# shroglck/open-pi-zero

Hardware: AMD Instinct MI355X
Metric: train samples/sec at gbsz 1024 (bf16 fwd+bwd+clip+AdamW) (higher is better)
Workload: dtype bf16; 1 GPU; Pi0 bridge training step: 256 img + 20 text + 1 proprio + 4 action tokens; model=pi0 (SigLIP-So400m/14 + Gemma-2B + 0.3B action expert), global_batch=1024, micro_batch=256, grad_accum=4, seq_len=281, parallelism=dp1

## Files before the change

### include/pz_abi.h

```cpp
#ifndef PZ_ABI_H
#define PZ_ABI_H

#include <stdint.h>

#ifdef __cplusplus
extern "C" {
#endif

#define PZ_ABI_VERSION 22

enum {
  PZ_OK = 0,
  PZ_ERR_INVALID_ARG = 1,
  PZ_ERR_LAUNCH = 2,
  PZ_ERR_UNSUPPORTED = 3,
};

enum {
  PZ_EPI_NONE = 0,
  PZ_EPI_GELU = 1,
  PZ_EPI_GEGLU = 2,
  PZ_EPI_SILU = 3,
  PZ_EPI_DGELU = 4,
  PZ_EPI_DSILU = 5,
  PZ_EPI_DGEGLU = 6,
};

typedef struct pz_gemm_args {
  int64_t M, N, K;
  const void* A; int64_t lda; int32_t a_kcontig;
  const void* B; int64_t ldb; int32_t b_kcontig;
  void* C; int64_t ldc; int32_t c_fp32;
  int64_t batch, batch_inner;
  int64_t sA_outer, sA_inner, sB_outer, sB_inner, sC_outer, sC_inner, sR_outer, sR_inner;
  int32_t epilogue;
  float alpha;
  int32_t beta_accum;
  const void* bias;
  const void* resid; int64_t ld_resid;
  void* aux; int64_t ld_aux;
  int64_t geglu_inter;
  void* workspace; int64_t ws_bytes;
  const void* norm_w; float norm_eps;
  int32_t fp8_mode; const float* a_row_scale;
  const void* A2; int64_t lda2;
  const void* B2; int64_t ldb2;
  int64_t K2;
} pz_gemm_args;
int pz_gemm(const pz_gemm_args* args, void* stream);
#define PZ_ABSMAX_PARTS 1024
int pz_fp8_quant_vt(const void* v, int64_t ldv, int64_t v_bstride, int64_t Z, int64_t nk, void* vt, float* vs,
                    int64_t ldt, void* stream);
int pz_fp8_quant_attn(const void* q, int64_t nqr, const void* k, int64_t nkr, const void* v, int64_t ldv,
                      int64_t v_bstride, int64_t Z, int64_t nk, void* qc, float* qs, void* kc, float* ks, void* vt,
                      float* vs, int64_t ldt, void* stream);
int pz_rmsnorm_fwd_f8(const void* x, int64_t ldx, const void* w, void* q, int64_t ldq, float* qscale, int64_t R,
                      int64_t D, float eps, void* stream);
int pz_layernorm_fwd_f8(const void* x, int64_t ldx, const void* w, const void* b, void* q, int64_t ldq, float* qscale,
                        int64_t R, int64_t D, float eps, void* stream);
int pz_fp8_quant_rows(const void* x, int64_t ldx, void* q, int64_t ldq, float* row_scale, int64_t R, int64_t D,
                      void* stream);
int pz_fp8_quant_tensor(const void* x, int64_t n, void* q, float inv_scale, void* stream);
int pz_fp8_absmax(const void* x, int64_t n, float* parts, void* stream);
const char* pz_gemm_kernel_name(const pz_gemm_args* args);

typedef struct pz_small_gemm_args {
  int64_t M, N, K;
  const void* A; int64_t sAm, sAk;
  const void* B; int64_t sBk, sBn;
  void* C; int64_t ldc;
  const void* bias;
  float alpha;
  int32_t beta;
} pz_small_gemm_args;
int pz_gemm_small(const pz_small_gemm_args* args, void* stream);

int pz_rmsnorm_fwd(const void* x, int64_t ldx, const void* w, void* y, int64_t ldy, float* rstd,
                   int64_t R, int64_t D, float eps, void* stream);
int pz_rmsnorm_bwd(const void* dy, int64_t lddy, const void* x, int64_t ldx, const void* w,
                   const float* rstd, const void* dres, void* dx, int64_t lddx, float* dw_part,
                   int64_t R, int64_t D, void* stream);
int pz_layernorm_fwd(const void* x, int64_t ldx, const void* w, const void* b, void* y, int64_t ldy,
                     float* mean, float* rstd, int64_t R, int64_t D, float eps, void* stream);
int pz_layernorm_bwd(const void* dy, int64_t lddy, const void* x, int64_t ldx, const void* w,
                     const float* mean, const float* rstd, const void* dres, void* dx, int64_t lddx,
                     float* dw_part, float* db_part, int64_t R, int64_t D, float* dx_part, void* stream);
int64_t pz_norm_rows_per_part(void);
int pz_reduce_parts(const float* part, int64_t P, int64_t D, void* out, int32_t beta, void* stream);
typedef struct pz_reduce_seg {
  const float* part; int64_t P, D; void* out; int32_t beta;
} pz_reduce_seg;
int pz_reduce_parts_multi(const pz_reduce_seg* segs, int32_t nseg, void* stream);
int pz_act_bwd_colsum(const void* dh, int64_t lddh, const void* pre, int64_t ldpre, void* dpre, int64_t M, int64_t N,
                      int32_t act, float* ws, int64_t ws_rows, void* dbias, int32_t beta, void* stream);
int pz_colsum(const void* X, int64_t ld, int64_t M, int64_t N, void* out, int32_t beta, float* ws,
              void* stream);
int pz_batch_sum(const void* X, int64_t B, int64_t stride, int64_t n, void* out, int32_t beta, void* stream);

int pz_rope_table(float* cs, int64_t max_pos, int64_t head_dim, float theta, void* stream);
int pz_qkv_rope_split(const void* qkv, const int64_t* pos, const float* cs, void* q_out, void* k_out,
                      void* v_out, int64_t B, int64_t T, int64_t nh, int64_t nkv, int64_t hd,
                      int64_t Lq, int64_t qoff, int64_t Lk, int64_t koff, void* stream);
typedef struct pz_qkv_rope_args {
  const void* x; int64_t ldx;
  const void* W; int64_t ldw;
  int64_t M, N, K;
  const void* norm_w; float norm_eps;
  const int64_t* pos; const float* cs;
  void* q_out; void* k_out; void* v_out;
  int64_t T, nh, hd, Lq, qoff, Lk, koff;
  int32_t w_fp8; float w_scale;
  const void* x2; int64_t ldx2;
  const void* W2; int64_t ldw2;
  int64_t K2;
} pz_qkv_rope_args;
int pz_gemv_qkv_rope(const pz_qkv_rope_args* a, void* stream);
int pz_gemm_qkv_rope(const pz_qkv_rope_args* a, void* stream);
int pz_qkv_rope_split_bwd(const void* dq, const void* dk, const void* dv, const int64_t* pos,
                          const float* cs, void* dqkv, int64_t B, int64_t T, int64_t nh, int64_t nkv,
                          int64_t hd, int64_t Lq, int64_t qoff, int64_t Lk, int64_t koff, void* stream);

typedef struct pz_softmax_args {
  const float* S; int64_t lds;
  void* P; int64_t ldp;
  void* tcap;
  int64_t R, N;
  float scale, cap;
  int32_t mask_mode;
  int64_t rows_per_batch, heads, qoff;
  const int32_t* cnt; int64_t prefix, cond;
  const float* mask; int64_t ldm, mask_bstride;
} pz_softmax_args;
int pz_attn_softmax(const pz_softmax_args* a, void* stream);
int pz_attn_softmax_bwd(const void* P, const float* dP, int64_t lddp, const void* tcap, void* dS,
                        int64_t ldp, int64_t R, int64_t N, float scale, float cap, void* stream);

typedef struct pz_flash_args {
  int64_t Z, H, nq, nk, head_dim;
  const void* q; int64_t ldq, q_bstride, q_hstride;
  const void* k; int64_t ldk, k_bstride, k_hstride;
  const void* v; int64_t ldv, v_bstride, v_hstride;
  int32_t n_groups;
  int64_t g_row0[3];
  void* g_o[3];
  int64_t g_bstride[3], g_ld[3];
  int64_t o_hstride;
  float* lse;
  float scale, cap;
  int32_t mask_mode;
  const int32_t* cnt; int64_t prefix, cond, rows_per_token;
  const void* g_do[3];
  float* delta;
  void* dq; void* dk; void* dv;
  float* ws; int64_t ws_bytes;
  int64_t mask_row0;
} pz_flash_args;
int pz_flash_fwd(const pz_flash_args* a, void* stream);
int pz_flash_fwd_f8(const pz_flash_args* a, const void* qc, const float* qs, const void* kc, const float* ks,
                    int64_t krows, const void* vtc, const float* vs, int64_t ldvt, void* stream);
int pz_flash_fwd_probs(const pz_flash_args* a, void* P, void* tcap, int64_t ldp, void* stream);
int pz_flash_bwd_ds(const pz_flash_args* a, const void* P, const void* tcap, void* dS, int64_t ldp, void* stream);
int pz_flash_bwd_prep(const pz_flash_args* a, void* stream);
int pz_flash_bwd(const pz_flash_args* a, void* stream);

typedef struct pz_decode_attn_args {
  const void* q; int64_t ldq, Lq, qoff;
  const void* k; const void* v; int64_t k_bstride, v_bstride;
  void* o; int64_t ldo;
  int64_t B, nh, T, nk, head_dim;
  float scale, cap;
  const int32_t* cnt; int64_t prefix, cond, qtok0;
  float* ws; int64_t ws_bytes;
} pz_decode_attn_args;
int64_t pz_decode_attn_ws_bytes(int64_t B, int64_t rows, int64_t nk);
int pz_decode_attn(const pz_decode_attn_args* a, void* stream);

int pz_patchify(const void* pix, void* cols, int64_t B, int64_t H, int64_t W, int64_t ps, int64_t ldc,
                void* stream);
int pz_embed_merge(const int64_t* ids, const void* table, int64_t vocab, const void* img, void* out,
                   int64_t B, int64_t P, int64_t D, int64_t n_img, int64_t image_token, int64_t pad_token,
                   float emb_scale, float img_scale, void* stream);
int pz_embed_merge_bwd(const int64_t* ids, const void* dout, void* dimg, int64_t B, int64_t P,
                       int64_t D, int64_t n_img, int64_t image_token, float img_scale, void* stream);

int pz_time_embed(const float* t, void* out, int64_t B, int64_t D, float max_period, int32_t mode,
                  void* stream);
int pz_time_embed_rows(const float* t, void* out, int64_t ldo, int64_t B, int64_t H, int64_t D, float max_period,
                       int32_t mode, void* stream);
int pz_concat_time(const void* temb, const void* e1, void* out, int64_t B, int64_t H, int64_t D,
                   void* stream);
int pz_split_time_grad(const void* dcat, void* de1, int64_t rows, int64_t D, void* stream);
int pz_flow_psi(const float* x0, const float* x1, const float* t, void* psi, int64_t B, int64_t HA,
                float sig_min, void* stream);
int pz_flow_loss(const void* v, int64_t ldv, int64_t v_bstride, const float* x0, const float* x1, float* loss,
                 void* dv, const float* grad_scale, int64_t B, int64_t H, int64_t A, float sig_min, void* stream);
int pz_action_in(const float* action, int64_t A, const void* w1, const void* b1, const float* t, void* cat,
                 int64_t ldc, int64_t B, int64_t H, int64_t D, float max_period, int32_t mode, void* stream);
int pz_action_out(const void* x, int64_t ldx, const void* norm_w, float eps, const void* wd, const void* bd, int64_t D,
                  int64_t A, float* action, float* t, int64_t B, int64_t H, float dt, void* stream);
int pz_euler_step(float* action, const void* v, int64_t ldv, int64_t v_bstride, float* t, int64_t B, int64_t H,
                  int64_t A, float dt, void* stream);
int pz_clamp(float* x, int64_t n, float lo, float hi, void* stream);

int pz_geglu_bwd(const void* dh, int64_t lddh, const void* gu, int64_t ldgu, void* dgu, void* h_out,
                 int64_t ldh, int64_t M, int64_t I, void* stream);
int pz_act_bwd(const void* dh, int64_t lddh, const void* pre, int64_t ldpre, void* dpre, void* h_out,
               int64_t ldh, int64_t M, int64_t N, int32_t act ,
               void* stream);

int pz_adamw(void* p, const void* g, float* m, float* v, int64_t n, float lr, float beta1,
             float beta2, float eps, float wd, float bc1, float bc2, const float* gscale, void* stream);
#define PZ_SUMSQ_PARTS 2048
int pz_sumsq(const void* g, int64_t n, float* parts, void* stream);
int pz_clip_coef(const float* parts, int64_t nparts, float* coef, float* norm_out, float max_norm,
                 void* stream);

typedef struct pz_adamw8_args {
  void* p; const void* g;
  uint8_t* s1; uint8_t* s2;
  float* absmax1; float* absmax2;
  float* m32; float* v32;
  const int64_t* seg;
  int64_t nseg, nblocks;
  const float* qmap1; const float* qmap2;
  float beta1, beta2, omb1, omb2, step, epsc, decay;
  const float* gscale;
} pz_adamw8_args;
int pz_adamw8bit(const pz_adamw8_args* a, void* stream);

int pz_adamw8bit_r(const pz_adamw8_args* a, void* comp, int32_t mode, uint64_t rng_key, int64_t rng_base,
                   void* stream);
int pz_adamw_r(void* p, void* comp, const void* g, float* m, float* v, int64_t n, float lr, float beta1, float beta2,
               float eps, float wd, float bc1, float bc2, const float* gscale, int32_t mode, uint64_t rng_key,
               int64_t rng_base, void* stream);

int pz_fill_uniform(void* x, int32_t out_fp32, int64_t n, uint64_t seed, float off, float scale,
                    void* stream);
int pz_copy_rows(const void* src, int64_t sld, int64_t sbs, void* dst, int64_t dld, int64_t dbs, int64_t B,
                 int64_t rows, int64_t D, float scale, int32_t beta, void* stream);
int pz_cast_f32_bf16(const float* x, void* y, int64_t n, void* stream);
int pz_cast_bf16_f32(const void* x, float* y, int64_t n, void* stream);

int pz_adaln_fwd(const void* x, int64_t ldx, const void* y, int64_t ldy, const float* gate_pre,
                 const void* gate_bias, void* xm, int64_t ldxm, const float* gamma_pre, const void* gamma_bias,
                 const float* beta, void* h, int64_t ldh, float* rstd, int64_t ldmod, int64_t R, int64_t D,
                 int64_t rows_per_sample, float eps, void* stream);
int pz_adaln_norm_bwd(const void* dh, int64_t lddh, const void* x, int64_t ldx, const float* rstd,
                      const float* gamma_pre, const void* gamma_bias, const void* dres, void* dx, int64_t lddx,
                      float* dgamma_pre, float* dbeta, int64_t ldmod, int64_t R, int64_t D, int64_t rows_per_sample,
                      void* stream);
int pz_adaln_gate_bwd(const void* dout, int64_t lddo, const void* y, int64_t ldy, const float* gate_pre,
                      const void* gate_bias, void* dy, int64_t lddy, float* dgate_pre, int64_t ldmod, int64_t R,
                      int64_t D, int64_t rows_per_sample, void* stream);

int64_t pz_lora_wgrad_ws_bytes(int64_t M, int64_t D, int64_t R);
int pz_lora_wgrad(const void* Q, int64_t ldq, const void* P, int64_t ldp, void* out, int64_t ld_out, int64_t M,
                  int64_t D, int64_t R, int32_t transposed, float alpha, int32_t beta, void* ws, int64_t ws_bytes,
                  void* stream);

int pz_avg_lerp(void* avg, const void* p, int64_t n, float w, void* stream);
int pz_avg_swap(void* a, void* b, int64_t n, void* stream);

#define PZ_OBS_MAX_TAPS 64
#define PZ_OBS_MAX_EXTENT 16384
enum { PZ_OBS_NORM_BOUND = 0, PZ_OBS_NORM_GAUSSIAN = 1 };
int64_t pz_image_resize_scratch_bytes(int64_t n, int64_t H_in, int64_t S);
int pz_image_resize_norm(const void* frames, int32_t channels_last, int64_t n, int64_t H_in, int64_t W_in, int64_t S,
                         const void* h_first, const void* h_count, const void* h_w, int64_t h_taps,
                         const void* v_first, const void* v_count, const void* v_w, int64_t v_taps, const void* lut,
                         void* scratch, int64_t scratch_bytes, void* out, void* stream);
int pz_proprio_normalize(const void* x, void* y, int64_t rows, int64_t D, const void* a, const void* b, int32_t mode,
                         void* stream);
int pz_action_denormalize(const void* x, void* y, int64_t rows, int64_t D, int64_t n_pass, const void* a,
                          const void* b, int32_t mode, void* stream);

enum {
  PZ_AUG_CROP = 1,
  PZ_AUG_BRIGHTNESS = 2,
  PZ_AUG_CONTRAST = 4,
  PZ_AUG_SATURATION = 8,
  PZ_AUG_HUE = 16,
  PZ_AUG_ALL = 31
};
int64_t pz_image_augment_scratch_bytes(int64_t n, int64_t S);
int pz_image_augment(const void* frames, int32_t channels_last, int64_t n, int64_t S, const void* params,
                     const void* mask, int32_t ops_union, const void* lut, void* scratch, int64_t scratch_bytes,
                     void* out, void* stream);
int pz_image_resize_u8(const void* frames, int32_t channels_last, int64_t n, int64_t H_in, int64_t W_in, int64_t S,
                       const void* h_first, const void* h_count, const void* h_w, int64_t h_taps, const void* v_first,
                       const void* v_count, const void* v_w, int64_t v_taps, void* scratch, int64_t scratch_bytes,
                       void* out, void* stream);

int pz_debug_poison_lds(uint32_t word, void* stream);
int pz_debug_spin(int64_t wgs, int64_t ticks, void* stream);

const char* pz_last_error(void);
int pz_abi_version(void);

#ifdef __cplusplus
}
#endif
#endif
```

### open-pi-zero_amd/csrc/pz_attn.hip

```cpp
#include "pz_common.h"

namespace {

__global__ void rope_table_kernel(float* cs, int64_t max_pos, int hd, float theta) {
  const int half = hd / 2;
  const int64_t idx = (int64_t)blockIdx.x * blockDim.x + threadIdx.x;
  if (idx >= (max_pos + 1) * half) return;
  const int64_t pos = idx / half;
  const int i = (int)(idx % half);
  const float expo = (float)(2 * i) / (float)hd;
  const float inv = 1.0f / powf(theta, expo);
  const float f = (float)pos * inv;
  cs[2 * idx] = cosf(f);
  cs[2 * idx + 1] = sinf(f);
}

__global__ void qkv_rope_split_kernel(const bf16_t* __restrict__ qkv, const int64_t* __restrict__ pos,
                                      const float* __restrict__ cs, bf16_t* q_out, bf16_t* k_out,
                                      bf16_t* v_out, int64_t T, int nh, int nkv, int hd, int64_t Lq,
                                      int64_t qoff, int64_t Lk, int64_t koff) {
  const int64_t t = blockIdx.x, b = blockIdx.y;
  const int64_t tok = b * T + t;
  const int half = hd / 2;
  const int width = (nh + 2 * nkv) * hd;
  const bf16_t* src = qkv + tok * width;
  const float* c = cs + pos[tok] * hd;
  if (q_out) {
    bf16_t* dq = q_out + (b * Lq + qoff + t) * (int64_t)(nh * hd);
    for (int e = threadIdx.x; e < nh * half; e += blockDim.x) {
      const int h = e / half, i = e % half;
      const float x1 = bf2f(src[h * hd + i]), x2 = bf2f(src[h * hd + i + half]);
      const float co = c[2 * i], si = c[2 * i + 1];
      float o1, o2;
      rope_pair(x1, x2, co, si, o1, o2);
      dq[h * hd + i] = f2bf(o1);
      dq[h * hd + i + half] = f2bf(o2);
    }
  }
  bf16_t* dk = k_out + (b * Lk + koff + t) * (int64_t)(nkv * hd);
  bf16_t* dv = v_out + (b * Lk + koff + t) * (int64_t)(nkv * hd);
  const bf16_t* sk = src + nh * hd;
  const bf16_t* sv = src + (nh + nkv) * hd;
  for (int e = threadIdx.x; e < nkv * half; e += blockDim.x) {
    const int h = e / half, i = e % half;
    const float x1 = bf2f(sk[h * hd + i]), x2 = bf2f(sk[h * hd + i + half]);
    const float co = c[2 * i], si = c[2 * i + 1];
    float o1, o2;
    rope_pair(x1, x2, co, si, o1, o2);
    dk[h * hd + i] = f2bf(o1);
    dk[h * hd + i + half] = f2bf(o2);
  }
  for (int e = threadIdx.x; e < nkv * hd; e += blockDim.x) dv[e] = sv[e];
}

__global__ void qkv_rope_split_bwd_kernel(const bf16_t* __restrict__ dq, const bf16_t* __restrict__ dk,
                                          const bf16_t* __restrict__ dv, const int64_t* __restrict__ pos,
                                          const float* __restrict__ cs, bf16_t* dqkv, int64_t T, int nh,
                                          int nkv, int hd, int64_t Lq, int64_t qoff, int64_t Lk,
                                          int64_t koff) {
  const int64_t t = blockIdx.x, b = blockIdx.y;
  const int64_t tok = b * T + t;
  const int half = hd / 2;
  const int width = (nh + 2 * nkv) * hd;
  bf16_t* dst = dqkv + tok * width;
  const float* c = cs + pos[tok] * hd;
  const bf16_t* sq = dq ? dq + (b * Lq + qoff + t) * (int64_t)(nh * hd) : nullptr;
  for (int e = threadIdx.x; e < nh * half; e += blockDim.x) {
    const int h = e / half, i = e % half;
    float o1 = 0.f, o2 = 0.f;
    if (sq) {
      const float y1 = bf2f(sq[h * hd + i]), y2 = bf2f(sq[h * hd + i + half]);
      const float co = c[2 * i], si = c[2 * i + 1];
      o1 = y1 * co + y2 * si;
      o2 = y2 * co - y1 * si;
    }
    dst[h * hd + i] = f2bf(o1);
    dst[h * hd + i + half] = f2bf(o2);
  }
  const bf16_t* sk = dk + (b * Lk + koff + t) * (int64_t)(nkv * hd);
  const bf16_t* sv = dv + (b * Lk + koff + t) * (int64_t)(nkv * hd);
  bf16_t* ok = dst + nh * hd;
  bf16_t* ov = dst + (nh + nkv) * hd;
  for (int e = threadIdx.x; e < nkv * half; e += blockDim.x) {
    const int h = e / half, i = e % half;
    const float y1 = bf2f(sk[h * hd + i]), y2 = bf2f(sk[h * hd + i + half]);
    const float co = c[2 * i], si = c[2 * i + 1];
    ok[h * hd + i] = f2bf(y1 * co + y2 * si);
    ok[h * hd + i + half] = f2bf(y2 * co - y1 * si);
  }
  for (int e = threadIdx.x; e < nkv * hd; e += blockDim.x) ov[e] = sv[e];
}

__device__ __forceinline__ bool block_allowed(int64_t i, int64_t j, int64_t cnt, int64_t P, int64_t C) {
  if (i < P) return i < cnt && j < cnt;
  if (i < P + C) return j < cnt || (j >= P && j < P + C);
  return j < cnt || j >= P;
}

template <int MAXE>
__global__ void __launch_bounds__(256) softmax_kernel(pz_softmax_args a) {
  const int lane = threadIdx.x & 63;
  const int64_t row = (int64_t)blockIdx.x * 4 + (threadIdx.x >> 6);
  if (row >= a.R) return;
  const float* s = a.S + row * a.lds;
  int64_t b = 0, qi = 0;
  if (a.mask_mode != 0) {
    b = row / a.rows_per_batch;
    qi = a.qoff + (row % a.rows_per_batch) / a.heads;
  }
  const int64_t cnt = a.mask_mode == 1 ? (int64_t)a.cnt[b] : 0;
  const float* mrow = a.mask_mode == 2 ? a.mask + b * a.mask_bstride + (qi - a.qoff) * a.ldm : nullptr;
  float x[MAXE];
  bool ok[MAXE];
  float mx = -INFINITY;
#pragma unroll
  for (int e = 0; e < MAXE; ++e) {
    const int64_t j = lane + 64 * e;
    ok[e] = false;
    x[e] = 0.f;
    if (j < a.N) {
      float v = s[j] * a.scale;
      if (a.cap > 0.f) v = a.cap * tanhf(v / a.cap);
      bool al = true;
      if (a.mask_mode == 1) al = block_allowed(qi, j, cnt, a.prefix, a.cond);
      else if (a.mask_mode == 2) {
        v += mrow[j];
        al = v > -INFINITY;
      }
      x[e] = v;
      ok[e] = al;
      if (al) mx = fmaxf(mx, v);
    }
  }
  mx = warp_max(mx);
  bf16_t* prow = (bf16_t*)a.P + row * a.ldp;
  bf16_t* trow = a.tcap ? (bf16_t*)a.tcap + row * a.ldp : nullptr;
  if (mx == -INFINITY) {
    const float u = 1.f / (float)a.N;
    for (int64_t j = lane; j < a.ldp; j += 64) {
      prow[j] = f2bf(j < a.N ? u : 0.f);
      if (trow) trow[j] = 0;
    }
    return;
  }
  float sum = 0.f;
#pragma unroll
  for (int e = 0; e < MAXE; ++e) {
    const float p = ok[e] ? __expf(x[e] - mx) : 0.f;
    x[e] = p;
    sum += p;
  }
  const float inv = 1.f / warp_sum(sum);
#pragma unroll
  for (int e = 0; e < MAXE; ++e) {
    const int64_t j = lane + 64 * e;
    if (j < a.N) {
      prow[j] = f2bf(x[e] * inv);
      if (trow) {
        float v = s[j] * a.scale;
        trow[j] = f2bf(a.cap > 0.f ? tanhf(v / a.cap) : 0.f);
      }
    }
  }
  for (int64_t j = a.N + lane; j < a.ldp; j += 64) {
    prow[j] = 0;
    if (trow) trow[j] = 0;
  }
}

__device__ __forceinline__ u32x2 pack4bf(const float (&v)[4]) { return u32x2{pack2bf(v[0], v[1]), pack2bf(v[2], v[3])}; }

template <int MAXV>
__global__ void __launch_bounds__(256) softmax4_kernel(pz_softmax_args a) {
  const int lane = threadIdx.x & 63;
  const int64_t row = (int64_t)blockIdx.x * 4 + (threadIdx.x >> 6);
  if (row >= a.R) return;
  const float* s = a.S + row * a.lds;
  int b = 0, qi = 0;
  if (a.mask_mode != 0) {
    const int rr = (int)row, rpb = (int)a.rows_per_batch;
    b = rr / rpb;
    qi = (int)a.qoff + (rr - b * rpb) / (int)a.heads;
  }
  const int cnt = a.mask_mode == 1 ? a.cnt[b] : 0;
  const int P = (int)a.prefix, Cc = (int)a.cond, N = (int)a.N;
  const float* mrow = a.mask_mode == 2 ? a.mask + b * a.mask_bstride + (qi - a.qoff) * a.ldm : nullptr;
  const float inv_cap = a.cap > 0.f ? 1.f / a.cap : 0.f;
  float x[MAXV][4], th[MAXV][4];
  bool ok[MAXV][4];
  float mx = -INFINITY;
#pragma unroll
  for (int e = 0; e < MAXV; ++e) {
    const int j0 = 4 * (lane + 64 * e);
    f32x4 sv = {0.f, 0.f, 0.f, 0.f};
    if (j0 < N) sv = *reinterpret_cast<const f32x4*>(s + j0);
#pragma unroll
    for (int i = 0; i < 4; ++i) {
      const int j = j0 + i;
      float v = j < N ? sv[i] * a.scale : 0.f;
      th[e][i] = 0.f;
      if (a.cap > 0.f && j < N) {
        th[e][i] = tanh_fast(v * inv_cap);
        v = a.cap * th[e][i];
      }
      bool al = j < N;
      if (al && a.mask_mode == 1) al = block_allowed(qi, j, cnt, P, Cc);
      else if (al && a.mask_mode == 2) {
        v += mrow[j];
        al = v > -INFINITY;
      }
      x[e][i] = v;
      ok[e][i] = al;
      if (al) mx = fmaxf(mx, v);
    }
  }
  mx = warp_max(mx);
  bf16_t* prow = (bf16_t*)a.P + row * a.ldp;
  bf16_t* trow = a.tcap ? (bf16_t*)a.tcap + row * a.ldp : nullptr;
  const int ldp = (int)a.ldp;
  if (mx == -INFINITY) {
    const float u = 1.f / (float)N;
    for (int j0 = 4 * lane; j0 < ldp; j0 += 256) {
      float v[4] = {j0 < N ? u : 0.f, j0 + 1 < N ? u : 0.f, j0 + 2 < N ? u : 0.f, j0 + 3 < N ? u : 0.f};
      *reinterpret_cast<u32x2*>(prow + j0) = pack4bf(v);
      if (trow) *reinterpret_cast<u32x2*>(trow + j0) = u32x2{0u, 0u};
    }
    return;
  }
  float sum = 0.f;
#pragma unroll
  for (int e = 0; e < MAXV; ++e)
#pragma unroll
    for (int i = 0; i < 4; ++i) {
      const float pv = ok[e][i] ? __expf(x[e][i] - mx) : 0.f;
      x[e][i] = pv;
      sum += pv;
    }
  const float inv = 1.f / warp_sum(sum);
#pragma unroll
  for (int e = 0; e < MAXV; ++e) {
    const int j0 = 4 * (lane + 64 * e);
    if (j0 < ldp) {
      float v[4] = {x[e][0] * inv, x[e][1] * inv, x[e][2] * inv, x[e][3] * inv};
      *reinterpret_cast<u32x2*>(prow + j0) = pack4bf(v);
      if (trow) *reinterpret_cast<u32x2*>(trow + j0) = pack4bf(th[e]);
    }
  }
}

template <int MAXV>
__global__ void __launch_bounds__(256) softmax_bwd4_kernel(const bf16_t* __restrict__ Pm, const float* __restrict__ dP,
                                                           int64_t lddp, const bf16_t* __restrict__ tcap, bf16_t* dS,
                                                           int64_t ldp, int64_t R, int N, float scale, float cap) {
  const int lane = threadIdx.x & 63;
  const int64_t row = (int64_t)blockIdx.x * 4 + (threadIdx.x >> 6);
  if (row >= R) return;
  const bf16_t* prow = Pm + row * ldp;
  const float* drow = dP + row * lddp;
  float p[MAXV][4], d[MAXV][4];
  float dot = 0.f;
#pragma unroll
  for (int e = 0; e < MAXV; ++e) {
    const int j0 = 4 * (lane + 64 * e);
    u32x2 pw = {0u, 0u};
    f32x4 dv = {0.f, 0.f, 0.f, 0.f};
    if (j0 < N) {
      pw = *reinterpret_cast<const u32x2*>(prow + j0);
      dv = *reinterpret_cast<const f32x4*>(drow + j0);
    }
    p[e][0] = __uint_as_float(pw[0] << 16);
    p[e][1] = __uint_as_float(pw[0] & 0xffff0000u);
    p[e][2] = __uint_as_float(pw[1] << 16);
    p[e][3] = __uint_as_float(pw[1] & 0xffff0000u);
#pragma unroll
    for (int i = 0; i < 4; ++i) {
      d[e][i] = j0 + i < N ? dv[i] : 0.f;
      dot += p[e][i] * d[e][i];
    }
  }
  dot = warp_sum(dot);
  bf16_t* orow = dS + row * ldp;
#pragma unroll
  for (int e = 0; e < MAXV; ++e) {
    const int j0 = 4 * (lane + 64 * e);
    if (j0 < (int)ldp) {
      float g[4];
      u32x2 tw = {0u, 0u};
      if (cap > 0.f && j0 < N) tw = *reinterpret_cast<const u32x2*>(tcap + row * ldp + j0);
      const float t[4] = {__uint_as_float(tw[0] << 16), __uint_as_float(tw[0] & 0xffff0000u),
                          __uint_as_float(tw[1] << 16), __uint_as_float(tw[1] & 0xffff0000u)};
#pragma unroll
      for (int i = 0; i < 4; ++i) {
        g[i] = j0 + i < N ? p[e][i] * (d[e][i] - dot) * scale : 0.f;
        if (cap > 0.f) g[i] *= (1.f - t[i] * t[i]);
      }
      *reinterpret_cast<u32x2*>(orow + j0) = pack4bf(g);
    }
  }
}

template <int MAXE>
__global__ void __launch_bounds__(256) softmax_bwd_kernel(const bf16_t* __restrict__ P,
                                                          const float* __restrict__ dP, int64_t lddp,
                                                          const bf16_t* __restrict__ tcap, bf16_t* dS,
                                                          int64_t ldp, int64_t R, int64_t N, float scale,
                                                          float cap) {
  const int lane = threadIdx.x & 63;
  const int64_t row = (int64_t)blockIdx.x * 4 + (threadIdx.x >> 6);
  if (row >= R) return;
  const bf16_t* prow = P + row * ldp;
  const float* drow = dP + row * lddp;
  float p[MAXE], d[MAXE];
  float dot = 0.f;
#pragma unroll
  for (int e = 0; e < MAXE; ++e) {
    const int64_t j = lane + 64 * e;
    p[e] = 0.f;
    d[e] = 0.f;
    if (j < N) {
      p[e] = bf2f(prow[j]);
      d[e] = drow[j];
      dot += p[e] * d[e];
    }
  }
  dot = warp_sum(dot);
  bf16_t* orow = dS + row * ldp;
#pragma unroll
  for (int e = 0; e < MAXE; ++e) {
    const int64_t j = lane + 64 * e;
    if (j < N) {
      float g = p[e] * (d[e] - dot) * scale;
      if (cap > 0.f) {
        const float t = bf2f(tcap[row * ldp + j]);
        g *= (1.f - t * t);
      }
      orow[j] = f2bf(g);
    }
  }
  for (int64_t j = N + lane; j < ldp; j += 64) orow[j] = 0;
}

}

extern "C" int pz_rope_table(float* cs, int64_t max_pos, int64_t head_dim, float theta, void* stream) {
  PZ_CHECK_ARG(cs && max_pos >= 0 && head_dim % 2 == 0, "rope_table: bad args");
  const int64_t n = (max_pos + 1) * (head_dim / 2);
  hipLaunchKernelGGL(rope_table_kernel, dim3((unsigned)((n + 255) / 256)), dim3(256), 0, (hipStream_t)stream, cs,
                     max_pos, (int)head_dim, theta);
  PZ_CHECK_LAUNCH();
  return PZ_OK;
}

extern "C" int pz_qkv_rope_split(const void* qkv, const int64_t* pos, const float* cs, void* q_out, void* k_out,
                                 void* v_out, int64_t B, int64_t T, int64_t nh, int64_t nkv, int64_t hd,
                                 int64_t Lq, int64_t qoff, int64_t Lk, int64_t koff, void* stream) {
  PZ_CHECK_ARG(qkv && pos && cs && k_out && v_out && B > 0 && T > 0 && hd % 2 == 0, "qkv_rope_split: bad args");
  PZ_CHECK_ARG(koff + T <= Lk && (!q_out || qoff + T <= Lq), "qkv_rope_split: token range");
  hipLaunchKernelGGL(qkv_rope_split_kernel, dim3((unsigned)T, (unsigned)B), dim3(256), 0, (hipStream_t)stream,
                     (const bf16_t*)qkv, pos, cs, (bf16_t*)q_out, (bf16_t*)k_out, (bf16_t*)v_out, T, (int)nh,
                     (int)nkv, (int)hd, Lq, qoff, Lk, koff);
  PZ_CHECK_LAUNCH();
  return PZ_OK;
}

extern "C" int pz_qkv_rope_split_bwd(const void* dq, const void* dk, const void* dv, const int64_t* pos,
                                     const float* cs, void* dqkv, int64_t B, int64_t T, int64_t nh, int64_t nkv,
                                     int64_t hd, int64_t Lq, int64_t qoff, int64_t Lk, int64_t koff, void* stream) {
  PZ_CHECK_ARG(dk && dv && pos && cs && dqkv && B > 0 && T > 0, "qkv_rope_split_bwd: bad args");
  hipLaunchKernelGGL(qkv_rope_split_bwd_kernel, dim3((unsigned)T, (unsigned)B), dim3(256), 0,
                     (hipStream_t)stream, (const bf16_t*)dq, (const bf16_t*)dk, (const bf16_t*)dv, pos, cs,
                     (bf16_t*)dqkv, T, (int)nh, (int)nkv, (int)hd, Lq, qoff, Lk, koff);
  PZ_CHECK_LAUNCH();
  return PZ_OK;
}

extern "C" int pz_attn_softmax(const pz_softmax_args* a, void* stream) {
  PZ_CHECK_ARG(a && a->S && a->P && a->R > 0 && a->N > 0 && a->ldp >= a->N && a->lds >= a->N,
               "attn_softmax: bad args");
  PZ_CHECK_ARG(a->N <= 1024, "attn_softmax: N=%lld > 1024 unsupported", (long long)a->N);
  if (a->mask_mode == 1) PZ_CHECK_ARG(a->cnt && a->rows_per_batch > 0 && a->heads > 0, "attn_softmax: block mask");
  if (a->mask_mode == 2) PZ_CHECK_ARG(a->mask && a->rows_per_batch > 0 && a->heads > 0, "attn_softmax: mask");
  dim3 grid((unsigned)((a->R + 3) / 4));
  hipStream_t st = (hipStream_t)stream;
  const bool vec = a->lds % 4 == 0 && a->ldp % 4 == 0 && PZ_ALIGNED(a->S, 16) && PZ_ALIGNED(a->P, 8) &&
                   (!a->tcap || PZ_ALIGNED(a->tcap, 8)) && a->R < (1LL << 31) && a->ldp <= 1024;
  if (vec) {
    if (a->ldp <= 512) hipLaunchKernelGGL(softmax4_kernel<2>, grid, dim3(256), 0, st, *a);
    else hipLaunchKernelGGL(softmax4_kernel<4>, grid, dim3(256), 0, st, *a);
    PZ_CHECK_LAUNCH();
    return PZ_OK;
  }
  if (a->N <= 256) hipLaunchKernelGGL(softmax_kernel<4>, grid, dim3(256), 0, st, *a);
  else if (a->N <= 512) hipLaunchKernelGGL(softmax_kernel<8>, grid, dim3(256), 0, st, *a);
  else hipLaunchKernelGGL(softmax_kernel<16>, grid, dim3(256), 0, st, *a);
  PZ_CHECK_LAUNCH();
  return PZ_OK;
}

extern "C" int pz_attn_softmax_bwd(const void* P, const float* dP, int64_t lddp, const void* tcap, void* dS,
                                   int64_t ldp, int64_t R, int64_t N, float scale, float cap, void* stream) {
  PZ_CHECK_ARG(P && dP && dS && R > 0 && N > 0 && N <= 1024 && (cap <= 0.f || tcap), "attn_softmax_bwd: bad args");
  dim3 grid((unsigned)((R + 3) / 4));
  hipStream_t st = (hipStream_t)stream;
  if (lddp % 4 == 0 && ldp % 4 == 0 && ldp <= 1024 && PZ_ALIGNED(dP, 16) && PZ_ALIGNED(P, 8) && PZ_ALIGNED(dS, 8) &&
      (cap <= 0.f || PZ_ALIGNED(tcap, 8))) {
    if (ldp <= 512)
      hipLaunchKernelGGL(softmax_bwd4_kernel<2>, grid, dim3(256), 0, st, (const bf16_t*)P, dP, lddp,
                         (const bf16_t*)tcap, (bf16_t*)dS, ldp, R, (int)N, scale, cap);
    else
      hipLaunchKernelGGL(softmax_bwd4_kernel<4>, grid, dim3(256), 0, st, (const bf16_t*)P, dP, lddp,
                         (const bf16_t*)tcap, (bf16_t*)dS, ldp, R, (int)N, scale, cap);
    PZ_CHECK_LAUNCH();
    return PZ_OK;
  }
  if (N <= 256)
    hipLaunchKernelGGL(softmax_bwd_kernel<4>, grid, dim3(256), 0, st, (const bf16_t*)P, dP, lddp,
                       (const bf16_t*)tcap, (bf16_t*)dS, ldp, R, N, scale, cap);
  else if (N <= 512)
    hipLaunchKernelGGL(softmax_bwd_kernel<8>, grid, dim3(256), 0, st, (const bf16_t*)P, dP, lddp,
                       (const bf16_t*)tcap, (bf16_t*)dS, ldp, R, N, scale, cap);
  else
    hipLaunchKernelGGL(softmax_bwd_kernel<16>, grid, dim3(256), 0, st, (const bf16_t*)P, dP, lddp,
                       (const bf16_t*)tcap, (bf16_t*)dS, ldp, R, N, scale, cap);
  PZ_CHECK_LAUNCH();
  return PZ_OK;
}
```

### open-pi-zero_amd/csrc/pz_flash.hip

```cpp
#include "pz_common.h"

#include <type_traits>

namespace {

constexpr int FA_KB = 64;
constexpr int FA_NW = 4;
constexpr int FA_QS = 32;

template <int HD>
struct FaDims {
  static constexpr int HDK = (HD + 31) / 32 * 32;
  static constexpr int HDV = (HD + 15) / 16 * 16;
  static constexpr int NKS = HDK / 32;
  static constexpr int NDB = HDV / 16;
  static constexpr int ROW = HD == 256 ? 272 : (HD == 72 ? 112 : HDK + 16);
  static constexpr int FNW = HD == 256 ? 8 : 4;
  static constexpr int FNQB = HD == 256 ? 1 : 2;
};

__device__ __forceinline__ bool fa_allowed(int64_t i, int64_t j, int64_t cnt, int64_t P, int64_t C) {
  if (i < P) return i < cnt && j < cnt;
  if (i < P + C) return j < cnt || (j >= P && j < P + C);
  return j < cnt || j >= P;
// ... 2000 lines not shown
#pragma unroll
    for (int kb2 = 0; kb2 < 2; ++kb2) {
      const int key = wave * 32 + kb2 * 16 + (lane & 15);
      fs_load_rows(kfr[kb2], K + key * a.ldk, g);
      fs_load_rows(vfr[kb2], V + key * a.ldv, g);
    }
  };
  auto issue = [&](int64_t un, int t1) {
    const int64_t bn = un / a.H, hn = un % a.H;
    const bf16_t* Q = (const bf16_t*)a.q + bn * a.q_bstride + hn * a.q_hstride;
    const bf16_t* dO = (const bf16_t*)a.g_do[0] + bn * a.g_bstride[0] + hn * a.o_hstride;
    const float* L = a.lse + un * FS_N;
    const float* D = a.delta + un * FS_N;
    char* nxt = fa_smem + (t1 & 1) * 2 * FS_IMG;
#pragma unroll
    for (int s2 = 0; s2 < FS_PER; ++s2)
      fs_glds16(side[s2] ? (const bf16_t*)(L + offl[s2]) : Q + offq[s2], nxt + (wave * FS_PER + s2) * 1024);
#pragma unroll
    for (int s2 = 0; s2 < FS_PER; ++s2)
      fs_glds16(side[s2] ? (const bf16_t*)(D + offl[s2]) : dO + offd[s2], nxt + FS_IMG + (wave * FS_PER + s2) * 1024);
  };
  if (w0) tix.take(tk);
  FS_WAIT_VM(0);
  if (w0) tix.publish(tk, fa_smem + 2 * FS_IMG + FS_SLOT1);
  FS_BARRIER();
  int64_t u = tix.unit(tix.read(fa_smem + 2 * FS_IMG + FS_SLOT1));
  if (u < units) {
    issue_kv(u);
    issue(u, 0);
    if (w0) tix.take(tk);
  }
  FS_WAIT_VM(0);
  if (u < units && w0) tix.publish(tk, fa_smem + FS_SLOT1);
  FS_BARRIER();
  for (int t = 0; u < units; ++t) {
    const int64_t b = u / a.H, h = u % a.H;
#pragma unroll
    for (int kb2 = 0; kb2 < 2; ++kb2) {
#pragma unroll
      for (int ks = 0; ks < 3; ++ks) asm volatile("" : "+v"(kfr[kb2][ks]), "+v"(vfr[kb2][ks]));
      if (g != 0) kfr[kb2][2] = vfr[kb2][2] = bf16x8{};
    }
    const int64_t un = tix.unit(tix.read(fa_smem + (t & 1) * 2 * FS_IMG + FS_SLOT1));
    if (un < units) {
      issue(un, t + 1);
      if (w0) tix.take(tk);
    }
    const char* cur = fa_smem + (t & 1) * 2 * FS_IMG;
    const bf16_t* Qall = reinterpret_cast<const bf16_t*>(cur);
    const bf16_t* Dall = reinterpret_cast<const bf16_t*>(cur + FS_IMG);
    f32x4 dk[5][2], dv[5][2];
#pragma unroll
    for (int db = 0; db < 5; ++db) dk[db][0] = dk[db][1] = dv[db][0] = dv[db][1] = f32x4{0.f, 0.f, 0.f, 0.f};
    auto step = [&](int qs, bool last) {
      const int r0 = qs * FA_QS;
      const bf16_t* Qs = Qall + r0 * FS_ROW;
      const bf16_t* Ds = Dall + r0 * FS_ROW;
      unsigned pp[2][2][2], dd[2][2][2];
#pragma unroll
      for (int i = 0; i < 2; ++i) {
        const f32x4 l2r = *reinterpret_cast<const f32x4*>(Qs + (i * 16 + 4 * g) * FS_ROW + 72) * FA_LOG2E;
        const f32x4 dlr = *reinterpret_cast<const f32x4*>(Ds + (i * 16 + 4 * g) * FS_ROW + 72);
        bf16x8 qa[3], da[3];
#pragma unroll
        for (int ks = 0; ks < 3; ++ks) {
          qa[ks] = fs_frag(Qs, i * 16, ks, lane);
          da[ks] = fs_frag(Ds, i * 16, ks, lane);
        }
#pragma unroll
        for (int kb2 = 0; kb2 < 2; ++kb2) {
          f32x4 sv = {0.f, 0.f, 0.f, 0.f}, dp = {0.f, 0.f, 0.f, 0.f};
#pragma unroll
          for (int ks = 0; ks < 3; ++ks) {
            sv = mfma(qa[ks], kfr[kb2][ks], sv);
            dp = mfma(da[ks], vfr[kb2][ks], dp);
          }
          float pe[4], de[4];
#pragma unroll
          for (int e = 0; e < 4; ++e) {
            pe[e] = __builtin_amdgcn_exp2f(fmaf(sv[e], sl2, -l2r[e]));
            de[e] = pe[e] * (dp[e] - dlr[e]);
          }
          pp[i][kb2][0] = pack2bf(pe[0], pe[1]);
          pp[i][kb2][1] = pack2bf(pe[2], pe[3]);
          dd[i][kb2][0] = pack2bf(de[0], de[1]);
          dd[i][kb2][1] = pack2bf(de[2], de[3]);
        }
      }
      if (last && un < units) issue_kv(un);
      auto cat4 = [](unsigned x0, unsigned x1, unsigned x2, unsigned x3) {
        return __builtin_bit_cast(bf16x8, u32x4{x0, x1, x2, x3});
      };
      const bf16x8 pb0 = cat4(pp[0][0][0], pp[0][0][1], pp[1][0][0], pp[1][0][1]);
      const bf16x8 pb1 = cat4(pp[0][1][0], pp[0][1][1], pp[1][1][0], pp[1][1][1]);
      const bf16x8 sb0 = cat4(dd[0][0][0], dd[0][0][1], dd[1][0][0], dd[1][0][1]);
      const bf16x8 sb1 = cat4(dd[0][1][0], dd[0][1][1], dd[1][1][0], dd[1][1][1]);
      const unsigned da0 = fs_lds_addr(Ds + (4 * g + ((lane & 15) >> 2)) * FS_ROW + 4 * (lane & 3));
      const unsigned qa0 = fs_lds_addr(Qs + (4 * g + ((lane & 15) >> 2)) * FS_ROW + 4 * (lane & 3));
      s16x4 td[5][2], tq[5][2];
#define FS_TR(db, hf)                                             \
  td[db][hf] = fs_tr<(16 * (hf)) * FS_ROW * 2 + (db) * 32>(da0); \
  tq[db][hf] = fs_tr<(16 * (hf)) * FS_ROW * 2 + (db) * 32>(qa0)
#define FS_MM(db)                                                                \
  {                                                                              \
    const bf16x8 dt = fs_cat(td[db][0], td[db][1]), qt = fs_cat(tq[db][0], tq[db][1]); \
    dv[db][0] = mfma(dt, pb0, dv[db][0]);                                        \
    dv[db][1] = mfma(dt, pb1, dv[db][1]);                                        \
    dk[db][0] = mfma(qt, sb0, dk[db][0]);                                        \
    dk[db][1] = mfma(qt, sb1, dk[db][1]);                                        \
  }
      FS_TR(0, 0); FS_TR(0, 1); FS_TR(1, 0); FS_TR(1, 1);
      asm volatile("s_waitcnt lgkmcnt(0)"
                   : "+v"(td[0][0]), "+v"(td[0][1]), "+v"(td[1][0]), "+v"(td[1][1]), "+v"(tq[0][0]), "+v"(tq[0][1]),
                     "+v"(tq[1][0]), "+v"(tq[1][1]));
      FS_TR(2, 0); FS_TR(2, 1); FS_TR(3, 0); FS_TR(3, 1);
      FS_MM(0) FS_MM(1)
      asm volatile("s_waitcnt lgkmcnt(0)"
                   : "+v"(td[2][0]), "+v"(td[2][1]), "+v"(td[3][0]), "+v"(td[3][1]), "+v"(tq[2][0]), "+v"(tq[2][1]),
                     "+v"(tq[3][0]), "+v"(tq[3][1]));
      FS_TR(4, 0); FS_TR(4, 1);
      FS_MM(2) FS_MM(3)
      asm volatile("s_waitcnt lgkmcnt(0)" : "+v"(td[4][0]), "+v"(td[4][1]), "+v"(tq[4][0]), "+v"(tq[4][1]));
      FS_MM(4)
#undef FS_MM
#undef FS_TR
    };
#pragma unroll 1
    for (int qs = 0; qs < FS_N / FA_QS - 1; ++qs) step(qs, false);
    step(FS_N / FA_QS - 1, true);
    FS_WAIT_VM(0);
#pragma unroll
    for (int kb2 = 0; kb2 < 2; ++kb2) {
      const int key = wave * 32 + kb2 * 16 + (lane & 15);
      bf16_t* dK = (bf16_t*)a.dk + b * a.k_bstride + h * a.k_hstride + (int64_t)key * a.ldk;
      bf16_t* dV = (bf16_t*)a.dv + b * a.v_bstride + h * a.v_hstride + (int64_t)key * a.ldv;
#pragma unroll
      for (int db = 0; db < 5; ++db) {
        const int d = db * 16 + 4 * g;
        if (d < 72) {
          *reinterpret_cast<u32x2*>(dK + d) = u32x2{pack2bf(dk[db][kb2][0] * a.scale, dk[db][kb2][1] * a.scale),
                                                    pack2bf(dk[db][kb2][2] * a.scale, dk[db][kb2][3] * a.scale)};
          *reinterpret_cast<u32x2*>(dV + d) =
              u32x2{pack2bf(dv[db][kb2][0], dv[db][kb2][1]), pack2bf(dv[db][kb2][2], dv[db][kb2][3])};
        }
      }
    }
    if (un < units && w0) tix.publish(tk, fa_smem + ((t + 1) & 1) * 2 * FS_IMG + FS_SLOT1);
    FS_BARRIER();
    u = un;
  }
}

constexpr int JD_SLOT = 64 * 512, JD_SMEM = 4 * JD_SLOT;

struct JdDma {
  int wave, lane;
  bool trs;
  __device__ __forceinline__ JdDma(int wave_, int lane_, bool trs_) : wave(wave_), lane(lane_), trs(trs_) {}
  __device__ __forceinline__ void issue(const bf16_t* X, int64_t ld, int kb, int nk, char* slot, int) const {
    int ln = lane;
    asm volatile("" : "+v"(ln));
#pragma unroll
    for (int s = 0; s < 4; ++s) {
      const int r = 2 * (wave * 4 + s) + (ln >> 5), pch = ln & 31;
      const int coff = 8 * (pch ^ (trs ? 2 * (r & 7) : (r & 15)));
      int key = kb * 64 + r;
      key = key < nk ? key : nk - 1;
      fs_glds16(X + (int64_t)key * ld + coff, slot + (wave * 4 + s) * 1024);
    }
  }
};

template <int K2, int DG>
__device__ __forceinline__ void jd_pv_group(f32x4 (&o)[16], const unsigned (&vs)[8], const bf16x8& pk) {
  s16x4 tv[4][2];
#define JD_TR(u, hf) tv[u][hf] = fs_tr<(K2 * 32 + 16 * (hf)) * 512 + ((DG * 4 + (u)) & 8) * 32>(vs[(DG * 4 + (u)) & 7])
  JD_TR(0, 0); JD_TR(0, 1); JD_TR(1, 0); JD_TR(1, 1); JD_TR(2, 0); JD_TR(2, 1); JD_TR(3, 0); JD_TR(3, 1);
#undef JD_TR
  asm volatile("s_waitcnt lgkmcnt(0)"
               : "+v"(tv[0][0]), "+v"(tv[0][1]), "+v"(tv[1][0]), "+v"(tv[1][1]), "+v"(tv[2][0]), "+v"(tv[2][1]),
                 "+v"(tv[3][0]), "+v"(tv[3][1]));
#pragma unroll
  for (int u = 0; u < 4; ++u) o[DG * 4 + u] = mfma(fs_cat(tv[u][0], tv[u][1]), pk, o[DG * 4 + u]);
}

template <bool CAP>
__global__ void __launch_bounds__(JP_NW * 64, 1) flash_fwd_probs_dma_kernel(pz_flash_args a, bf16_t* P, bf16_t* TC,
                                                                         int64_t ldp) {
  extern __shared__ __attribute__((aligned(16))) char fa_smem[];
  constexpr int RPW = JP_NW * 16;
  const int lane = threadIdx.x & 63, wave = threadIdx.x >> 6, g = lane >> 4, l15 = lane & 15;
  int64_t zh;
  int qblk;
  fa_unit_block((int)((a.nq + RPW - 1) / RPW), (int)(a.Z * a.H), zh, qblk);
  const int64_t b = zh / a.H, h = zh % a.H;
  const int64_t r = (int64_t)qblk * RPW + wave * 16 + l15;
  const bool live = r < a.nq;
  const bf16_t* Q = (const bf16_t*)a.q + b * a.q_bstride + h * a.q_hstride;
  const bf16_t* K = (const bf16_t*)a.k + b * a.k_bstride + h * a.k_hstride;
  const bf16_t* V = (const bf16_t*)a.v + b * a.v_bstride + h * a.v_hstride;
  const FaMask mk(a, b);
  const FaFast ff(a);
  const int nk = (int)a.nk;
  const JdDma dmk(wave, lane, false), dmv(wave, lane, true);
  bf16x8 qf[8];
  {
    const bf16_t* qrow = Q + (live ? r : 0) * a.ldq + 8 * g;
#define JD_QLD(ks) asm volatile("global_load_dwordx4 %0, %1, off offset:%2" : "=v"(qf[ks]) : "v"(qrow), "i"((ks) * 64) : "memory")
    JD_QLD(0); JD_QLD(1); JD_QLD(2); JD_QLD(3); JD_QLD(4); JD_QLD(5); JD_QLD(6); JD_QLD(7);
#undef JD_QLD
  }
  auto issue = [&](int s) {
    char* slot = fa_smem + (s % 4) * JD_SLOT;
    if (s < 5) dmk.issue(K, a.ldk, s, nk, slot, wave);
    else dmv.issue(V, a.ldv, s - 5, nk, slot, wave);
  };
  issue(0);
  issue(1);
  issue(2);
  const int t = mk.token((int)r);
  const bool dead = mk.dead(t);
  const int rb = fa_row_bits(mk, t), full_keys = fa_full_keys(mk);
  const bool clean = __ballot(dead || !live) == 0ull;
  f32x4 sc[JP_MAXKB][4];
  u32x2 tcv[JP_MAXKB][4];
  float mx = -INFINITY;
  auto logits_blk = [&](int kb) {
    auto logits = [&](auto FAST) {
#pragma unroll
      for (int i = 0; i < 4; ++i) {
        float tv[4];
#pragma unroll
        for (int e = 0; e < 4; ++e) {
          const float sv = sc[kb][i][e];
          float th = 0.f, x2;
          if constexpr (CAP) {
            th = fmaf(-2.f, __builtin_amdgcn_rcpf(__builtin_amdgcn_exp2f(sv * ff.k2) + 1.f), 1.f);
            x2 = th * ff.crow_live;
          } else {
            x2 = sv * ff.crow_live;
          }
          if constexpr (!decltype(FAST)::value) {
            const int j = kb * FA_KB + i * 16 + 4 * g + e;
            const bool ok = j < nk && (j < full_keys || ((rb >> fa_key_class(mk, j)) & 1));
            x2 = ok ? x2 : -INFINITY;
            th = (dead || j >= nk) ? 0.f : th;
          }
          sc[kb][i][e] = x2;
          mx = fmaxf(mx, x2);
          tv[e] = th;
        }
        tcv[kb][i] = u32x2{pack2bf(tv[0], tv[1]), pack2bf(tv[2], tv[3])};
      }
    };
    if (clean && (kb + 1) * 64 <= full_keys) logits(std::true_type{});
    else logits(std::false_type{});
  };
#pragma unroll
  for (int kb = 0; kb < JP_MAXKB; ++kb) {
    FS_WAIT_VM(8);
    FS_BARRIER();
    if (kb == 0)
      asm volatile("" : "+v"(qf[0]), "+v"(qf[1]), "+v"(qf[2]), "+v"(qf[3]), "+v"(qf[4]), "+v"(qf[5]), "+v"(qf[6]),
                   "+v"(qf[7]));
    issue(kb + 3);
    const char* slot = fa_smem + (kb % 4) * JD_SLOT + l15 * 512;
#pragma unroll
    for (int i = 0; i < 4; ++i) sc[kb][i] = f32x4{0.f, 0.f, 0.f, 0.f};
#pragma unroll
    for (int ks = 0; ks < 8; ++ks) {
      const char* kp = slot + 16 * ((4 * ks + g) ^ l15);
#pragma unroll
      for (int i = 0; i < 4; ++i) sc[kb][i] = mfma(*reinterpret_cast<const bf16x8*>(kp + i * 8192), qf[ks], sc[kb][i]);
    }
    if (kb >= 1) logits_blk(kb - 1);
  }
  logits_blk(JP_MAXKB - 1);
  FS_WAIT_VM(4);
  bf16_t* prow = P + (b * a.nq + (live ? r : 0)) * ldp;
  if (TC) {
    bf16_t* trow = TC + (b * a.nq + (live ? r : 0)) * ldp;
#pragma unroll
    for (int kb = 0; kb < JP_MAXKB; ++kb)
#pragma unroll
      for (int i = 0; i < 4; ++i) {
        const int j0 = kb * FA_KB + i * 16 + 4 * g;
        if (clean && (kb + 1) * 64 <= full_keys) *reinterpret_cast<u32x2*>(trow + j0) = tcv[kb][i];
        else if (live && j0 < ldp) *reinterpret_cast<u32x2*>(trow + j0) = tcv[kb][i];
      }
  }
  mx = fs_max4(mx);
  float sum = 0.f;
#pragma unroll
  for (int kb = 0; kb < JP_MAXKB; ++kb)
#pragma unroll
    for (int i = 0; i < 4; ++i)
#pragma unroll
      for (int e = 0; e < 4; ++e) {
        const float pv = __builtin_amdgcn_exp2f(sc[kb][i][e] - mx);
        sc[kb][i][e] = pv;
        sum += pv;
      }
  sum = fs_sum4(sum);
  const float inv = 1.f / sum, uni = 1.f / (float)nk;
  bf16x8 pf[JP_MAXKB][2];
#pragma unroll
  for (int kb = 0; kb < JP_MAXKB; ++kb) {
    unsigned pk[4][2];
    auto probs = [&](auto FAST) {
#pragma unroll
      for (int i = 0; i < 4; ++i) {
        if constexpr (decltype(FAST)::value) {
          pk[i][0] = pack2bf(sc[kb][i][0] * inv, sc[kb][i][1] * inv);
          pk[i][1] = pack2bf(sc[kb][i][2] * inv, sc[kb][i][3] * inv);
        } else {
          float pv[4];
#pragma unroll
          for (int e = 0; e < 4; ++e) {
            const int j = kb * FA_KB + i * 16 + 4 * g + e;
            pv[e] = dead ? (j < nk ? uni : 0.f) : sc[kb][i][e] * inv;
          }
          pk[i][0] = pack2bf(pv[0], pv[1]);
          pk[i][1] = pack2bf(pv[2], pv[3]);
        }
        const int j0 = kb * FA_KB + i * 16 + 4 * g;
        if (decltype(FAST)::value || (live && j0 < ldp)) *reinterpret_cast<u32x2*>(prow + j0) = u32x2{pk[i][0], pk[i][1]};
      }
    };
    if (clean && (kb + 1) * 64 <= full_keys) probs(std::true_type{});
    else probs(std::false_type{});
    pf[kb][0] = __builtin_bit_cast(bf16x8, u32x4{pk[0][0], pk[0][1], pk[1][0], pk[1][1]});
    pf[kb][1] = __builtin_bit_cast(bf16x8, u32x4{pk[2][0], pk[2][1], pk[3][0], pk[3][1]});
  }
  f32x4 o[16];
#pragma unroll
  for (int db = 0; db < 16; ++db) o[db] = f32x4{0.f, 0.f, 0.f, 0.f};
  const int q4 = l15 >> 2, p4 = lane & 3, w = 4 * (g & 1) + q4;
  unsigned va[8];
#pragma unroll
  for (int d7 = 0; d7 < 8; ++d7) va[d7] = fs_lds_addr(fa_smem + (4 * g + q4) * 512 + 32 * (d7 ^ w) + 8 * p4);
#pragma unroll
  for (int kb = 0; kb < JP_MAXKB; ++kb) {
    const int s = 5 + kb;
    if (s == 7) FS_WAIT_VM(8);
    if (s == 8) FS_WAIT_VM(4);
    if (s == 9) FS_WAIT_VM(0);
    FS_BARRIER();
    if (s + 3 <= 9) issue(s + 3);
    const unsigned sb = (unsigned)((s % 4) * JD_SLOT);
    unsigned vs[8];
#pragma unroll
    for (int d7 = 0; d7 < 8; ++d7) vs[d7] = va[d7] + sb;
    jd_pv_group<0, 0>(o, vs, pf[kb][0]);
    jd_pv_group<0, 1>(o, vs, pf[kb][0]);
    jd_pv_group<0, 2>(o, vs, pf[kb][0]);
    jd_pv_group<0, 3>(o, vs, pf[kb][0]);
    jd_pv_group<1, 0>(o, vs, pf[kb][1]);
    jd_pv_group<1, 1>(o, vs, pf[kb][1]);
    jd_pv_group<1, 2>(o, vs, pf[kb][1]);
    jd_pv_group<1, 3>(o, vs, pf[kb][1]);
  }
  if (!live) return;
  const FaRow fr{&a};
  const int gi = fr.grp(r);
  bf16_t* O = (bf16_t*)a.g_o[gi] + fr.off(b, h, r, gi);
#pragma unroll
  for (int db = 0; db < 16; ++db) {
    const int d = db * 16 + 4 * g;
    *reinterpret_cast<u32x2*>(O + d) = u32x2{pack2bf(o[db][0], o[db][1]), pack2bf(o[db][2], o[db][3])};
  }
}

__global__ void __launch_bounds__(JP_NW * 64, 1) flash_bwd_ds_dma_kernel(pz_flash_args a, const bf16_t* P,
                                                                      const bf16_t* TC, bf16_t* dS, int64_t ldp) {
  extern __shared__ __attribute__((aligned(16))) char fa_smem[];
  constexpr int RPW = JP_NW * 16;
  const int lane = threadIdx.x & 63, wave = threadIdx.x >> 6, g = lane >> 4, l15 = lane & 15;
  int64_t zh;
  int qblk;
  fa_unit_block((int)((a.nq + RPW - 1) / RPW), (int)(a.Z * a.H), zh, qblk);
  const int64_t b = zh / a.H, h = zh % a.H;
  const int64_t r = (int64_t)qblk * RPW + wave * 16 + l15;
  const bool live = r < a.nq;
  const bool want_dq = a.dq != nullptr;
  const bf16_t* V = (const bf16_t*)a.v + b * a.v_bstride + h * a.v_hstride;
  const bf16_t* K = want_dq ? (const bf16_t*)a.k + b * a.k_bstride + h * a.k_hstride : V;
  const int64_t ldk = want_dq ? a.ldk : a.ldv;
  const int nk = (int)a.nk;
  const JdDma dmv(wave, lane, false), dmk(wave, lane, true);
  auto issue = [&](int s) {
    char* slot = fa_smem + (s % 4) * JD_SLOT;
    if (s < 5) dmv.issue(V, a.ldv, s, nk, slot, wave);
    else dmk.issue(K, ldk, s - 5, nk, slot, wave);
  };
  bf16x8 df[8];
  bool has_do;
  {
    const FaRow fr{&a};
    const int gi = live ? fr.grp(r) : 0;
    has_do = live && a.g_do[gi];
    const bf16_t* dOr = has_do ? (const bf16_t*)a.g_do[gi] + fr.off(b, h, r, gi) + 8 * g : V;
#define JD_DLD(ks) asm volatile("global_load_dwordx4 %0, %1, off offset:%2" : "=v"(df[ks]) : "v"(dOr), "i"((ks) * 64) : "memory")
    JD_DLD(0); JD_DLD(1); JD_DLD(2); JD_DLD(3); JD_DLD(4); JD_DLD(5); JD_DLD(6); JD_DLD(7);
#undef JD_DLD
  }
  issue(0);
  issue(1);
  issue(2);
  const bf16_t* prow = P + (b * a.nq + (live ? r : 0)) * ldp;
  const bf16_t* trow = TC ? TC + (b * a.nq + (live ? r : 0)) * ldp : prow;
  const bool clean = __ballot(!live) == 0ull;
  f32x4 dp[JP_MAXKB][4];
  u32x2 pw[JP_MAXKB][4], tw[JP_MAXKB][4];
#pragma unroll
  for (int kb = 0; kb < JP_MAXKB; ++kb) {
    FS_WAIT_VM(8);
    FS_BARRIER();
    if (kb == 0) {
      asm volatile("" : "+v"(df[0]), "+v"(df[1]), "+v"(df[2]), "+v"(df[3]), "+v"(df[4]), "+v"(df[5]), "+v"(df[6]),
                   "+v"(df[7]));
      if (!has_do) {
#pragma unroll
        for (int ks = 0; ks < 8; ++ks) df[ks] = bf16x8{};
      }
    }
    issue(kb + 3);
    const char* slot = fa_smem + (kb % 4) * JD_SLOT + l15 * 512;
#pragma unroll
    for (int i = 0; i < 4; ++i) dp[kb][i] = f32x4{0.f, 0.f, 0.f, 0.f};
#pragma unroll
    for (int ks = 0; ks < 8; ++ks) {
      const char* vp = slot + 16 * ((4 * ks + g) ^ l15);
#pragma unroll
      for (int i = 0; i < 4; ++i) dp[kb][i] = mfma(*reinterpret_cast<const bf16x8*>(vp + i * 8192), df[ks], dp[kb][i]);
    }
  }
  int gl = g;
  asm volatile("" : "+v"(gl));
#pragma unroll
  for (int k2 = 0; k2 < JP_MAXKB; ++k2)
#pragma unroll
    for (int i = 0; i < 4; ++i) {
      const int j0 = k2 * FA_KB + i * 16 + 4 * gl;
      const int jc = j0 < ldp ? j0 : 0;
      asm volatile("global_load_dwordx2 %0, %1, off" : "=v"(pw[k2][i]) : "v"(prow + jc) : "memory");
    }
#pragma unroll
  for (int k2 = 0; k2 < JP_MAXKB; ++k2)
#pragma unroll
    for (int i = 0; i < 4; ++i) {
      const int j0 = k2 * FA_KB + i * 16 + 4 * gl;
      const int jc = j0 < ldp ? j0 : 0;
      asm volatile("global_load_dwordx2 %0, %1, off" : "=v"(tw[k2][i]) : "v"(trow + jc) : "memory");
    }
  FS_WAIT_VM(20);
  bf16_t* orow = dS + (b * a.nq + (live ? r : 0)) * ldp;
  const bool cap = a.cap > 0.f;
  float dot = 0.f;
#pragma unroll
  for (int kb = 0; kb < JP_MAXKB; ++kb)
#pragma unroll
    for (int i = 0; i < 4; ++i) {
      asm volatile("" : "+v"(pw[kb][i]));
      const int j0 = kb * FA_KB + i * 16 + 4 * g;
      if (!(live && j0 < nk)) pw[kb][i] = u32x2{0u, 0u};
      const float p0 = __uint_as_float(pw[kb][i][0] << 16), p1 = __uint_as_float(pw[kb][i][0] & 0xffff0000u);
      const float p2 = __uint_as_float(pw[kb][i][1] << 16), p3 = __uint_as_float(pw[kb][i][1] & 0xffff0000u);
      dot += p0 * dp[kb][i][0] + p1 * dp[kb][i][1] + p2 * dp[kb][i][2] + p3 * dp[kb][i][3];
    }
  dot += __shfl_xor(dot, 16, 64);
  dot += __shfl_xor(dot, 32, 64);
  FS_WAIT_VM(0);
#pragma unroll
  for (int kb = 0; kb < JP_MAXKB; ++kb)
#pragma unroll
    for (int i = 0; i < 4; ++i) asm volatile("" : "+v"(tw[kb][i]));
  bf16x8 dsf[JP_MAXKB][2];
#pragma unroll
  for (int kb = 0; kb < JP_MAXKB; ++kb) {
    unsigned pk[4][2];
#pragma unroll
    for (int i = 0; i < 4; ++i) {
      const int j0 = kb * FA_KB + i * 16 + 4 * g;
      const u32x2 tv2 = (cap && live && j0 < nk) ? tw[kb][i] : u32x2{0u, 0u};
      const float pv[4] = {__uint_as_float(pw[kb][i][0] << 16), __uint_as_float(pw[kb][i][0] & 0xffff0000u),
                           __uint_as_float(pw[kb][i][1] << 16), __uint_as_float(pw[kb][i][1] & 0xffff0000u)};
      const float tv[4] = {__uint_as_float(tv2[0] << 16), __uint_as_float(tv2[0] & 0xffff0000u),
                           __uint_as_float(tv2[1] << 16), __uint_as_float(tv2[1] & 0xffff0000u)};
      float x[4];
#pragma unroll
      for (int e = 0; e < 4; ++e) {
        x[e] = pv[e] * (dp[kb][i][e] - dot) * a.scale;
        if (cap) x[e] *= fmaf(-tv[e], tv[e], 1.f);
      }
      pk[i][0] = pack2bf(x[0], x[1]);
      pk[i][1] = pack2bf(x[2], x[3]);
      if (clean ? j0 < ldp : (live && j0 < ldp)) *reinterpret_cast<u32x2*>(orow + j0) = u32x2{pk[i][0], pk[i][1]};
    }
    dsf[kb][0] = __builtin_bit_cast(bf16x8, u32x4{pk[0][0], pk[0][1], pk[1][0], pk[1][1]});
    dsf[kb][1] = __builtin_bit_cast(bf16x8, u32x4{pk[2][0], pk[2][1], pk[3][0], pk[3][1]});
  }
  f32x4 dq[16];
#pragma unroll
  for (int db = 0; db < 16; ++db) dq[db] = f32x4{0.f, 0.f, 0.f, 0.f};
  const int q4 = l15 >> 2, p4 = lane & 3, w = 4 * (g & 1) + q4;
  unsigned ka[8];
#pragma unroll
  for (int d7 = 0; d7 < 8; ++d7) ka[d7] = fs_lds_addr(fa_smem + (4 * g + q4) * 512 + 32 * (d7 ^ w) + 8 * p4);
#pragma unroll
  for (int kb = 0; kb < JP_MAXKB; ++kb) {
    const int s = 5 + kb;
    if (s == 8) FS_WAIT_VM(4);
    if (s == 9) FS_WAIT_VM(0);
    FS_BARRIER();
    if (s + 3 <= 9) issue(s + 3);
    if (want_dq) {
      const unsigned sb = (unsigned)((s % 4) * JD_SLOT);
      unsigned ks_[8];
#pragma unroll
      for (int d7 = 0; d7 < 8; ++d7) ks_[d7] = ka[d7] + sb;
      jd_pv_group<0, 0>(dq, ks_, dsf[kb][0]);
      jd_pv_group<0, 1>(dq, ks_, dsf[kb][0]);
      jd_pv_group<0, 2>(dq, ks_, dsf[kb][0]);
      jd_pv_group<0, 3>(dq, ks_, dsf[kb][0]);
      jd_pv_group<1, 0>(dq, ks_, dsf[kb][1]);
      jd_pv_group<1, 1>(dq, ks_, dsf[kb][1]);
      jd_pv_group<1, 2>(dq, ks_, dsf[kb][1]);
      jd_pv_group<1, 3>(dq, ks_, dsf[kb][1]);
    }
  }
  if (!live || !want_dq) return;
  bf16_t* dQ = (bf16_t*)a.dq + b * a.q_bstride + h * a.q_hstride + r * a.ldq;
#pragma unroll
  for (int db = 0; db < 16; ++db) {
    const int d = db * 16 + 4 * g;
    *reinterpret_cast<u32x2*>(dQ + d) = u32x2{pack2bf(dq[db][0], dq[db][1]), pack2bf(dq[db][2], dq[db][3])};
  }
}

constexpr int F8_KB = 128, F8_KT = F8_KB * 256, F8_VT = 256 * F8_KB;
constexpr int F8_SMEM = 2 * (F8_KT + F8_VT) + 2 * F8_KB * 4;

__device__ __forceinline__ int f8_kswz(int r) { return (r & 3) | ((r >> 5) << 2); }
__device__ __forceinline__ int f8_vswz(int d) { return (d & 6) | ((d >> 3) & 1); }
__device__ __forceinline__ i32x8 f8_cat(const u32x4& lo, const u32x4& hi) {
  return i32x8{(int)lo[0], (int)lo[1], (int)lo[2], (int)lo[3], (int)hi[0], (int)hi[1], (int)hi[2], (int)hi[3]};
}
__device__ __forceinline__ unsigned f8_enc4(float a, float b, float c, float d) {
  int v = __builtin_amdgcn_cvt_pk_fp8_f32(a, b, 0, false);
  v = __builtin_amdgcn_cvt_pk_fp8_f32(c, d, v, true);
  return (unsigned)v;
}

__global__ void __launch_bounds__(512) flash_fwd_f8_kernel(pz_flash_args a, const uint8_t* __restrict__ qc,
                                                          const float* __restrict__ qs, const uint8_t* __restrict__ kc,
                                                          const float* __restrict__ ks, int64_t krows,
                                                          const uint8_t* __restrict__ vtc,
                                                          const float* __restrict__ vs, int64_t ldvt) {
  extern __shared__ __attribute__((aligned(16))) char fa_smem[];
  auto Kt = [&](int bi) { return fa_smem + bi * F8_KT; };
  auto Vt = [&](int bi) { return fa_smem + 2 * F8_KT + bi * F8_VT; };
  auto Sk = [&](int bi) { return reinterpret_cast<float*>(fa_smem + 2 * (F8_KT + F8_VT)) + bi * F8_KB; };
  const int t = threadIdx.x, lane = t & 63, wave = t >> 6, g = lane >> 4, l15 = lane & 15;
  const int64_t b = blockIdx.y;
  const int64_t q0 = (int64_t)blockIdx.x * 128 + wave * 16;
  const int64_t r = q0 + l15;
  const FaMask mk(a, b);
  const int nkb = (int)((a.nk + F8_KB - 1) / F8_KB);
  const int per = (nkb + (int)gridDim.z - 1) / (int)gridDim.z;
  const int kb_begin = (int)blockIdx.z * per, kb_end = min(nkb, kb_begin + per);
  u32x4 sk_[4], sv_[4];
  float sks = 0.f;
  auto load = [&](int kb) {
#pragma unroll
    for (int j = 0; j < 4; ++j) {
      const int c = t + 512 * j;
      const int64_t kr = min((int64_t)kb * F8_KB + (c >> 4), krows - 1);
      sk_[j] = *reinterpret_cast<const u32x4*>(kc + (b * krows + kr) * 256 + (c & 15) * 16);
      sv_[j] = *reinterpret_cast<const u32x4*>(vtc + (b * 256 + (c >> 3)) * ldvt + (int64_t)kb * F8_KB + (c & 7) * 16);
    }
    if (t < F8_KB) sks = ks[b * krows + min((int64_t)kb * F8_KB + t, krows - 1)];
  };
  auto store = [&](int bi) {
#pragma unroll
    for (int j = 0; j < 4; ++j) {
      const int c = t + 512 * j;
      const int kr = c >> 4, d = c >> 3;
      *reinterpret_cast<u32x4*>(Kt(bi) + kr * 256 + (((c & 15) ^ f8_kswz(kr)) << 4)) = sk_[j];
      *reinterpret_cast<u32x4*>(Vt(bi) + d * 128 + (((c & 7) ^ f8_vswz(d)) << 4)) = sv_[j];
    }
    if (t < F8_KB) Sk(bi)[t] = sks;
  };
  i32x8 qf[2];
  float sq = 0.f;
  {
    const bool ok = r < a.nq;
    const uint8_t* qr = qc + (b * a.nq + (ok ? r : 0)) * 256 + 32 * g;
#pragma unroll
    for (int k2 = 0; k2 < 2; ++k2) {
      const u32x4 lo = ok ? *reinterpret_cast<const u32x4*>(qr + 128 * k2) : u32x4{0u, 0u, 0u, 0u};
      const u32x4 hi = ok ? *reinterpret_cast<const u32x4*>(qr + 128 * k2 + 16) : u32x4{0u, 0u, 0u, 0u};
      qf[k2] = f8_cat(lo, hi);
    }
    if (ok) sq = qs[b * a.nq + r];
  }
  const int tq = mk.token((int)r);
  f32x4 o[16];
#pragma unroll
  for (int db = 0; db < 16; ++db) o[db] = f32x4{0.f, 0.f, 0.f, 0.f};
  float m = -INFINITY, l = 0.f;
  if (kb_begin < kb_end) {
    load(kb_begin);
    store(0);
  }
  __syncthreads();
  const int krow0 = 32 * (l15 >> 2) + (l15 & 3);
  for (int kb = kb_begin; kb < kb_end; ++kb) {
    const int bi = (kb - kb_begin) & 1;
    const bool more = kb + 1 < kb_end;
    if (more) load(kb + 1);
    const char* K = Kt(bi);
    f32x4 sc[8];
#pragma unroll
    for (int i = 0; i < 8; ++i) {
      sc[i] = f32x4{0.f, 0.f, 0.f, 0.f};
      const int kr = krow0 + 4 * i, sw = f8_kswz(kr);
#pragma unroll
      for (int k2 = 0; k2 < 2; ++k2) {
        const int c0 = 8 * k2 + 2 * g;
        const u32x4 lo = *reinterpret_cast<const u32x4*>(K + kr * 256 + ((c0 ^ sw) << 4));
        const u32x4 hi = *reinterpret_cast<const u32x4*>(K + kr * 256 + (((c0 + 1) ^ sw) << 4));
        sc[i] = __builtin_amdgcn_mfma_scale_f32_16x16x128_f8f6f4(f8_cat(lo, hi), qf[k2], sc[i], 0, 0, 0, 0, 0, 0);
      }
    }
    float mx = -INFINITY;
#pragma unroll
    for (int i = 0; i < 8; ++i) {
      const f32x4 skv = *reinterpret_cast<const f32x4*>(Sk(bi) + 32 * g + 4 * i);
#pragma unroll
      for (int e = 0; e < 4; ++e) {
        const int j = kb * F8_KB + 32 * g + 4 * i + e;
        const float x = fa_logit(mk, sc[i][e] * sq * skv[e], tq, j);
        sc[i][e] = x;
        mx = fmaxf(mx, x);
      }
    }
    mx = fmaxf(mx, __shfl_xor(mx, 16, 64));
    mx = fmaxf(mx, __shfl_xor(mx, 32, 64));
    const float mn = fmaxf(m, mx);
    const float alpha = mn == -INFINITY ? 1.f : __expf(m - mn);
    float sum = 0.f;
    unsigned pw[8];
#pragma unroll
    for (int i = 0; i < 8; ++i) {
      float pv[4];
#pragma unroll
      for (int e = 0; e < 4; ++e) {
        pv[e] = mn == -INFINITY ? 0.f : __expf(sc[i][e] - mn);
        sum += pv[e];
      }
      pw[i] = f8_enc4(pv[0] * 256.f, pv[1] * 256.f, pv[2] * 256.f, pv[3] * 256.f);
    }
    sum += __shfl_xor(sum, 16, 64);
    sum += __shfl_xor(sum, 32, 64);
    l = l * alpha + sum;
    m = mn;
#pragma unroll
    for (int db = 0; db < 16; ++db) o[db] *= alpha;
    const i32x8 pf = i32x8{(int)pw[0], (int)pw[1], (int)pw[2], (int)pw[3], (int)pw[4], (int)pw[5], (int)pw[6], (int)pw[7]};
    const char* V = Vt(bi);
#pragma unroll
    for (int db = 0; db < 16; ++db) {
      const int d = 16 * db + l15, sw = f8_vswz(d);
      const u32x4 lo = *reinterpret_cast<const u32x4*>(V + d * 128 + (((2 * g) ^ sw) << 4));
      const u32x4 hi = *reinterpret_cast<const u32x4*>(V + d * 128 + (((2 * g + 1) ^ sw) << 4));
      o[db] = __builtin_amdgcn_mfma_scale_f32_16x16x128_f8f6f4(f8_cat(lo, hi), pf, o[db], 0, 0, 0, 0, 0, 0);
    }
    __syncthreads();
    if (more) store(bi ^ 1);
    __syncthreads();
  }
  if (r >= a.nq) return;
  const float* svb = vs + b * 256;
  if (gridDim.z > 1) {
// ... 12 lines not shown
    }
    return;
  }
  const float inv = l > 0.f ? 1.f / (256.f * l) : 0.f;
  const FaRow fr{&a};
  const int gi = fr.grp(r);
  bf16_t* O = (bf16_t*)a.g_o[gi] + fr.off(b, 0, r, gi);
#pragma unroll
  for (int db = 0; db < 16; ++db) {
    const int d = 16 * db + 4 * g;
    const f32x4 sv4 = *reinterpret_cast<const f32x4*>(svb + d);
    const f32x4 v = o[db] * sv4 * inv;
    *reinterpret_cast<u32x2*>(O + d) = u32x2{pack2bf(v[0], v[1]), pack2bf(v[2], v[3])};
  }
  if (g == 0 && a.lse) a.lse[b * a.nq + r] = m + __logf(l);
}

}

#define FA_DISPATCH(HDV_, KERNEL, GRID, ...)                                                        \
  switch (HDV_) {                                                                                   \
    case 256: hipLaunchKernelGGL(KERNEL<256>, GRID, __VA_ARGS__); break;                            \
    case 72: hipLaunchKernelGGL(KERNEL<72>, GRID, __VA_ARGS__); break;                              \
    case 32: hipLaunchKernelGGL(KERNEL<32>, GRID, __VA_ARGS__); break;                              \
    default: hipLaunchKernelGGL(KERNEL<16>, GRID, __VA_ARGS__); break;                              \
  }
#define FA_T2(K, X) FaT2<X>::template K##_t
template <auto X>
struct FaT2 {
  template <int HD> static constexpr auto flash_bwd_q2_kernel_t = flash_bwd_q2_kernel<HD, (bool)X>;
  template <int HD> static constexpr auto flash_bwd_kv_kernel_t = flash_bwd_kv_kernel<HD, (int)X>;
};
static int fa_fast_bwd(const pz_flash_args* a) { return a->cap > 0.f ? 2 : 1; }
static bool fa_hd_ok(int64_t hd) { return hd == 256 || hd == 72 || hd == 32 || hd == 16; }

static bool fa_resident(const pz_flash_args* a) {
  const char* e = getenv("PZ_FLASH_RESIDENT");
  if (e && e[0] == '0') return false;
  return a->head_dim == 72 && a->nq <= FR_MAX && a->nk <= FR_MAX;
}

static bool fa_unit(const pz_flash_args* a) {
  const char* e = getenv("PZ_FLASH_UNIT");
  if (e && e[0] == '0') return false;
  if (e && e[0] == '1') return true;
  return a->Z * a->H >= 128;
}

static bool fa_plain(const pz_flash_args* a) { return a->mask_mode == 0 && a->cap == 0.f; }

static int fa_device_cus() {
  static int cache[64] = {0};
  int dev = 0;
  if (hipGetDevice(&dev) != hipSuccess || dev < 0 || dev >= 64) return 256;
  if (!cache[dev]) {
    int n = 0;
    if (hipDeviceGetAttribute(&n, hipDeviceAttributeMultiprocessorCount, dev) != hipSuccess || n <= 0) n = 256;
    cache[dev] = n;
  }
  return cache[dev];
}

static int fa_sig_grid(const pz_flash_args* a) { return (int)std::min<int64_t>(a->Z * a->H, fa_device_cus()); }

static bool fa_sig(const pz_flash_args* a) {
  const char* e = getenv("PZ_FLASH_SIG");
  if (e && e[0] == '0') return false;
  return fa_plain(a) && a->head_dim == 72 && a->nq == FS_N && a->nk == FS_N && a->n_groups == 1 &&
         a->o_hstride % 8 == 0 && a->g_ld[0] % 8 == 0 && a->g_bstride[0] % 8 == 0 &&
         a->ldq * FS_N < (1 << 30) && a->ldk * FS_N < (1 << 30) && a->ldv * FS_N < (1 << 30) &&
         a->g_ld[0] * FS_N < (1 << 30);
}

template <class Kern>
static void fa_smem_attr(Kern k, int bytes, bool& done) {
  if (!done) {
    if (hipFuncSetAttribute((const void*)k, hipFuncAttributeMaxDynamicSharedMemorySize, bytes) != hipSuccess)
      (void)hipGetLastError();
    done = true;
  }
}

extern "C" int pz_flash_fwd(const pz_flash_args* a, void* stream) {
  PZ_CHECK_ARG(a && a->q && a->k && a->v && a->Z > 0 && a->H > 0 && a->nq > 0 && a->nk > 0,
               "flash_fwd: bad args");
  PZ_CHECK_ARG(fa_hd_ok(a->head_dim), "flash_fwd: head_dim %lld unsupported (16, 32, 72, 256)",
               (long long)a->head_dim);
  PZ_CHECK_ARG(a->n_groups >= 1 && a->n_groups <= 3 && a->g_row0[0] == 0, "flash_fwd: output groups");
  for (int i = 0; i < a->n_groups; ++i) PZ_CHECK_ARG(a->g_o[i] && a->g_ld[i] % 4 == 0, "flash_fwd: group %d", i);
  PZ_CHECK_ARG(PZ_ALIGNED(a->q, 16) && PZ_ALIGNED(a->k, 16) && PZ_ALIGNED(a->v, 16) && a->ldq % 8 == 0 &&
                   a->ldk % 8 == 0 && a->ldv % 8 == 0 && a->q_hstride % 8 == 0 && a->k_hstride % 8 == 0 &&
                   a->v_hstride % 8 == 0 && a->q_bstride % 8 == 0 && a->k_bstride % 8 == 0 &&
                   a->v_bstride % 8 == 0 && a->o_hstride % 4 == 0,
               "flash_fwd: operands need 16-byte aligned rows");
  if (a->mask_mode == 1) PZ_CHECK_ARG(a->cnt && a->rows_per_token > 0, "flash_fwd: block mask needs cnt");
  PZ_CHECK_ARG(a->nq + a->mask_row0 < (1 << 22) && a->nk < (1 << 22) && a->mask_row0 >= 0, "flash_fwd: nq/nk too large");
  PZ_CHECK_ARG(a->Z * a->H < 65536, "flash_fwd: too many units");
  const int64_t qblk = (a->nq + 127) / 128, units = qblk * a->Z * a->H;
  const int64_t nkb = (a->nk + FA_KB - 1) / FA_KB;
  int64_t sp = 1;
  if (a->ws && units < 128 && nkb > 1 && a->head_dim % 4 == 0) {
    sp = (256 + units - 1) / units;
    sp = sp < nkb ? sp : nkb;
    sp = sp < 16 ? sp : 16;
    while (sp > 1 && sp * a->Z * a->H * a->nq * (a->head_dim + 2) * 4 > a->ws_bytes) --sp;
    const int64_t per = (nkb + sp - 1) / sp;
    sp = (nkb + per - 1) / per;
  }
  dim3 grid((unsigned)qblk, (unsigned)(a->Z * a->H), (unsigned)sp);
  hipStream_t st = (hipStream_t)stream;
  if (sp == 1 && fa_resident(a) && fa_unit(a)) {
    static bool attr = false;
    static bool attr2 = false;
    static bool attr3 = false;
    const dim3 gu((unsigned)(a->Z * a->H));
    if (fa_sig(a)) {
      const int G = fa_sig_grid(a);
      (void)attr3;
      {
        static bool attr4 = false;
        fa_smem_attr(flash_fwd_sig_kernel<1>, FS_SMEM, attr4);
        hipLaunchKernelGGL(flash_fwd_sig_kernel<1>, dim3((unsigned)G), dim3(16 * 64), FS_SMEM, st, *a, G);
      }
    } else if (fa_plain(a)) {
      fa_smem_attr(flash_fwd_unit_kernel<72, true>, FR_SMEM_KQ, attr);
      hipLaunchKernelGGL((flash_fwd_unit_kernel<72, true>), gu, dim3(FU_NW * 64), FR_SMEM_KQ, st, *a);
    } else {
      fa_smem_attr(flash_fwd_unit_kernel<72, false>, FR_SMEM_KQ, attr2);
      hipLaunchKernelGGL((flash_fwd_unit_kernel<72, false>), gu, dim3(FU_NW * 64), FR_SMEM_KQ, st, *a);
    }
    PZ_CHECK_LAUNCH();
    return PZ_OK;
  }
  if (sp == 1 && fa_resident(a)) {
    static bool attr = false;
    fa_smem_attr(flash_fwd_res_kernel<72>, FR_SMEM_KQ, attr);
    hipLaunchKernelGGL(flash_fwd_res_kernel<72>, dim3((unsigned)((a->nq + FR_NW * 16 - 1) / (FR_NW * 16) * a->Z * a->H)),
                       dim3(FR_NW * 64), FR_SMEM_KQ, st, *a);
    PZ_CHECK_LAUNCH();
    return PZ_OK;
  }
  FA_DISPATCH(a->head_dim, flash_fwd_kernel, grid, dim3((a->head_dim == 256 ? 8 : 4) * 64), 0, st, *a);
  PZ_CHECK_LAUNCH();
  if (sp > 1) {
    const int64_t n = a->Z * a->H * a->nq * (a->head_dim / 4);
    FA_DISPATCH(a->head_dim, flash_fwd_combine_kernel, dim3((unsigned)((n + 255) / 256)), dim3(256), 0, st, *a,
                (int)sp);
    PZ_CHECK_LAUNCH();
  }
  return PZ_OK;
}


extern "C" int pz_flash_fwd_probs(const pz_flash_args* a, void* P, void* tcap, int64_t ldp, void* stream) {
  PZ_CHECK_ARG(a && a->q && a->k && a->v && P && a->Z > 0 && a->H > 0 && a->nq > 0 && a->nk > 0,
               "flash_fwd_probs: bad args");
  PZ_CHECK_ARG(a->head_dim == 256, "flash_fwd_probs: head_dim %lld (256 only)", (long long)a->head_dim);
  PZ_CHECK_ARG(a->nk <= JP_MAXKB * FA_KB && ldp >= a->nk && ldp % 4 == 0, "flash_fwd_probs: nk %lld / ldp %lld",
               (long long)a->nk, (long long)ldp);
  PZ_CHECK_ARG(a->mask_mode == 0 || (a->mask_mode == 1 && a->cnt && a->rows_per_token > 0),
               "flash_fwd_probs: mask mode %d", a->mask_mode);
  PZ_CHECK_ARG(a->n_groups >= 1 && a->n_groups <= 3 && a->g_row0[0] == 0, "flash_fwd_probs: output groups");
  for (int i = 0; i < a->n_groups; ++i) PZ_CHECK_ARG(a->g_o[i] && a->g_ld[i] % 4 == 0, "flash_fwd_probs: group %d", i);
  PZ_CHECK_ARG(PZ_ALIGNED(a->q, 16) && PZ_ALIGNED(a->k, 16) && PZ_ALIGNED(a->v, 16) && PZ_ALIGNED(P, 8) &&
                   (!tcap || PZ_ALIGNED(tcap, 8)) && a->ldq % 8 == 0 && a->ldk % 8 == 0 && a->ldv % 8 == 0 &&
                   a->q_bstride % 8 == 0 && a->k_bstride % 8 == 0 && a->v_bstride % 8 == 0,
               "flash_fwd_probs: operands need 16-byte aligned rows");
  PZ_CHECK_ARG(a->nq + a->mask_row0 < (1 << 22) && a->Z * a->H < 65536, "flash_fwd_probs: nq / units too large");
  const int64_t units = a->Z * a->H, nqb = (a->nq + JP_NW * 16 - 1) / (JP_NW * 16);
  {
    static bool attr0 = false, attr1 = false;
    if (a->cap > 0.f) {
      fa_smem_attr(flash_fwd_probs_dma_kernel<true>, JD_SMEM, attr1);
      hipLaunchKernelGGL(flash_fwd_probs_dma_kernel<true>, dim3((unsigned)(nqb * units)), dim3(JP_NW * 64), JD_SMEM,
                         (hipStream_t)stream, *a, (bf16_t*)P, (bf16_t*)tcap, ldp);
    } else {
      fa_smem_attr(flash_fwd_probs_dma_kernel<false>, JD_SMEM, attr0);
      hipLaunchKernelGGL(flash_fwd_probs_dma_kernel<false>, dim3((unsigned)(nqb * units)), dim3(JP_NW * 64), JD_SMEM,
                         (hipStream_t)stream, *a, (bf16_t*)P, (bf16_t*)tcap, ldp);
    }
    PZ_CHECK_LAUNCH();
    return PZ_OK;
  }
}

extern "C" int pz_flash_bwd_ds(const pz_flash_args* a, const void* P, const void* tcap, void* dS, int64_t ldp,
                               void* stream) {
  PZ_CHECK_ARG(a && a->v && P && dS && a->Z > 0 && a->H > 0 && a->nq > 0 && a->nk > 0, "flash_bwd_ds: bad args");
  PZ_CHECK_ARG(a->head_dim == 256, "flash_bwd_ds: head_dim %lld (256 only)", (long long)a->head_dim);
  PZ_CHECK_ARG(a->nk <= JP_MAXKB * FA_KB && ldp >= a->nk && ldp % 4 == 0, "flash_bwd_ds: nk %lld / ldp %lld",
               (long long)a->nk, (long long)ldp);
  PZ_CHECK_ARG(a->cap <= 0.f || tcap, "flash_bwd_ds: soft-cap needs tcap");
  PZ_CHECK_ARG(a->n_groups >= 1 && a->n_groups <= 3 && a->g_row0[0] == 0, "flash_bwd_ds: output groups");
  for (int i = 0; i < a->n_groups; ++i) PZ_CHECK_ARG(!a->g_do[i] || a->g_ld[i] % 8 == 0, "flash_bwd_ds: dO group %d", i);
  PZ_CHECK_ARG(PZ_ALIGNED(a->v, 16) && a->ldv % 8 == 0 && a->v_bstride % 8 == 0 && PZ_ALIGNED(P, 8) &&
                   PZ_ALIGNED(dS, 8) && (!tcap || PZ_ALIGNED(tcap, 8)),
               "flash_bwd_ds: alignment");
  if (a->dq)
    PZ_CHECK_ARG(a->k && PZ_ALIGNED(a->k, 16) && a->ldk % 8 == 0 && a->k_bstride % 8 == 0 && PZ_ALIGNED(a->dq, 8) &&
                     a->ldq % 4 == 0 && a->q_bstride % 4 == 0,
                 "flash_bwd_ds: dQ needs K (16-byte rows) and an 8-byte aligned dQ");
  PZ_CHECK_ARG(a->Z * a->H < 65536, "flash_bwd_ds: too many units");
  const int64_t units = a->Z * a->H, nqb = (a->nq + JP_NW * 16 - 1) / (JP_NW * 16);
  static bool attr = false;
  fa_smem_attr(flash_bwd_ds_dma_kernel, JD_SMEM, attr);
  hipLaunchKernelGGL(flash_bwd_ds_dma_kernel, dim3((unsigned)(nqb * units)), dim3(JP_NW * 64), JD_SMEM,
                     (hipStream_t)stream, *a, (const bf16_t*)P, (const bf16_t*)tcap, (bf16_t*)dS, ldp);
  PZ_CHECK_LAUNCH();
  return PZ_OK;
}

extern "C" int pz_flash_bwd_prep(const pz_flash_args* a, void* stream) {
  PZ_CHECK_ARG(a && a->delta && a->n_groups >= 1 && a->n_groups <= 3, "flash_bwd_prep: bad args");
  for (int i = 0; i < a->n_groups; ++i) PZ_CHECK_ARG(a->g_o[i] && a->g_do[i], "flash_bwd_prep: group %d", i);
  const int64_t rows = a->Z * a->H * a->nq;
  PZ_CHECK_ARG(fa_hd_ok(a->head_dim), "flash_bwd_prep: head_dim");
  FA_DISPATCH(a->head_dim, flash_bwd_prep_kernel, dim3((unsigned)((rows + 3) / 4)), dim3(256), 0, (hipStream_t)stream,
              *a);
  PZ_CHECK_LAUNCH();
  return PZ_OK;
}

extern "C" int pz_flash_bwd(const pz_flash_args* a, void* stream) {
  PZ_CHECK_ARG(a && a->lse && a->delta && a->dq && a->dk && a->dv, "flash_bwd: bad args");
  PZ_CHECK_ARG(fa_hd_ok(a->head_dim), "flash_bwd: head_dim");
  PZ_CHECK_ARG(PZ_ALIGNED(a->dq, 16) && PZ_ALIGNED(a->dk, 16) && PZ_ALIGNED(a->dv, 16), "flash_bwd: alignment");
  for (int i = 0; i < a->n_groups; ++i) PZ_CHECK_ARG(a->g_do[i] && a->g_ld[i] % 8 == 0, "flash_bwd: dO group %d", i);
  hipStream_t st = (hipStream_t)stream;
  const int64_t nkb = (a->nk + FA_KB - 1) / FA_KB;
  int64_t splits = 1;
  if (a->ws && a->head_dim % 4 == 0) {
    splits = (1024 + nkb * a->Z * a->H - 1) / (nkb * a->Z * a->H);
    splits = splits < 8 ? splits : 8;
    while (splits > 1 && splits * 2 * a->Z * a->H * a->nk * a->head_dim * 4 > a->ws_bytes) --splits;
  }
  if (fa_resident(a) && fa_unit(a)) {
    static bool aq = false, akv = false, aq2 = false, akv2 = false, aq3 = false, akv3 = false;
    const dim3 gu((unsigned)(a->Z * a->H));
    if (fa_sig(a)) {
      const int G = fa_sig_grid(a);
      fa_smem_attr(flash_bwd_kv_sig_kernel, FS_SMEM, akv3);
      (void)aq3;
      {
        static bool aq4 = false;
        fa_smem_attr(flash_bwd_q_sig_kernel<true>, FS_SMEM, aq4);
        hipLaunchKernelGGL(flash_bwd_q_sig_kernel<true>, dim3((unsigned)G), dim3(FS_NW * 64), FS_SMEM, st, *a, G);
      }
      PZ_CHECK_LAUNCH();
      hipLaunchKernelGGL(flash_bwd_kv_sig_kernel, dim3((unsigned)G), dim3(FS_NW * 64), FS_SMEM, st, *a, G);
    } else if (fa_plain(a)) {
      fa_smem_attr(flash_bwd_q_unit_kernel<72, true>, FR_SMEM_KQ, aq);
      fa_smem_attr(flash_bwd_kv_unit_kernel<72, true>, FU_SMEM_KV, akv);
      hipLaunchKernelGGL((flash_bwd_q_unit_kernel<72, true>), gu, dim3(FU_NW * 64), FR_SMEM_KQ, st, *a);
      PZ_CHECK_LAUNCH();
      hipLaunchKernelGGL((flash_bwd_kv_unit_kernel<72, true>), gu, dim3(FU_NW * 64), FU_SMEM_KV, st, *a);
    } else {
      fa_smem_attr(flash_bwd_q_unit_kernel<72, false>, FR_SMEM_KQ, aq2);
      fa_smem_attr(flash_bwd_kv_unit_kernel<72, false>, FU_SMEM_KV, akv2);
      hipLaunchKernelGGL((flash_bwd_q_unit_kernel<72, false>), gu, dim3(FU_NW * 64), FR_SMEM_KQ, st, *a);
      PZ_CHECK_LAUNCH();
      hipLaunchKernelGGL((flash_bwd_kv_unit_kernel<72, false>), gu, dim3(FU_NW * 64), FU_SMEM_KV, st, *a);
    }
    PZ_CHECK_LAUNCH();
    return PZ_OK;
  }
  if (fa_resident(a)) {
    static bool aq = false, akv = false;
    fa_smem_attr(flash_bwd_q_res_kernel<72>, FR_SMEM_KQ, aq);
    fa_smem_attr(flash_bwd_kv_res_kernel<72>, FR_SMEM_KV, akv);
    hipLaunchKernelGGL(flash_bwd_q_res_kernel<72>, dim3((unsigned)((a->nq + FR_NW * 16 - 1) / (FR_NW * 16) * a->Z * a->H)),
                       dim3(FR_NW * 64), FR_SMEM_KQ, st, *a);
    PZ_CHECK_LAUNCH();
    hipLaunchKernelGGL(flash_bwd_kv_res_kernel<72>, dim3((unsigned)(nkb * a->Z * a->H)), dim3(FR_NW * 64),
                       FR_SMEM_KV, st, *a);
    PZ_CHECK_LAUNCH();
    return PZ_OK;
  }
  const int fm = fa_fast_bwd(a);
  {
    const int64_t units = a->Z * a->H, nqb = (a->nq + JQ_NW * 32 - 1) / (JQ_NW * 32);
    const dim3 gq2((unsigned)(nqb * units));
    if (fm == 2) {
      FA_DISPATCH(a->head_dim, FA_T2(flash_bwd_q2_kernel, true), gq2, dim3(JQ_NW * 64), 0, st, *a);
    } else {
      FA_DISPATCH(a->head_dim, FA_T2(flash_bwd_q2_kernel, false), gq2, dim3(JQ_NW * 64), 0, st, *a);
    }
  }
  PZ_CHECK_LAUNCH();
  const dim3 gkv1((unsigned)(nkb * a->Z * a->H * splits));
  if (fm == 2) {
    FA_DISPATCH(a->head_dim, FA_T2(flash_bwd_kv_kernel, 2), gkv1, dim3(FA_NW * 64), 0, st, *a, (int)splits);
  } else {
    FA_DISPATCH(a->head_dim, FA_T2(flash_bwd_kv_kernel, 1), gkv1, dim3(FA_NW * 64), 0, st, *a, (int)splits);
  }
  if (splits > 1) {
    PZ_CHECK_LAUNCH();
    const int64_t n4 = 2 * a->Z * a->H * a->nk * (a->head_dim / 4);
    FA_DISPATCH(a->head_dim, flash_bwd_kv_reduce_kernel, dim3((unsigned)((n4 + 255) / 256)), dim3(256), 0, st, *a,
                (int)splits);
  }
  PZ_CHECK_LAUNCH();
  return PZ_OK;
}

extern "C" int pz_flash_fwd_f8(const pz_flash_args* a, const void* qc, const float* qs, const void* kc, const float* ks,
                               int64_t krows, const void* vtc, const float* vs, int64_t ldvt, void* stream) {
  PZ_CHECK_ARG(a && qc && qs && kc && ks && vtc && vs && a->Z > 0 && a->nq > 0 && a->nk > 0 && a->H == 1,
               "flash_fwd_f8: bad args (one K / V head: H == 1)");
  PZ_CHECK_ARG(a->head_dim == 256, "flash_fwd_f8: head_dim %lld (256 only)", (long long)a->head_dim);
  PZ_CHECK_ARG(krows >= a->nk && ldvt >= (a->nk + F8_KB - 1) / F8_KB * F8_KB && ldvt % 16 == 0,
               "flash_fwd_f8: krows %lld / ldvt %lld (ldvt >= nk rounded up to 128)", (long long)krows,
               (long long)ldvt);
  PZ_CHECK_ARG(PZ_ALIGNED(qc, 16) && PZ_ALIGNED(kc, 16) && PZ_ALIGNED(vtc, 16) && PZ_ALIGNED(vs, 16),
               "flash_fwd_f8: 16-byte aligned codes / scales");
  PZ_CHECK_ARG(a->n_groups >= 1 && a->n_groups <= 3 && a->g_row0[0] == 0 && a->o_hstride == 0, "flash_fwd_f8: groups");
  for (int i = 0; i < a->n_groups; ++i) PZ_CHECK_ARG(a->g_o[i] && a->g_ld[i] % 4 == 0, "flash_fwd_f8: group %d", i);
  PZ_CHECK_ARG(a->mask_mode == 0 || (a->mask_mode == 1 && a->cnt && a->rows_per_token > 0), "flash_fwd_f8: mask");
  PZ_CHECK_ARG(a->nq + a->mask_row0 < (1 << 22) && a->Z < 65536, "flash_fwd_f8: nq / Z too large");
  const int64_t qblk = (a->nq + 127) / 128, nkb = (a->nk + F8_KB - 1) / F8_KB;
  int64_t sp = 1;
  if (a->ws && qblk * a->Z < 128 && nkb > 1) {
    sp = (256 + qblk * a->Z - 1) / (qblk * a->Z);
    sp = sp < nkb ? sp : nkb;
    sp = sp < 16 ? sp : 16;
    while (sp > 1 && sp * a->Z * a->nq * (256 + 2) * 4 > a->ws_bytes) --sp;
    const int64_t per = (nkb + sp - 1) / sp;
    sp = (nkb + per - 1) / per;
  }
  static bool attr = false;
  fa_smem_attr(flash_fwd_f8_kernel, F8_SMEM, attr);
  hipStream_t st = (hipStream_t)stream;
  hipLaunchKernelGGL(flash_fwd_f8_kernel, dim3((unsigned)qblk, (unsigned)a->Z, (unsigned)sp), dim3(512), F8_SMEM, st, *a,
                     (const uint8_t*)qc, qs, (const uint8_t*)kc, ks, krows, (const uint8_t*)vtc, vs, ldvt);
  PZ_CHECK_LAUNCH();
  if (sp > 1) {
    const int64_t n = a->Z * a->nq * 64;
    hipLaunchKernelGGL(flash_fwd_combine_kernel<256>, dim3((unsigned)((n + 255) / 256)), dim3(256), 0, st, *a, (int)sp);
    PZ_CHECK_LAUNCH();
  }
  return PZ_OK;
}
```

### open-pi-zero_amd/pizero_native/_lib.py

```python

from __future__ import annotations

import ctypes as C
import os

_HERE = os.path.dirname(os.path.dirname(os.path.abspath(__file__)))
LIB_PATH = os.path.join(_HERE, "libpizero_hip.so")
if os.environ.get("PZ_LIB_PATH"):
    LIB_PATH = os.path.join(_HERE, os.path.basename(os.environ["PZ_LIB_PATH"]))
    import sys as _sys

    print(f"[pizero_native] PZ_LIB_PATH override: loading {LIB_PATH} instead of the default libpizero_hip.so",
          file=_sys.stderr, flush=True)

ABI_VERSION = 22
PZ_EPI_NONE, PZ_EPI_GELU, PZ_EPI_GEGLU, PZ_EPI_SILU = 0, 1, 2, 3
PZ_EPI_DGELU, PZ_EPI_DSILU, PZ_EPI_DGEGLU = 4, 5, 6
PZ_SUMSQ_PARTS = 2048
PZ_OBS_MAX_TAPS, PZ_OBS_MAX_EXTENT = 64, 16384
PZ_OBS_NORM_BOUND, PZ_OBS_NORM_GAUSSIAN = 0, 1
PZ_AUG_CROP, PZ_AUG_BRIGHTNESS, PZ_AUG_CONTRAST, PZ_AUG_SATURATION, PZ_AUG_HUE, PZ_AUG_ALL = 1, 2, 4, 8, 16, 31

i64, i32, f32, vp = C.c_int64, C.c_int32, C.c_float, C.c_void_p
fp = C.POINTER(C.c_float)


class GemmArgs(C.Structure):
    _fields_ = [
        ("M", i64), ("N", i64), ("K", i64),
        ("A", vp), ("lda", i64), ("a_kcontig", i32),
        ("B", vp), ("ldb", i64), ("b_kcontig", i32),
        ("C", vp), ("ldc", i64), ("c_fp32", i32),
        ("batch", i64), ("batch_inner", i64),
        ("sA_outer", i64), ("sA_inner", i64), ("sB_outer", i64), ("sB_inner", i64),
        ("sC_outer", i64), ("sC_inner", i64), ("sR_outer", i64), ("sR_inner", i64),
        ("epilogue", i32), ("alpha", f32), ("beta_accum", i32),
        ("bias", vp), ("resid", vp), ("ld_resid", i64), ("aux", vp), ("ld_aux", i64),
        ("geglu_inter", i64),
        ("workspace", vp), ("ws_bytes", i64),
        ("norm_w", vp), ("norm_eps", f32),
        ("fp8_mode", i32), ("a_row_scale", vp),
        ("A2", vp), ("lda2", i64), ("B2", vp), ("ldb2", i64), ("K2", i64),
    ]


class SmallGemmArgs(C.Structure):
    _fields_ = [
        ("M", i64), ("N", i64), ("K", i64),
        ("A", vp), ("sAm", i64), ("sAk", i64),
        ("B", vp), ("sBk", i64), ("sBn", i64),
        ("C", vp), ("ldc", i64), ("bias", vp), ("alpha", f32), ("beta", i32),
    ]


class SoftmaxArgs(C.Structure):
    _fields_ = [
        ("S", vp), ("lds", i64), ("P", vp), ("ldp", i64), ("tcap", vp),
        ("R", i64), ("N", i64), ("scale", f32), ("cap", f32), ("mask_mode", i32),
        ("rows_per_batch", i64), ("heads", i64), ("qoff", i64),
        ("cnt", vp), ("prefix", i64), ("cond", i64),
        ("mask", vp), ("ldm", i64), ("mask_bstride", i64),
    ]


class FlashArgs(C.Structure):
    _fields_ = [
        ("Z", i64), ("H", i64), ("nq", i64), ("nk", i64), ("head_dim", i64),
        ("q", vp), ("ldq", i64), ("q_bstride", i64), ("q_hstride", i64),
        ("k", vp), ("ldk", i64), ("k_bstride", i64), ("k_hstride", i64),
        ("v", vp), ("ldv", i64), ("v_bstride", i64), ("v_hstride", i64),
        ("n_groups", i32),
        ("g_row0", i64 * 3), ("g_o", vp * 3), ("g_bstride", i64 * 3), ("g_ld", i64 * 3),
        ("o_hstride", i64),
        ("lse", vp),
        ("scale", f32), ("cap", f32),
        ("mask_mode", i32),
        ("cnt", vp), ("prefix", i64), ("cond", i64), ("rows_per_token", i64),
        ("g_do", vp * 3),
        ("delta", vp),
        ("dq", vp), ("dk", vp), ("dv", vp),
        ("ws", vp), ("ws_bytes", i64),
        ("mask_row0", i64),
    ]


class AdamW8Args(C.Structure):
    _fields_ = [
        ("p", vp), ("g", vp), ("s1", vp), ("s2", vp), ("absmax1", vp), ("absmax2", vp),
        ("m32", vp), ("v32", vp), ("seg", vp), ("nseg", i64), ("nblocks", i64),
        ("qmap1", vp), ("qmap2", vp),
        ("beta1", f32), ("beta2", f32), ("omb1", f32), ("omb2", f32), ("step", f32), ("epsc", f32),
        ("decay", f32), ("gscale", vp),
    ]


class QkvRopeArgs(C.Structure):
    _fields_ = [
        ("x", vp), ("ldx", i64), ("W", vp), ("ldw", i64), ("M", i64), ("N", i64), ("K", i64),
        ("norm_w", vp), ("norm_eps", f32), ("pos", vp), ("cs", vp), ("q_out", vp), ("k_out", vp), ("v_out", vp),
        ("T", i64), ("nh", i64), ("hd", i64), ("Lq", i64), ("qoff", i64), ("Lk", i64), ("koff", i64),
        ("w_fp8", i32), ("w_scale", f32),
        ("x2", vp), ("ldx2", i64), ("W2", vp), ("ldw2", i64), ("K2", i64),
    ]


class ReduceSeg(C.Structure):
    _fields_ = [("part", vp), ("P", i64), ("D", i64), ("out", vp), ("beta", i32)]


class DecodeAttnArgs(C.Structure):
    _fields_ = [
        ("q", vp), ("ldq", i64), ("Lq", i64), ("qoff", i64), ("k", vp), ("v", vp), ("k_bstride", i64),
        ("v_bstride", i64), ("o", vp), ("ldo", i64), ("B", i64), ("nh", i64), ("T", i64), ("nk", i64),
        ("head_dim", i64), ("scale", f32), ("cap", f32), ("cnt", vp), ("prefix", i64), ("cond", i64),
        ("qtok0", i64), ("ws", vp), ("ws_bytes", i64),
    ]


SIGNATURES = {
    "pz_gemm": [C.POINTER(GemmArgs), vp],
    "pz_fp8_quant_rows": [vp, i64, vp, i64, vp, i64, i64, vp],
    "pz_fp8_quant_tensor": [vp, i64, vp, f32, vp],
    "pz_fp8_quant_vt": [vp, i64, i64, i64, i64, vp, vp, i64, vp],
    "pz_rmsnorm_fwd_f8": [vp, i64, vp, vp, i64, vp, i64, i64, f32, vp],
    "pz_layernorm_fwd_f8": [vp, i64, vp, vp, vp, i64, vp, i64, i64, f32, vp],
    "pz_fp8_quant_attn": [vp, i64, vp, i64, vp, i64, i64, i64, i64, vp, vp, vp, vp, vp, vp, i64, vp],
    "pz_flash_fwd_f8": [C.POINTER(FlashArgs), vp, vp, vp, vp, i64, vp, vp, i64, vp],
    "pz_fp8_absmax": [vp, i64, vp, vp],
    "pz_gemm_kernel_name": [C.POINTER(GemmArgs)],
    "pz_gemm_small": [C.POINTER(SmallGemmArgs), vp],
    "pz_rmsnorm_fwd": [vp, i64, vp, vp, i64, vp, i64, i64, f32, vp],
    "pz_rmsnorm_bwd": [vp, i64, vp, i64, vp, vp, vp, vp, i64, vp, i64, i64, vp],
    "pz_layernorm_fwd": [vp, i64, vp, vp, vp, i64, vp, vp, i64, i64, f32, vp],
    "pz_layernorm_bwd": [vp, i64, vp, i64, vp, vp, vp, vp, vp, i64, vp, vp, i64, i64, vp, vp],
    "pz_act_bwd_colsum": [vp, i64, vp, i64, vp, i64, i64, i32, vp, i64, vp, i32, vp],
    "pz_reduce_parts_multi": [vp, i32, vp],
    "pz_norm_rows_per_part": [],
    "pz_reduce_parts": [vp, i64, i64, vp, i32, vp],
    "pz_colsum": [vp, i64, i64, i64, vp, i32, vp, vp],
    "pz_batch_sum": [vp, i64, i64, i64, vp, i32, vp],
    "pz_rope_table": [vp, i64, i64, f32, vp],
    "pz_qkv_rope_split": [vp, vp, vp, vp, vp, vp, i64, i64, i64, i64, i64, i64, i64, i64, i64, vp],
    "pz_qkv_rope_split_bwd": [vp, vp, vp, vp, vp, vp, i64, i64, i64, i64, i64, i64, i64, i64, i64, vp],
    "pz_gemv_qkv_rope": [C.POINTER(QkvRopeArgs), vp],
    "pz_gemm_qkv_rope": [C.POINTER(QkvRopeArgs), vp],
    "pz_decode_attn": [C.POINTER(DecodeAttnArgs), vp],
    "pz_decode_attn_ws_bytes": [i64, i64, i64],
    "pz_attn_softmax": [C.POINTER(SoftmaxArgs), vp],
    "pz_attn_softmax_bwd": [vp, vp, i64, vp, vp, i64, i64, i64, f32, f32, vp],
    "pz_flash_fwd": [C.POINTER(FlashArgs), vp],
    "pz_flash_fwd_probs": [C.POINTER(FlashArgs), vp, vp, i64, vp],
    "pz_flash_bwd_ds": [C.POINTER(FlashArgs), vp, vp, vp, i64, vp],
    "pz_flash_bwd_prep": [C.POINTER(FlashArgs), vp],
    "pz_flash_bwd": [C.POINTER(FlashArgs), vp],
    "pz_patchify": [vp, vp, i64, i64, i64, i64, i64, vp],
    "pz_embed_merge": [vp, vp, i64, vp, vp, i64, i64, i64, i64, i64, i64, f32, f32, vp],
    "pz_embed_merge_bwd": [vp, vp, vp, i64, i64, i64, i64, i64, f32, vp],
    "pz_time_embed": [vp, vp, i64, i64, f32, i32, vp],
    "pz_concat_time": [vp, vp, vp, i64, i64, i64, vp],
    "pz_split_time_grad": [vp, vp, i64, i64, vp],
    "pz_flow_psi": [vp, vp, vp, vp, i64, i64, f32, vp],
    "pz_flow_loss": [vp, i64, i64, vp, vp, vp, vp, vp, i64, i64, i64, f32, vp],
    "pz_euler_step": [vp, vp, i64, i64, vp, i64, i64, i64, f32, vp],
    "pz_action_in": [vp, i64, vp, vp, vp, vp, i64, i64, i64, i64, f32, i32, vp],
    "pz_action_out": [vp, i64, vp, f32, vp, vp, i64, i64, vp, vp, i64, i64, f32, vp],
    "pz_copy_rows": [vp, i64, i64, vp, i64, i64, i64, i64, i64, f32, i32, vp],
    "pz_time_embed_rows": [vp, vp, i64, i64, i64, i64, f32, i32, vp],
    "pz_clamp": [vp, i64, f32, f32, vp],
    "pz_geglu_bwd": [vp, i64, vp, i64, vp, vp, i64, i64, i64, vp],
    "pz_act_bwd": [vp, i64, vp, i64, vp, vp, i64, i64, i64, i32, vp],
    "pz_adamw": [vp, vp, vp, vp, i64, f32, f32, f32, f32, f32, f32, f32, vp, vp],
    "pz_adamw8bit": [C.POINTER(AdamW8Args), vp],
    "pz_adamw8bit_r": [C.POINTER(AdamW8Args), vp, i32, C.c_uint64, i64, vp],
    "pz_adamw_r": [vp, vp, vp, vp, vp, i64, f32, f32, f32, f32, f32, f32, f32, vp, i32, C.c_uint64, i64, vp],
    "pz_sumsq": [vp, i64, vp, vp],
    "pz_clip_coef": [vp, i64, vp, vp, f32, vp],
    "pz_fill_uniform": [vp, i32, i64, C.c_uint64, f32, f32, vp],
    "pz_cast_f32_bf16": [vp, vp, i64, vp],
    "pz_cast_bf16_f32": [vp, vp, i64, vp],
    "pz_adaln_fwd": [vp, i64, vp, i64, vp, vp, vp, i64, vp, vp, vp, vp, i64, vp, i64, i64, i64, i64, f32, vp],
    "pz_adaln_norm_bwd": [vp, i64, vp, i64, vp, vp, vp, vp, vp, i64, vp, vp, i64, i64, i64, i64, vp],
    "pz_adaln_gate_bwd": [vp, i64, vp, i64, vp, vp, vp, i64, vp, i64, i64, i64, i64, vp],
    "pz_lora_wgrad_ws_bytes": [i64, i64, i64],
    "pz_lora_wgrad": [vp, i64, vp, i64, vp, i64, i64, i64, i64, i32, f32, i32, vp, i64, vp],
    "pz_avg_lerp": [vp, vp, i64, f32, vp],
    "pz_avg_swap": [vp, vp, i64, vp],
    "pz_image_resize_scratch_bytes": [i64, i64, i64],
    "pz_image_resize_norm": [vp, i32, i64, i64, i64, i64, vp, vp, vp, i64, vp, vp, vp, i64, vp, vp, i64, vp, vp],
    "pz_proprio_normalize": [vp, vp, i64, i64, vp, vp, i32, vp],
    "pz_action_denormalize": [vp, vp, i64, i64, i64, vp, vp, i32, vp],
    "pz_image_augment_scratch_bytes": [i64, i64],
    "pz_image_augment": [vp, i32, i64, i64, vp, vp, i32, vp, vp, i64, vp, vp],
    "pz_image_resize_u8": [vp, i32, i64, i64, i64, i64, vp, vp, vp, i64, vp, vp, vp, i64, vp, i64, vp, vp],
    "pz_debug_poison_lds": [C.c_uint32, vp],
    "pz_debug_spin": [i64, i64, vp],
    "pz_last_error": [],
    "pz_abi_version": [],
}
_RESTYPE = {"pz_last_error": C.c_char_p, "pz_gemm_kernel_name": C.c_char_p, "pz_norm_rows_per_part": i64,
            "pz_decode_attn_ws_bytes": i64, "pz_lora_wgrad_ws_bytes": i64, "pz_image_resize_scratch_bytes": i64,
            "pz_image_augment_scratch_bytes": i64}

_lib = None


class NativeError(RuntimeError):
    pass


def lib():
    global _lib
    if _lib is None:
        if not os.path.exists(LIB_PATH):
            raise NativeError(
                f"{LIB_PATH} not found: build it with `python open-pi-zero_amd/build_native.py` "
                "(or __graft_entry__.build()); the Pi0 path has no CPU/eager fallback")
        L = C.CDLL(LIB_PATH)
        for name, argt in SIGNATURES.items():
            fn = getattr(L, name)
            fn.argtypes = argt
            fn.restype = _RESTYPE.get(name, C.c_int)
        if L.pz_abi_version() != ABI_VERSION:
            raise NativeError(f"{LIB_PATH}: ABI version {L.pz_abi_version()} != {ABI_VERSION}; rebuild it")
        _lib = L
    return _lib


_NO_LAUNCH = {"pz_last_error", "pz_abi_version", "pz_gemm_kernel_name", "pz_norm_rows_per_part",
              "pz_decode_attn_ws_bytes", "pz_lora_wgrad_ws_bytes", "pz_debug_poison_lds",
              "pz_image_resize_scratch_bytes", "pz_image_augment_scratch_bytes"}
_POISON_LDS = [0xFFFFFFFF if os.environ.get("PZ_POISON_LDS", "0") == "1" else None]


_RECENT = [[] if os.environ.get("PZ_CHECK_FINITE", "0") == "1" else None]


def recent_launches(clear=True):
    r = _RECENT[0] or []
    if clear and _RECENT[0] is not None:
        _RECENT[0] = []
    return r


def set_poison_lds(word):
    _POISON_LDS[0] = None if word is None else int(word) & 0xFFFFFFFF


def call(name, *args):
    if _POISON_LDS[0] is not None and name not in _NO_LAUNCH:
        rc = lib().pz_debug_poison_lds(_POISON_LDS[0], args[-1])
        if rc != 0:
            raise NativeError(f"pz_debug_poison_lds failed (rc={rc}): {lib().pz_last_error().decode(errors='replace')}")
    if _RECENT[0] is not None:
        _RECENT[0].append(name)
    rc = getattr(lib(), name)(*args)
    if rc != 0:
        msg = lib().pz_last_error().decode(errors="replace")
        raise NativeError(f"{name} failed (rc={rc}): {msg}")
    return rc
```

### open-pi-zero_amd/pizero_native/engine.py

```python

from __future__ import annotations

import contextlib
import functools
import math
import os
import weakref
from dataclasses import dataclass

import torch

from . import ops
from .ops import PZ_EPI_DGEGLU, PZ_EPI_GEGLU, PZ_EPI_GELU, PZ_EPI_NONE, PZ_EPI_SILU

BF16 = torch.bfloat16
F32 = torch.float32


def _cfg(cfg, key, default=None):
    from src.utils.config import cfg_get

    return cfg_get(cfg, key, default)


# ... 905 lines not shown
        s_dn = self.lora(p + "mlp.down_proj.weight")
        lo_o = s_o.fwd(O) if s_o is not None else None
        ops.linear(O, self.w(p + "self_attn.o_proj.weight"), xm, resid=x, lora=lo_o)
        h2 = torch.empty_like(x)
        r2 = torch.empty(M, device=dev, dtype=F32)
        ops.rmsnorm(xm, self.w(p + "post_attention_layernorm.weight"), h2, r2, d.rms_eps)
        gu = torch.empty(M, 2 * g.inter, device=dev, dtype=BF16)
        hm = torch.empty(M, g.inter, device=dev, dtype=BF16)
        lo_gu = s_gu.fwd(h2) if s_gu is not None else None
        ops.linear(h2, self.gu_w(p), hm, epi=PZ_EPI_GEGLU, aux=gu, lora=lo_gu)
        xn = torch.empty_like(x)
        lo_dn = s_dn.fwd(hm) if s_dn is not None else None
        ops.linear(hm, self.w(p + "mlp.down_proj.weight"), xn, resid=xm, lora=lo_dn)
        gs.update(O=O, xm=xm, h2=h2, r2=r2, gu=gu, hm=hm, skip=False, u_o=lo_o[0] if lo_o else None,
                  u_gu=lo_gu[0] if lo_gu else None, u_dn=lo_dn[0] if lo_dn else None)
        X[g.name] = xn

    def _joint_layers_train(self, groups, X, pos, cnt, B, save):
        d = self.d
        dev = X[groups[0].name].device
        L, Lp, nh, hd = d.L, d.Lp, d.nh, d.hd
        S = None
        layers = []
        Kall, Vall = self._joint_kv(B, Lp, dev, save)
        ada = save.get("ada")
        main = torch.cuda.current_stream(dev)
        side = None
        if self.expert_stream and self.expert_stream_fwd and len(groups) > 1 and dev.type == "cuda":
            side = self._side_stream(dev)
            side.wait_stream(main)
            for t in X.values():
                if t is not None:
                    t.record_stream(side)
            for A in (ada or {}).values():
                A.mod.record_stream(side)
        for l in range(d.nL):
            last = l == d.nL - 1
            Qj = torch.empty(B, L, nh * hd, device=dev, dtype=BF16)
            if side is not None:
                Qj.record_stream(side)
            Kj, Vj = Kall[l], Vall[l]
            st = {"Q": Qj, "K": Kj, "V": Vj, "g": {}}
            for g in groups:
                with self._on(side, g):
                    self._pre_attn_train(g, l, X, pos, st, Qj, Kj, Vj, dev, ada)
            if side is not None:
                main.wait_stream(side)
            Os = {g.name: torch.empty(B * g.T, nh * hd, device=dev, dtype=BF16) for g in groups}
            if self.joint_flash and not isinstance(cnt, GeneralMask):
                lse = torch.empty(B, L * nh, device=dev, dtype=F32)
                ops.flash_fwd(self._joint_flash(groups, Qj, Kj, Vj, Os, lse, cnt, B, L))
                st["lse"], st["O"] = lse, Os
            elif self.joint_probs and not isinstance(cnt, GeneralMask) and L <= 320 and hd == 256:
                Pm = torch.empty(B, L * nh, Lp, device=dev, dtype=BF16)
                tc = torch.empty(B, L * nh, Lp, device=dev, dtype=BF16)
                ops.flash_fwd_probs(self._joint_flash(groups, Qj, Kj, Vj, Os, None, cnt, B, L), Pm, tc, Lp)
                st["P"], st["tc"], st["O"] = Pm, tc, Os
            else:
                if S is None:
                    S = torch.empty(B, L * nh, Lp, device=dev, dtype=F32)
                ops.gemm(L * nh, L, hd, Qj, hd, True, Kj, hd, True, S, Lp, batch=B, sA=(L * nh * hd, 0),
                         sB=(Lp * hd, 0), sC=(L * nh * Lp, 0))
                Pm = torch.empty(B, L * nh, Lp, device=dev, dtype=BF16)
                tc = torch.empty(B, L * nh, Lp, device=dev, dtype=BF16)
                ops.attn_softmax(S, Lp, Pm, Lp, B * L * nh, L, 1.0 / math.sqrt(hd), cap=50.0, tcap=tc,
                                 rows_per_batch=L * nh, heads=nh, qoff=0, **_mask_kw(d, cnt, "full"))
                st["P"], st["tc"] = Pm, tc
                for g in groups:
                    if not (last and g.skip_last):
                        ops.gemm(g.T * nh, hd, Lp, Pm[:, g.off * nh:], Lp, True, Vj, hd, False, Os[g.name], hd, batch=B,
                                 sA=(L * nh * Lp, 0), sB=(Lp * hd, 0), sC=(g.T * nh * hd, 0))
                st["O"] = Os
            if side is not None:
                side.wait_stream(main)
                for t in Os.values():
                    t.record_stream(side)
            for g in groups:
                gs = st["g"][g.name]
                if last and g.skip_last:
                    X[g.name] = None
                    gs["skip"] = True
                    continue
                with self._on(side, g):
                    if ada and g.name in ada:
                        self._post_attn_ada(ada[g.name], g, l, X, gs, Os, dev)
                    else:
                        self._post_attn_train(g, l, X, gs, Os, dev)
            layers.append(st)
            self._chk(f"joint fwd layer {l}", Q=Qj, K=Kj, V=Vj, O=Os, P=st.get("P"), tc=st.get("tc"), X=X)
        if side is not None:
            main.wait_stream(side)
            for t in X.values():
                if t is not None:
                    t.record_stream(main)
            for st in layers:
                for g in groups:
                    if g.name != "vlm":
                        for t in st["g"][g.name].values():
                            if isinstance(t, torch.Tensor):
                                t.record_stream(main)
        save["joint"] = layers
        return X

    def _mlp_oproj_backward(self, g, gs, p, dX, dO, dXm, beta, rpp, nh, hd, dev, A=None, l=None):
        dx = dres = dX[g.name]
        M = dx.shape[0]
        part = None if A is not None else torch.empty((M + rpp - 1) // rpp, g.hid, device=dev, dtype=F32)
        if A is not None and A.zero:
            dx = ops.adaln_gate_bwd(dres, gs["yd"], A.mod, A.biased(l, "final_z"), torch.empty_like(dres), A.dmod, g.T)
            gs["yd"] = None
        gu = gs["gu"]
        s_o = self.lora(p + "self_attn.o_proj.weight")
        s_gu = self.lora(p + "mlp.gate_proj.weight", p + "mlp.up_proj.weight")
        s_dn = self.lora(p + "mlp.down_proj.weight")
        lo = None
        if s_dn is not None:
            lo = s_dn.bwd(dx)
            s_dn.grads(gs["hm"], gs["u_dn"], dx, lo[0], beta)
        ops.linear_dgrad(dx, self.w(p + "mlp.down_proj.weight"), gu, epi=PZ_EPI_DGEGLU, aux=gu, lora=lo)
        if self.rg(p + "mlp.down_proj.weight"):
            ops.linear_wgrad(dx, gs["hm"], self.gw(p + "mlp.down_proj.weight"), beta=beta)
        gs["hm"] = None
        if self.rg(p + "mlp.gate_proj.weight") and self.rg(p + "mlp.up_proj.weight"):
            ops.linear_wgrad(gu, gs["h2"], self.ar.grad_span(p + "mlp.gate_proj.weight", p + "mlp.up_proj.weight"),
                             beta=beta)
        dh2 = torch.empty(M, g.hid, device=dev, dtype=BF16)
        lo = None
        if s_gu is not None:
            lo = s_gu.bwd(gu)
            s_gu.grads(gs["h2"], gs["u_gu"], gu, lo[0], beta)
        ops.linear_dgrad(gu, self.gu_w(p), dh2, lora=lo)
        dxm = torch.empty_like(dx)
        if A is not None:
            A.norm_bwd(dh2, gs["xm"], gs["r2"], l, "post_", g.T, dxm, dres=dres)
        else:
            ops.rmsnorm_bwd(dh2, gs["xm"], self.w(p + "post_attention_layernorm.weight"), gs["r2"], dxm, dres=dx,
                            dw_part=part)
            self._norm_grads(p + "post_attention_layernorm.", part, None, beta)
        dyo = dxm
        if A is not None and A.zero:
            dyo = ops.adaln_gate_bwd(dxm, gs["yo"], A.mod, A.biased(l, "post_z"), torch.empty_like(dxm), A.dmod, g.T)
            gs["yo"] = None
        if self.rg(p + "self_attn.o_proj.weight"):
            ops.linear_wgrad(dyo, gs["O"], self.gw(p + "self_attn.o_proj.weight"), beta=beta)
        o = torch.empty(M, nh * hd, device=dev, dtype=BF16)
        lo = None
        if s_o is not None:
            lo = s_o.bwd(dyo)
            s_o.grads(gs["O"], gs["u_o"], dyo, lo[0], beta)
        ops.linear_dgrad(dyo, self.w(p + "self_attn.o_proj.weight"), o, lora=lo)
        dO[g.name] = o
        dXm[g.name] = dxm

    def _qkv_backward(self, g, gs, p, dQ, dK, dV, dX, dXm, pos, B, L, Lp, beta, rpp, nh, hd, dev, A=None, l=None):
        x = gs["x"]
        M = x.shape[0]
        W = (nh + 2) * hd
        dqkv = torch.empty(M, W, device=dev, dtype=BF16)
        ops.qkv_rope_split_bwd(None if gs.get("skip") else dQ, dK, dV, pos[g.pos_key], self.rope(g.theta), dqkv,
                               B, g.T, nh, 1, hd, L, g.off, Lp, g.off)
        names = [p + f"self_attn.{k}_proj.weight" for k in "qkv"]
        rgs = [self.rg(n) for n in names]
        site = self.lora(*names)
        lo = None
        if site is not None:
            lo = site.bwd(dqkv)
            site.grads(gs["h"], gs["u_qkv"], dqkv, lo[0], beta)
        if gs.get("skip") and site is None:
            if rgs[0] and not beta:
                self.gw(names[0]).zero_()
            for n, rgk, c0, c1 in zip(names[1:], rgs[1:], (nh * hd, (nh + 1) * hd), ((nh + 1) * hd, W)):
                if rgk:
                    ops.linear_wgrad(dqkv[:, c0:c1], gs["h"], self.gw(n), beta=beta)
            dh = torch.empty(M, g.hid, device=dev, dtype=BF16)
            ops.linear_dgrad(dqkv[:, nh * hd:], self.span(names[1], names[2]), dh)
        else:
            if all(rgs):
                ops.linear_wgrad(dqkv, gs["h"], self.ar.grad_span(names[0], names[2]), beta=beta)
            elif rgs[0] and rgs[1]:
                ops.linear_wgrad(dqkv[:, : (nh + 1) * hd], gs["h"], self.ar.grad_span(names[0], names[1]),
                                 beta=beta)
            else:
                for n, rgk, c0, c1 in zip(names, rgs, (0, nh * hd, (nh + 1) * hd), (nh * hd, (nh + 1) * hd, W)):
                    if rgk:
                        ops.linear_wgrad(dqkv[:, c0:c1], gs["h"], self.gw(n), beta=beta)
            dh = torch.empty(M, g.hid, device=dev, dtype=BF16)
            ops.linear_dgrad(dqkv, self.qkv_w(p), dh, lora=lo)
        dxn = torch.empty(M, g.hid, device=dev, dtype=BF16)
        if A is not None:
            A.norm_bwd(dh, x, gs["r"], l, "in_", g.T, dxn, dres=dXm.get(g.name))
        else:
            part = torch.empty((M + rpp - 1) // rpp, g.hid, device=dev, dtype=F32)
            ops.rmsnorm_bwd(dh, x, self.w(p + "input_layernorm.weight"), gs["r"], dxn, dres=dXm.get(g.name),
                            dw_part=part)
            self._norm_grads(p + "input_layernorm.", part, None, beta)
        dX[g.name] = dxn

    def _joint_layers_backward(self, groups, dX, pos, cnt, B, sv, beta):
        d = self.d
        L, Lp, nh, hd = d.L, d.Lp, d.nh, d.hd
        dev = next(v for v in dX.values() if v is not None).device
        delta = dP = dS = None
        rpp = ops.rows_per_part()
        main = torch.cuda.current_stream(dev)
        side = None
        if self.expert_stream and len(groups) > 1 and dev.type == "cuda":
            side = self._side_stream(dev)
            side.wait_stream(main)
            for st in sv["joint"]:
                for g in groups:
                    if g.name != "vlm":
                        for t in st["g"][g.name].values():
                            if isinstance(t, torch.Tensor):
                                t.record_stream(side)
            for t in dX.values():
                if t is not None:
                    t.record_stream(side)
            for A in (sv.get("ada") or {}).values():
                A.mod.record_stream(side)
                A.dmod.record_stream(side)
        ada = sv.get("ada") or {}
        for l in reversed(range(d.nL)):
            st = sv["joint"][l]
            dQ = torch.empty(B, L, nh * hd, device=dev, dtype=BF16)
            dK = torch.empty(B, Lp, hd, device=dev, dtype=BF16)
            dV = torch.empty(B, Lp, hd, device=dev, dtype=BF16)
            dO = {}
            dXm = {}
            any_skip = False
            for g in groups:
                gs = st["g"][g.name]
                p = f"{g.prefix}{l}."
                if gs.get("skip"):
                    any_skip = True
                    continue
                with self._on(side, g):
                    self._mlp_oproj_backward(g, gs, p, dX, dO, dXm, beta, rpp, nh, hd, dev, ada.get(g.name), l)
                if side is not None and g.name != "vlm":
                    dO[g.name].record_stream(main)
            if side is not None:
                main.wait_stream(side)
            if "lse" in st:
                for g in groups:
                    if g.name not in dO:
                        dO[g.name] = torch.zeros(B * g.T, nh * hd, device=dev, dtype=BF16)
                if delta is None:
                    delta = torch.empty(B, L * nh, device=dev, dtype=F32)
                ops.flash_bwd(self._joint_flash(groups, st["Q"], st["K"], st["V"], st["O"], st["lse"], cnt, B, L,
                                                dO=dO, delta=delta, dq=dQ, dk=dK, dv=dV))
            else:
                Pm, tc, Qj, Kj, Vj = st["P"], st["tc"], st["Q"], st["K"], st["V"]
                dq_done = False
                if not isinstance(cnt, GeneralMask) and L <= 320 and hd == 256:
                    if dS is None:
                        dS = torch.empty(B, L * nh, Lp, device=dev, dtype=BF16)
                    ops.flash_bwd_ds(self._joint_flash(groups, Qj, Kj, Vj, st["O"], None, cnt, B, L, dO=dO,
                                                       dq=dQ), Pm, tc, dS, Lp)
                    dq_done = True
                else:
                    if dP is None:
                        dP = torch.empty(B, L * nh, Lp, device=dev, dtype=F32)
                    if dS is None:
                        dS = torch.empty(B, L * nh, Lp, device=dev, dtype=BF16)
                    if any_skip:
                        dP.zero_()
                    for g in groups:
                        if g.name not in dO:
                            continue
                        ops.gemm(g.T * nh, L, hd, dO[g.name], hd, True, Vj, hd, True, dP[:, g.off * nh:], Lp,
                                 batch=B, sA=(g.T * nh * hd, 0), sB=(Lp * hd, 0), sC=(L * nh * Lp, 0))
                    ops.attn_softmax_bwd(Pm, dP, Lp, tc, dS, Lp, B * L * nh, L, 1.0 / math.sqrt(hd), 50.0)
                if not dq_done:
                    ops.gemm(L * nh, hd, Lp, dS, Lp, True, Kj, hd, False, dQ, hd, batch=B, sA=(L * nh * Lp, 0),
                             sB=(Lp * hd, 0), sC=(L * nh * hd, 0))
                ops.gemm(Lp, hd, L * nh, dS, Lp, False, Qj, hd, False, dK, hd, batch=B, sA=(L * nh * Lp, 0),
                         sB=(L * nh * hd, 0), sC=(Lp * hd, 0))
                first = True
                for g in sorted(groups, key=lambda g: g.T):
                    if g.name not in dO:
                        continue
                    ops.gemm(Lp, hd, g.T * nh, Pm[:, g.off * nh:], Lp, False, dO[g.name], hd, False, dV, hd, batch=B,
                             sA=(L * nh * Lp, 0), sB=(g.T * nh * hd, 0), sC=(Lp * hd, 0), beta=not first)
                    first = False
                if first:
                    dV.zero_()
            if side is not None:
                side.wait_stream(main)
                for t in (dQ, dK, dV):
                    t.record_stream(side)
            for g in groups:
                with self._on(side, g):
                    self._qkv_backward(g, st["g"][g.name], f"{g.prefix}{l}.", dQ, dK, dV, dX, dXm, pos, B, L, Lp, beta,
                                       rpp, nh, hd, dev, ada.get(g.name), l)
            self._chk(f"joint bwd layer {l}", dO=dO, dS=dS, dQ=dQ, dK=dK, dV=dV, dX=dX)
            self._notify("joint", l, (side,) if side is not None else ())
        if side is not None:
            main.wait_stream(side)
            for t in dX.values():
                if t is not None:
                    t.record_stream(main)
        sv.pop("_jkv_token", None)
        return dX

    def train_forward(self, ids, pix, cnt, pos, proprios, actions, t, x0, save):
        d = self.d
        dev = pix.device
        B = ids.shape[0]
        tied = self.m._tied
        sv_v = {}
        img = self.siglip_forward(pix, sv_v)
        Xv = self.embed_prefix(ids, img)
        prop = proprios.reshape(B * d.C, d.Pd).to(BF16)
        pe = torch.empty(B * d.C, d.aH, device=dev, dtype=BF16)
        ops.small_linear(prop, self.w("proprio_encoder.weight"), pe, bias=self.w("proprio_encoder.bias"))
        psi = torch.empty(B * d.H, d.A, device=dev, dtype=BF16)
        ops.flow_psi(x0, actions, t, psi, d.sig_min)
        e3 = self.action_embed(psi, t, save)
        sa = math.sqrt(d.aH)
        if tied:
            Xe = torch.empty(B * (d.C + d.H), d.aH, device=dev, dtype=BF16)
            T = d.C + d.H
            ops.copy_rows(pe, d.aH, d.C * d.aH, Xe, d.aH, T * d.aH, B, d.C, d.aH, scale=sa)
            ops.copy_rows(e3, d.aH, d.H * d.aH, Xe[d.C:], d.aH, T * d.aH, B, d.H, d.aH, scale=sa)
            X = {"vlm": Xv, "expert": Xe}
        else:
            Xp = torch.empty(B * d.C, d.aH, device=dev, dtype=BF16)
            Xa = torch.empty(B * d.H, d.aH, device=dev, dtype=BF16)
            ops.copy_rows(pe, d.aH, 0, Xp, d.aH, 0, 1, B * d.C, d.aH, scale=sa)
            ops.copy_rows(e3, d.aH, 0, Xa, d.aH, 0, 1, B * d.H, d.aH, scale=sa)
            X = {"vlm": Xv, "proprio": Xp, "action": Xa}
        groups = self.groups(tied)
        if d.ada:
            cond = torch.empty(B, d.tH, device=dev, dtype=BF16)
            ops.time_embed(t, cond, d.tmax, ref_bf16=d.time_bf16)
            save["cond"] = cond
            save["ada"] = {g.name: Ada(self, g, cond) for g in groups if g.name != "vlm"}
        X = self._joint_layers_train(groups, X, pos, cnt, B, save)
        ag = "expert" if tied else "action"
        aoff = d.C if tied else 0
        Tg = d.C + d.H if tied else d.H
        Xl = X[ag]
        ya = torch.empty_like(Xl)
        ra = torch.empty(Xl.shape[0], device=dev, dtype=F32)
        if d.ada:
            save["ada"][ag].norm_fwd(Xl, "norm", "", Tg, ya, ra)
        else:
            ops.rmsnorm(Xl, self.w("joint_model.mixtures.action.norm.weight"), ya, ra, d.rms_eps)
        v = torch.empty(B * Tg, 8, device=dev, dtype=BF16)
        ops.small_linear(ya, self.w("action_decoder.weight"), v, bias=self.w("action_decoder.bias"))
        loss = torch.empty(1, device=dev, dtype=F32)
        ops.flow_loss(v[aoff:], 8, Tg * 8, x0, actions, loss, None, None, B, d.H, d.A, d.sig_min)
        save.update(sv_v=sv_v, ids=ids, cnt=cnt, pos=pos, B=B, prop=prop, pe=pe, tied=tied, Xl=Xl, ya=ya, ra=ra,
                    x0=x0, x1=actions, v=v, ag=ag, aoff=aoff, Tg=Tg, groups=groups)
        self._chk("train fwd head (action norm, decoder, flow loss)", embed=Xv, ya=ya, v=v, loss=loss)
        return loss

    def train_backward(self, sv, grad_loss, beta):
        d = self.d
        B = sv["B"]
        dev = sv["v"].device
        Tg, aoff = sv["Tg"], sv["aoff"]
        ws = self.colsum_ws(2 * d.aH)
        rpp = ops.rows_per_part()
        dv = torch.zeros(B * Tg, 8, device=dev, dtype=BF16)
        tmp = torch.empty(1, device=dev, dtype=F32)
        ops.flow_loss(sv["v"][aoff:], 8, Tg * 8, sv["x0"], sv["x1"], tmp, dv[aoff:], grad_loss, B, d.H, d.A, d.sig_min)
        R = B * Tg
        if self.rg("action_decoder.weight"):
            ops.small_gemm(d.A, d.aH, R, dv, 1, 8, sv["ya"], d.aH, 1, self.gw("action_decoder.weight"), d.aH, beta=beta)
        if self.rg("action_decoder.bias"):
            ops.colsum(dv[:, : d.A], self.gw("action_decoder.bias"), ws, beta=beta)
        dya = torch.empty(R, d.aH, device=dev, dtype=BF16)
        ops.small_gemm(R, d.aH, d.A, dv, 8, 1, self.w("action_decoder.weight"), d.aH, 1, dya, d.aH)
        dXl = torch.empty_like(dya)
        ada = sv.get("ada")
        if ada:
            for A in ada.values():
                A.dmod = torch.zeros_like(A.mod)
            ada[sv["ag"]].norm_bwd(dya, sv["Xl"], sv["ra"], "norm", "", Tg, dXl)
        else:
            part = torch.empty((R + rpp - 1) // rpp, d.aH, device=dev, dtype=F32)
            ops.rmsnorm_bwd(dya, sv["Xl"], self.w("joint_model.mixtures.action.norm.weight"), sv["ra"], dXl,
                            dw_part=part)
            self._norm_grads("joint_model.mixtures.action.norm.", part, None, beta)
        self._chk("train bwd head", dv=dv, dya=dya, dXl=dXl)
        groups = sv["groups"]
        dX = {g.name: None for g in groups}
        dX[sv["ag"]] = dXl
        dX = self._joint_layers_backward(groups, dX, sv["pos"], sv["cnt"], B, sv, beta)
        if ada:
            for A in ada.values():
                A.weight_grads(sv["cond"], self.colsum_ws(A.mod.shape[1]), beta)
        sa = math.sqrt(d.aH)
        dpe = torch.empty(B * d.C, d.aH, device=dev, dtype=BF16)
        de3 = torch.empty(B * d.H, d.aH, device=dev, dtype=BF16)
        if sv["tied"]:
            T = d.C + d.H
            ops.copy_rows(dX["expert"], d.aH, T * d.aH, dpe, d.aH, d.C * d.aH, B, d.C, d.aH, scale=sa)
            ops.copy_rows(dX["expert"][d.C:], d.aH, T * d.aH, de3, d.aH, d.H * d.aH, B, d.H, d.aH, scale=sa)
        else:
            ops.copy_rows(dX["proprio"], d.aH, 0, dpe, d.aH, 0, 1, B * d.C, d.aH, scale=sa)
            ops.copy_rows(dX["action"], d.aH, 0, de3, d.aH, 0, 1, B * d.H, d.aH, scale=sa)
        if self.rg("proprio_encoder.weight"):
            ops.small_gemm(d.aH, d.Pd, B * d.C, dpe, 1, d.aH, sv["prop"], d.Pd, 1, self.gw("proprio_encoder.weight"),
                           d.Pd, beta=beta)
        if self.rg("proprio_encoder.bias"):
            ops.colsum(dpe, self.gw("proprio_encoder.bias"), ws, beta=beta)
        ae = "action_encoder."
        if self.rg(ae + "linear_3.weight"):
            ops.linear_wgrad(de3, sv["ae_e2"], self.gw(ae + "linear_3.weight"), beta=beta)
        if self.rg(ae + "linear_3.bias"):
            ops.colsum(de3, self.gw(ae + "linear_3.bias"), ws, beta=beta)
        de2 = torch.empty_like(de3)
        ops.linear_dgrad(de3, self.w(ae + "linear_3.weight"), de2)
        ops.act_bwd(de2, sv["ae_pre"], de2, None, PZ_EPI_SILU)
        if self.rg(ae + "linear_2.weight"):
            ops.linear_wgrad(de2, sv["ae_cat"], self.gw(ae + "linear_2.weight"), beta=beta)
        if self.rg(ae + "linear_2.bias"):
            ops.colsum(de2, self.gw(ae + "linear_2.bias"), ws, beta=beta)
        if d.ada:
            de1 = torch.empty_like(de3)
            ops.linear_dgrad(de2, self.w(ae + "linear_2.weight"), de1)
        else:
            dcat = torch.empty(B * d.H, 2 * d.aH, device=dev, dtype=BF16)
            ops.linear_dgrad(de2, self.w(ae + "linear_2.weight"), dcat)
            de1 = torch.empty_like(de3)
            ops.split_time_grad(dcat, de1, B * d.H, d.aH)
        if self.rg(ae + "linear_1.weight"):
            ops.small_gemm(d.aH, d.A, B * d.H, de1, 1, d.aH, sv["ae_psi"], d.A, 1, self.gw(ae + "linear_1.weight"), d.A,
                           beta=beta)
        if self.rg(ae + "linear_1.bias"):
            ops.colsum(de1, self.gw(ae + "linear_1.bias"), ws, beta=beta)
        self._notify("encoders", -1)
        if self.m._vlm_needs_grad():
            dimg = torch.empty(B * d.n_img, d.gH, device=dev, dtype=BF16)
            ops.embed_merge_bwd(sv["ids"], dX["vlm"], dimg, d.n_img, d.image_token, 1.0)
            self._chk("train bwd embed-merge", dimg=dimg)
            self.siglip_backward(sv["sv_v"], dimg, beta)
        self._chk("train bwd end (gradient arena)", grad=self.ar.grad)
        if self.post_backward is not None:
            self.post_backward()

    def joint_train(self, embeds, pos, cnt, dout, beta=False):
        d = self.d
        Ev, Ep, Ea = embeds["vlm"], embeds["proprio"], embeds["action"]
        B = Ev.shape[0]
        dev = Ev.device
# ... 448 lines not shown
```

### open-pi-zero_amd/pizero_native/ops.py

```python

from __future__ import annotations

import ctypes as C

import torch

from ._lib import (
    PZ_EPI_DGEGLU,
    PZ_EPI_DGELU,
    PZ_EPI_DSILU,
    PZ_EPI_GEGLU,
    PZ_EPI_GELU,
    PZ_EPI_NONE,
    PZ_EPI_SILU,
    PZ_OBS_MAX_EXTENT,
    PZ_OBS_MAX_TAPS,
    PZ_OBS_NORM_BOUND,
    PZ_OBS_NORM_GAUSSIAN,
    PZ_SUMSQ_PARTS,
    AdamW8Args,
    QkvRopeArgs,
    DecodeAttnArgs,
    FlashArgs,
    GemmArgs,
    SmallGemmArgs,
    NativeError,
    SoftmaxArgs,
    call,
    lib,
)

__all__ = ["PZ_EPI_NONE", "PZ_EPI_GELU", "PZ_EPI_GEGLU", "PZ_EPI_SILU", "PZ_EPI_DGELU", "PZ_EPI_DSILU", "PZ_EPI_DGEGLU"]

BF16 = torch.bfloat16


def _st():
    return C.c_void_p(torch.cuda.current_stream().cuda_stream)


def _p(t):
    return None if t is None else t.data_ptr()


_PROBE = None


def set_probe(pred):
    global _PROBE
    _PROBE = None if pred is None else (pred, [])
    return None if _PROBE is None else _PROBE[1]


def gemm(M, N, K, A, lda, a_kc, B, ldb, b_kc, Cm, ldc, *, epi=PZ_EPI_NONE, alpha=1.0, beta=False,
         bias=None, resid=None, ld_resid=0, aux=None, ld_aux=0, geglu_inter=0, batch=1, batch_inner=1,
         sA=(0, 0), sB=(0, 0), sC=(0, 0), sR=(0, 0), norm=None, ext=None):
    if _PROBE is not None and _PROBE[0](M, N, K, epi, batch):
        e0, e1 = torch.cuda.Event(enable_timing=True), torch.cuda.Event(enable_timing=True)
        e0.record()
        _gemm(M, N, K, A, lda, a_kc, B, ldb, b_kc, Cm, ldc, epi, alpha, beta, bias, resid, ld_resid, aux, ld_aux,
              geglu_inter, batch, batch_inner, sA, sB, sC, sR, norm, ext)
        e1.record()
        _PROBE[1].append((e0, e1))
        return
    _gemm(M, N, K, A, lda, a_kc, B, ldb, b_kc, Cm, ldc, epi, alpha, beta, bias, resid, ld_resid, aux, ld_aux,
          geglu_inter, batch, batch_inner, sA, sB, sC, sR, norm, ext)


_WS_BYTES = 160 << 20
_WS = {}


_WS_SLOT = [0]


class workspace_slot:

    def __init__(self, slot):
        self.slot, self.prev = slot, None

    def __enter__(self):
        self.prev = _WS_SLOT[0]
        _WS_SLOT[0] = self.slot

    def __exit__(self, *exc):
        _WS_SLOT[0] = self.prev


def workspace(device=None):
    dev = torch.device("cuda", torch.cuda.current_device()) if device is None else torch.device(device)
    key = (dev, _WS_SLOT[0])
    ws = _WS.get(key)
    if ws is None:
        ws = torch.empty(_WS_BYTES // 4, dtype=torch.float32, device=dev)
        _WS[key] = ws
    return ws


def _args(M, N, K, A, lda, a_kc, B, ldb, b_kc, Cm, ldc, epi, alpha, beta, bias, resid, ld_resid, aux, ld_aux,
          geglu_inter, batch, batch_inner, sA, sB, sC, sR, ws=None, norm=None):
    a = GemmArgs()
    a.M, a.N, a.K = int(M), int(N), int(K)
    a.A, a.lda, a.a_kcontig = _p(A), int(lda), int(bool(a_kc))
    a.B, a.ldb, a.b_kcontig = _p(B), int(ldb), int(bool(b_kc))
    a.C, a.ldc, a.c_fp32 = _p(Cm), int(ldc), int(Cm.dtype == torch.float32)
    a.batch, a.batch_inner = int(batch), int(batch_inner)
    a.sA_outer, a.sA_inner = int(sA[0]), int(sA[1])
    a.sB_outer, a.sB_inner = int(sB[0]), int(sB[1])
    a.sC_outer, a.sC_inner = int(sC[0]), int(sC[1])
    a.sR_outer, a.sR_inner = int(sR[0]), int(sR[1])
    a.epilogue, a.alpha, a.beta_accum = int(epi), float(alpha), int(bool(beta))
    a.bias, a.resid, a.ld_resid = _p(bias), _p(resid), int(ld_resid)
    a.aux, a.ld_aux, a.geglu_inter = _p(aux), int(ld_aux), int(geglu_inter)
    if ws is not None:
        a.workspace, a.ws_bytes = ws.data_ptr(), ws.numel() * ws.element_size()
    if norm is not None:
        a.norm_w, a.norm_eps = _p(norm[0]), float(norm[1])
    return a


def _gemm(M, N, K, A, lda, a_kc, B, ldb, b_kc, Cm, ldc, epi, alpha, beta, bias, resid, ld_resid, aux, ld_aux,
          geglu_inter, batch, batch_inner, sA, sB, sC, sR, norm=None, ext=None):
    ws = workspace(Cm.device) if batch == 1 else None
    a = _args(M, N, K, A, lda, a_kc, B, ldb, b_kc, Cm, ldc, epi, alpha, beta, bias, resid, ld_resid, aux, ld_aux,
              geglu_inter, batch, batch_inner, sA, sB, sC, sR, ws, norm)
    if ext is not None:
        a.A2, a.lda2, a.B2, a.ldb2, a.K2 = _p(ext[0]), int(ext[1]), _p(ext[2]), int(ext[3]), int(ext[4])
    call("pz_gemm", C.byref(a), _st())


def gemm_kernel_name(M, N, K, *, a_kc=True, b_kc=True, epi=PZ_EPI_NONE, geglu_inter=0, batch=1, c_fp32=False,
                     workspace_bytes=_WS_BYTES, fp8_mode=0, K2=0):
    a = GemmArgs()
    a.M, a.N, a.K = int(M), int(N), int(K)
    a.a_kcontig, a.b_kcontig, a.c_fp32 = int(a_kc), int(b_kc), int(c_fp32)
    a.batch, a.batch_inner, a.epilogue, a.geglu_inter = int(batch), 1, int(epi), int(geglu_inter)
    a.workspace, a.ws_bytes = (256 if workspace_bytes else None), int(workspace_bytes)
    a.fp8_mode = int(fp8_mode)
    a.K2 = int(K2)
    if fp8_mode == 1:
        a.a_row_scale, a.lda, a.ldb = 256, int(K), int(K)
    return lib().pz_gemm_kernel_name(C.byref(a)).decode()


def linear(x, W, out, *, bias=None, resid=None, epi=PZ_EPI_NONE, aux=None, alpha=1.0, beta=False, norm=None,
           lora=None):
    M, K = x.shape
    N = W.shape[0]
    ext = None if lora is None else (lora[0], lora[0].stride(0), lora[1], lora[1].stride(0), lora[0].shape[1])
    if epi == PZ_EPI_GEGLU:
        I = N // 2
        gemm(M, N, K, x, x.stride(0), True, W, W.stride(0), True, out, out.stride(0), epi=epi,
             aux=aux, ld_aux=0 if aux is None else aux.stride(0), geglu_inter=I, alpha=alpha, norm=norm, ext=ext)
        return out
    gemm(M, N, K, x, x.stride(0), True, W, W.stride(0), True, out, out.stride(0), epi=epi, alpha=alpha,
         beta=beta, bias=bias, resid=resid, ld_resid=0 if resid is None else resid.stride(0), aux=aux,
         ld_aux=0 if aux is None else aux.stride(0), norm=norm, ext=ext)
    return out


def lora_wgrad_ws_bytes(M, D, R):
    return int(lib().pz_lora_wgrad_ws_bytes(int(M), int(D), int(R)))


def lora_wgrad(Q, P, out, *, transposed=False, alpha=1.0, beta=False, ws=None):
    M, D = Q.shape
    R = P.shape[1]
    ws = workspace(Q.device) if ws is None else ws
    call("pz_lora_wgrad", _p(Q), Q.stride(0), _p(P), P.stride(0), _p(out), out.stride(0), M, D, R, int(transposed),
         float(alpha), int(bool(beta)), _p(ws), ws.numel() * ws.element_size(), _st())
    return out


ABSMAX_PARTS = 1024
E4M3_MAX = 448.0

# ... 67 lines not shown
        if M % (s * 64) == 0:
            best = s
            if tiles * s >= 240:
                break
    return best


def linear_wgrad(dy, x, dW, *, beta=False):
    M, N = dy.shape
    K = x.shape[1]
    S = _split_k(M, N, K) if dW.is_contiguous() else 1
    if S == 1:
        gemm(N, K, M, dy, dy.stride(0), False, x, x.stride(0), False, dW, dW.stride(0), beta=beta)
        return dW
    Mc = M // S
    slabs = torch.empty(S, N, K, device=dW.device, dtype=torch.float32)
    gemm(N, K, Mc, dy, dy.stride(0), False, x, x.stride(0), False, slabs, K, batch=S,
         sA=(Mc * dy.stride(0), 0), sB=(Mc * x.stride(0), 0), sC=(N * K, 0))
    reduce_parts(slabs.view(S, N * K), dW.view(-1), beta=beta)
    return dW


def small_linear(x, W, out, *, bias=None, beta=False):
    M, K = x.shape
    N = W.shape[0]
    a = SmallGemmArgs()
    a.M, a.N, a.K = M, N, K
    a.A, a.sAm, a.sAk = _p(x), x.stride(0), x.stride(1)
    a.B, a.sBk, a.sBn = _p(W), W.stride(1), W.stride(0)
    a.C, a.ldc, a.bias, a.alpha, a.beta = _p(out), out.stride(0), _p(bias), 1.0, int(beta)
    call("pz_gemm_small", C.byref(a), _st())
    return out


def small_gemm(M, N, K, A, sAm, sAk, B, sBk, sBn, out, ldc, *, beta=False, bias=None):
    a = SmallGemmArgs()
    a.M, a.N, a.K = M, N, K
    a.A, a.sAm, a.sAk = _p(A), sAm, sAk
    a.B, a.sBk, a.sBn = _p(B), sBk, sBn
    a.C, a.ldc, a.bias, a.alpha, a.beta = _p(out), ldc, _p(bias), 1.0, int(beta)
    call("pz_gemm_small", C.byref(a), _st())
    return out


def rmsnorm(x, w, y, rstd, eps):
    R, D = x.shape
    call("pz_rmsnorm_fwd", _p(x), x.stride(0), _p(w), _p(y), y.stride(0), _p(rstd), R, D, float(eps), _st())
    return y


def rmsnorm_bwd(dy, x, w, rstd, dx, dres=None, dw_part=None):
    R, D = x.shape
    call("pz_rmsnorm_bwd", _p(dy), dy.stride(0), _p(x), x.stride(0), _p(w), _p(rstd), _p(dres), _p(dx),
         dx.stride(0), _p(dw_part), R, D, _st())
    return dx


def layernorm(x, w, b, y, mean, rstd, eps):
    R, D = x.shape
    call("pz_layernorm_fwd", _p(x), x.stride(0), _p(w), _p(b), _p(y), y.stride(0), _p(mean), _p(rstd), R, D,
         float(eps), _st())
    return y


def layernorm_bwd(dy, x, w, mean, rstd, dx, dres=None, dw_part=None, db_part=None, dx_part=None):
    R, D = x.shape
    call("pz_layernorm_bwd", _p(dy), dy.stride(0), _p(x), x.stride(0), _p(w), _p(mean), _p(rstd), _p(dres),
         _p(dx), dx.stride(0), _p(dw_part), _p(db_part), R, D, _p(dx_part), _st())
    return dx


def adaln_fwd(x, mod, rows_per_sample, eps, *, y=None, gate=None, xm=None, gamma=None, beta=None, h=None, rstd=None):
    R, D = x.shape
    gp = gb = gmp = gmb = bp = None
    if y is not None:
        gp, gb = mod[:, gate[0]:].data_ptr(), _p(gate[1])
    if h is not None:
        gmp, gmb, bp = mod[:, gamma[0]:].data_ptr(), _p(gamma[1]), mod[:, beta:].data_ptr()
    call("pz_adaln_fwd", _p(x), x.stride(0), _p(y), 0 if y is None else y.stride(0), gp, gb, _p(xm),
         0 if xm is None else xm.stride(0), gmp, gmb, bp, _p(h), 0 if h is None else h.stride(0), _p(rstd),
         mod.stride(0), R, D, int(rows_per_sample), float(eps), _st())


def adaln_norm_bwd(dh, x, rstd, mod, gamma, dx, dmod, beta, rows_per_sample, dres=None):
    R, D = x.shape
    call("pz_adaln_norm_bwd", _p(dh), dh.stride(0), _p(x), x.stride(0), _p(rstd), mod[:, gamma[0]:].data_ptr(),
         _p(gamma[1]), _p(dres), _p(dx), dx.stride(0), None if dmod is None else dmod[:, gamma[0]:].data_ptr(),
         None if dmod is None else dmod[:, beta:].data_ptr(), mod.stride(0), R, D, int(rows_per_sample), _st())
    return dx


def adaln_gate_bwd(dout, y, mod, gate, dy, dmod, rows_per_sample):
    R, D = y.shape
    call("pz_adaln_gate_bwd", _p(dout), dout.stride(0), _p(y), y.stride(0), mod[:, gate[0]:].data_ptr(), _p(gate[1]),
         _p(dy), dy.stride(0), dmod[:, gate[0]:].data_ptr(), mod.stride(0), R, D, int(rows_per_sample), _st())
    return dy


def act_bwd_colsum(dh, pre, dpre, act, ws, dbias, beta=False):
    M, N = pre.shape
    call("pz_act_bwd_colsum", _p(dh), dh.stride(0), _p(pre), pre.stride(0), _p(dpre), M, N, int(act), _p(ws),
         ws.numel() // N, _p(dbias), int(beta), _st())
    return dpre


_RPP = None


def rows_per_part():
    global _RPP
    if _RPP is None:
        from ._lib import lib

        _RPP = int(lib().pz_norm_rows_per_part())
    return _RPP


def reduce_parts(part, out, beta=False):
    P, D = part.shape
    call("pz_reduce_parts", _p(part), P, D, _p(out), int(beta), _st())
    return out


def reduce_parts_multi(items, beta=False):
    from ._lib import ReduceSeg

    if not items:
        return
    segs = (ReduceSeg * len(items))()
    for s, (part, out) in zip(segs, items):
        s.part, s.P, s.D, s.out, s.beta = _p(part), part.shape[0], part.shape[1], _p(out), int(beta)
    call("pz_reduce_parts_multi", C.cast(segs, C.c_void_p), len(items), _st())


def colsum(X, out, ws, beta=False):
    M, N = X.shape
    call("pz_colsum", _p(X), X.stride(0), M, N, _p(out), int(beta), _p(ws), _st())
    return out


def batch_sum(X, B, stride, n, out, beta=False):
    call("pz_batch_sum", _p(X), B, stride, n, _p(out), int(beta), _st())
    return out


def rope_table(cs, max_pos, head_dim, theta):
    call("pz_rope_table", _p(cs), max_pos, head_dim, float(theta), _st())
    return cs


def qkv_rope_split(qkv, pos, cs, q_out, k_out, v_out, B, T, nh, nkv, hd, Lq, qoff, Lk, koff):
    call("pz_qkv_rope_split", _p(qkv), _p(pos), _p(cs), _p(q_out), _p(k_out), _p(v_out), B, T, nh, nkv, hd,
         Lq, qoff, Lk, koff, _st())


def qkv_rope_split_bwd(dq, dk, dv, pos, cs, dqkv, B, T, nh, nkv, hd, Lq, qoff, Lk, koff):
    call("pz_qkv_rope_split_bwd", _p(dq), _p(dk), _p(dv), _p(pos), _p(cs), _p(dqkv), B, T, nh, nkv, hd, Lq,
         qoff, Lk, koff, _st())


def gemv_qkv_rope(x, W, pos, cs, q_out, k_out, v_out, T, nh, hd, Lq, qoff, Lk, koff, norm=None):
    a = QkvRopeArgs()
    a.x, a.ldx = _p(x), x.stride(0)
    a.W, a.ldw = _p(W), W.stride(0)
    a.M, a.N, a.K = x.shape[0], W.shape[0], x.shape[1]
    if norm is not None:
        a.norm_w, a.norm_eps = _p(norm[0]), float(norm[1])
    a.pos, a.cs = _p(pos), _p(cs)
    a.q_out, a.k_out, a.v_out = _p(q_out), _p(k_out), _p(v_out)
    a.T, a.nh, a.hd, a.Lq, a.qoff, a.Lk, a.koff = T, nh, hd, Lq, qoff, Lk, koff
    call("pz_gemv_qkv_rope", C.byref(a), _st())


PZ_ERR_UNSUPPORTED = 3


def gemm_qkv_rope(x, W, pos, cs, q_out, k_out, v_out, T, nh, hd, Lq, qoff, Lk, koff, norm=None, w_scale=None,
                  lora=None):
    a = QkvRopeArgs()
    a.x, a.ldx = _p(x), x.stride(0)
    a.W, a.ldw = _p(W), W.stride(0)
    a.M, a.N, a.K = x.shape[0], W.shape[0], x.shape[1]
    if norm is not None:
        a.norm_w, a.norm_eps = _p(norm[0]), float(norm[1])
    if w_scale is not None:
        a.w_fp8, a.w_scale = 1, float(w_scale)
    a.pos, a.cs = _p(pos), _p(cs)
    a.q_out, a.k_out, a.v_out = _p(q_out), _p(k_out), _p(v_out)
    a.T, a.nh, a.hd, a.Lq, a.qoff, a.Lk, a.koff = T, nh, hd, Lq, qoff, Lk, koff
    if lora is not None:
        a.x2, a.ldx2, a.W2, a.ldw2, a.K2 = _p(lora[0]), lora[0].stride(0), _p(lora[1]), lora[1].stride(0), lora[0].shape[1]
    rc = lib().pz_gemm_qkv_rope(C.byref(a), _st())
    if rc == PZ_ERR_UNSUPPORTED:
        return False
    if rc != 0:
        raise NativeError(f"pz_gemm_qkv_rope failed (rc={rc}): {lib().pz_last_error().decode(errors='replace')}")
    return True


def decode_attn(q, Lq, qoff, k, v, o, B, nh, T, nk, scale, cap, cnt, prefix, cond, qtok0):
    a = DecodeAttnArgs()
    a.q, a.ldq, a.Lq, a.qoff = _p(q), q.shape[-1], Lq, qoff
    a.k, a.v = _p(k), _p(v)
    a.k_bstride, a.v_bstride = k.stride(0), v.stride(0)
    a.o, a.ldo = _p(o), o.stride(0)
    a.B, a.nh, a.T, a.nk, a.head_dim = B, nh, T, nk, k.shape[-1]
    a.scale, a.cap = float(scale), float(cap)
    a.cnt, a.prefix, a.cond, a.qtok0 = _p(cnt), prefix, cond, qtok0
    need = lib().pz_decode_attn_ws_bytes(B, T * nh, nk)
    ws = workspace(o.device)
    if ws.numel() * 4 < need:
        raise ValueError(f"decode_attn: {B} samples x {nk} keys need {need} B of workspace (> {ws.numel() * 4})")
    a.ws, a.ws_bytes = _p(ws), ws.numel() * 4
    call("pz_decode_attn", C.byref(a), _st())


def attn_softmax(S, lds, P, ldp, R, N, scale, cap=0.0, tcap=None, mask_mode=0, rows_per_batch=1, heads=1,
                 qoff=0, cnt=None, prefix=0, cond=0, mask=None, ldm=0, mask_bstride=0):
    a = SoftmaxArgs()
    a.S, a.lds, a.P, a.ldp, a.tcap = _p(S), lds, _p(P), ldp, _p(tcap)
    a.R, a.N, a.scale, a.cap, a.mask_mode = R, N, float(scale), float(cap), mask_mode
    a.rows_per_batch, a.heads, a.qoff = rows_per_batch, heads, qoff
    a.cnt, a.prefix, a.cond = _p(cnt), prefix, cond
    a.mask, a.ldm, a.mask_bstride = _p(mask), ldm, mask_bstride
    call("pz_attn_softmax", C.byref(a), _st())


def attn_softmax_bwd(P, dP, lddp, tcap, dS, ldp, R, N, scale, cap):
    call("pz_attn_softmax_bwd", _p(P), _p(dP), lddp, _p(tcap), _p(dS), ldp, R, N, float(scale), float(cap),
         _st())


def flash_args(Z, H, nq, nk, hd, q, q_strides, k, k_strides, v, v_strides, groups, o_hstride, lse, scale,
               cap=0.0, mask_mode=0, cnt=None, prefix=0, cond=0, rows_per_token=1, dgroups=None, delta=None,
               dq=None, dk=None, dv=None, mask_row0=0, key_split=False):
    a = FlashArgs()
    a.Z, a.H, a.nq, a.nk, a.head_dim = int(Z), int(H), int(nq), int(nk), int(hd)
    a.q, (a.ldq, a.q_bstride, a.q_hstride) = _p(q), tuple(int(x) for x in q_strides)
    a.k, (a.ldk, a.k_bstride, a.k_hstride) = _p(k), tuple(int(x) for x in k_strides)
    a.v, (a.ldv, a.v_bstride, a.v_hstride) = _p(v), tuple(int(x) for x in v_strides)
    a.n_groups = len(groups)
    for i, (r0, o, bs, ld) in enumerate(groups):
        a.g_row0[i], a.g_o[i], a.g_bstride[i], a.g_ld[i] = int(r0), _p(o), int(bs), int(ld)
        if dgroups is not None:
            a.g_do[i] = _p(dgroups[i])
    a.o_hstride = int(o_hstride)
    a.lse = _p(lse)
    a.scale, a.cap, a.mask_mode = float(scale), float(cap), int(mask_mode)
    a.cnt, a.prefix, a.cond, a.rows_per_token = _p(cnt), int(prefix), int(cond), int(rows_per_token)
    a.mask_row0 = int(mask_row0)
    a.delta, a.dq, a.dk, a.dv = _p(delta), _p(dq), _p(dk), _p(dv)
    if dq is not None or key_split:
        ws = flash_workspace(q.device)
        a.ws, a.ws_bytes = ws.data_ptr(), ws.numel() * ws.element_size()
    return a


_FLASH_WS_BYTES = 320 << 20
_FLASH_WS = {}


def flash_workspace(device):
    dev = torch.device(device)
    ws = _FLASH_WS.get(dev)
    if ws is None:
        ws = torch.empty(_FLASH_WS_BYTES // 4, dtype=torch.float32, device=dev)
        _FLASH_WS[dev] = ws
    return ws


def flash_fwd(a):
    call("pz_flash_fwd", C.byref(a), _st())


def fp8_quant_vt(v, Z, nk, vt, vs):
    call("pz_fp8_quant_vt", _p(v), v.stride(1), v.stride(0), Z, nk, _p(vt), _p(vs), vt.shape[2], _st())


def fp8_quant_attn(q, k, v, Z, nk, qc, qs, kc, ks, vt, vs):
    call("pz_fp8_quant_attn", _p(q), q.shape[0], _p(k), k.shape[0], _p(v), v.stride(1), v.stride(0), Z, nk, _p(qc),
         _p(qs), _p(kc), _p(ks), _p(vt), _p(vs), vt.shape[2], _st())


def flash_fwd_f8(a, qc, qs, kc, ks, krows, vt, vs):
    call("pz_flash_fwd_f8", C.byref(a), _p(qc), _p(qs), _p(kc), _p(ks), int(krows), _p(vt), _p(vs), vt.shape[2], _st())


def flash_bwd_ds(a, P, tcap, dS, ldp):
    call("pz_flash_bwd_ds", C.byref(a), _p(P), _p(tcap), _p(dS), int(ldp), _st())


def flash_fwd_probs(a, P, tcap, ldp):
    call("pz_flash_fwd_probs", C.byref(a), _p(P), _p(tcap), int(ldp), _st())


def flash_bwd(a):
    call("pz_flash_bwd", C.byref(a), _st())


def flash_bwd_prep(a):
    call("pz_flash_bwd_prep", C.byref(a), _st())


def siglip_flash_args(qkv, O, lse, B, nh, hd, N, dO=None, delta=None, dqkv=None):
    W = qkv.stride(0)
    H = nh * hd
    strides = (W, N * W, hd)
    return flash_args(B, nh, N, N, hd, qkv, strides, qkv[:, H:], strides, qkv[:, 2 * H:], strides,
                      [(0, O, N * O.stride(0), O.stride(0))], hd, lse, hd ** -0.5,
                      dgroups=None if dO is None else [dO], delta=delta,
                      dq=dqkv, dk=None if dqkv is None else dqkv[:, H:], dv=None if dqkv is None else dqkv[:, 2 * H:])


def patchify(pix, cols, ps):
    B, _, H, W = pix.shape
    call("pz_patchify", _p(pix), _p(cols), B, H, W, ps, cols.stride(0), _st())


def embed_merge(ids, table, img, out, n_img, image_token, pad_token, emb_scale, img_scale):
    B, P = ids.shape
    D = table.shape[1]
    call("pz_embed_merge", _p(ids), _p(table), table.shape[0], _p(img), _p(out), B, P, D, n_img, image_token,
         pad_token,
         float(emb_scale), float(img_scale), _st())


def embed_merge_bwd(ids, dout, dimg, n_img, image_token, img_scale):
    B, P = ids.shape
    D = dout.shape[-1]
    call("pz_embed_merge_bwd", _p(ids), _p(dout), _p(dimg), B, P, D, n_img, image_token, float(img_scale),
         _st())


def time_embed(t, out, max_period, ref_bf16=False):
    B, D = out.shape
    call("pz_time_embed", _p(t), _p(out), B, D, float(max_period), int(bool(ref_bf16)), _st())


def time_embed_rows(t, out, H, max_period, ref_bf16=False):
    rows, D = out.shape
    call("pz_time_embed_rows", _p(t), _p(out), out.stride(0), rows // H, H, D, float(max_period), int(bool(ref_bf16)),
         _st())


def concat_time(temb, e1, out, B, H, D):
    call("pz_concat_time", _p(temb), _p(e1), _p(out), B, H, D, _st())


def split_time_grad(dcat, de1, rows, D):
    call("pz_split_time_grad", _p(dcat), _p(de1), rows, D, _st())


def flow_psi(x0, x1, t, psi, sig_min):
    B = x0.shape[0]
    call("pz_flow_psi", _p(x0), _p(x1), _p(t), _p(psi), B, x0[0].numel(), float(sig_min), _st())


def flow_loss(v, ldv, vbs, x0, x1, loss, dv, grad_scale, B, H, A, sig_min):
    call("pz_flow_loss", _p(v), ldv, vbs, _p(x0), _p(x1), _p(loss), _p(dv), _p(grad_scale), B, H, A,
         float(sig_min), _st())


def action_in(action, W1, b1, t, cat, B, H, D, max_period, ref_bf16=False):
    A = action.shape[-1]
    call("pz_action_in", _p(action), A, _p(W1), _p(b1), _p(t), _p(cat), cat.stride(0), B, H, D, float(max_period),
         int(bool(ref_bf16)), _st())


def action_out(x, norm_w, eps, Wd, bd, action, t, B, H, dt):
    D = x.shape[1]
    call("pz_action_out", _p(x), x.stride(0), _p(norm_w), float(eps), _p(Wd), _p(bd), D, Wd.shape[0], _p(action),
         _p(t), B, H, float(dt), _st())


def euler_step(action, v, ldv, vbs, t, B, H, A, dt):
    call("pz_euler_step", _p(action), _p(v), ldv, vbs, _p(t), B, H, A, float(dt), _st())


def copy_rows(src, sld, sbs, dst, dld, dbs, B, rows, D, scale=1.0, beta=False):
    call("pz_copy_rows", _p(src), sld, sbs, _p(dst), dld, dbs, B, rows, D, float(scale), int(beta), _st())


def clamp_(x, lo, hi):
    call("pz_clamp", _p(x), x.numel(), float(lo), float(hi), _st())


def geglu_bwd(dh, gu, dgu, h_out, M, I):
    call("pz_geglu_bwd", _p(dh), dh.stride(0), _p(gu), gu.stride(0), _p(dgu), _p(h_out),
         0 if h_out is None else h_out.stride(0), M, I, _st())


def act_bwd(dh, pre, dpre, h_out, act):
    M, N = pre.shape
    call("pz_act_bwd", _p(dh), dh.stride(0), _p(pre), pre.stride(0), _p(dpre), _p(h_out),
         0 if h_out is None else h_out.stride(0), M, N, int(act), _st())


def adamw(p, g, m, v, lr, b1, b2, eps, wd, bc1, bc2, gscale=None):
    call("pz_adamw", _p(p), _p(g), _p(m), _p(v), p.numel(), float(lr), float(b1), float(b2), float(eps),
         float(wd), float(bc1), float(bc2), _p(gscale), _st())


ROUND_COMPENSATED, ROUND_STOCHASTIC = 1, 2


def splitmix64(z):
    m = 2 ** 64 - 1
    z = (z + 0x9E3779B97F4A7C15) & m
    z = ((z ^ (z >> 30)) * 0xBF58476D1CE4E5B9) & m
    z = ((z ^ (z >> 27)) * 0x94D049BB133111EB) & m
    return z ^ (z >> 31)


def adamw_r(p, comp, g, m, v, lr, b1, b2, eps, wd, bc1, bc2, gscale=None, *, mode, rng_key=0, rng_base=0):
    call("pz_adamw_r", _p(p), _p(comp), _p(g), _p(m), _p(v), p.numel(), float(lr), float(b1), float(b2), float(eps),
         float(wd), float(bc1), float(bc2), _p(gscale), int(mode), C.c_uint64(int(rng_key) & (2 ** 64 - 1)),
         int(rng_base), _st())


def _adamw8_args(run, g, qmap1, qmap2, lr, b1, b2, eps, wd, t, gscale):
    import numpy as np

    f = np.float32
    c1 = f(1.0 - b1 ** t)
    c2 = f(np.sqrt(1.0 - b2 ** t))
    a = AdamW8Args()
    a.p, a.g = _p(run["flat"]), _p(g)
    a.s1, a.s2 = _p(run["s1"]), _p(run["s2"])
    a.absmax1, a.absmax2 = _p(run["absmax1"]), _p(run["absmax2"])
    a.m32, a.v32 = _p(run["m32"]), _p(run["v32"])
    a.seg, a.nseg, a.nblocks = _p(run["seg"]), run["nseg"], run["nblocks"]
    a.qmap1, a.qmap2 = _p(qmap1), _p(qmap2)
    a.beta1, a.beta2 = float(f(b1)), float(f(b2))
    a.omb1, a.omb2 = float(f(1.0 - b1)), float(f(1.0 - b2))
    a.step = float(f(f(-lr) * c2 / c1))
    a.epsc = float(f(f(eps) * c2))
    a.decay = float(f(1.0 - lr * wd)) if wd > 0 else 1.0
    a.gscale = _p(gscale)
    return a


def adamw8bit(run, g, qmap1, qmap2, lr, b1, b2, eps, wd, t, gscale=None):
# ... 224 lines not shown
```

Baseline: 274.9 samples/s.

## Fuse dQ un-RoPE and packing into joint flash backward dS kernel; skip padded key tiles

The joint-attention backward dS kernel can now apply the inverse RoPE to dQ itself and write it straight into the packed per-group dqkv buffer. This removes the separate dQ tensor and the Q part of the split-backward kernel, which now handles only K/V. It also adds a HALF variant of the fwd-probs and bwd-ds kernels that skips MFMA work, loads and stores for the unused upper half of the last key block when ldp is short enough. The cost is more register pressure from the cos/sin tile loads, and more fragile wave-wait counts and pack logic, all gated by PZ_JOINT_LEAN.

```diff
diff --git a/include/pz_abi.h b/include/pz_abi.h
--- a/include/pz_abi.h
+++ b/include/pz_abi.h
@@ -119,6 +119,9 @@
 int pz_qkv_rope_split_bwd(const void* dq, const void* dk, const void* dv, const int64_t* pos,
                           const float* cs, void* dqkv, int64_t B, int64_t T, int64_t nh, int64_t nkv,
                           int64_t hd, int64_t Lq, int64_t qoff, int64_t Lk, int64_t koff, void* stream);
+int pz_qkv_rope_split_bwd_kv(const void* dk, const void* dv, const int64_t* pos, const float* cs, void* dqkv,
+                             int64_t B, int64_t T, int64_t nh, int64_t nkv, int64_t hd, int64_t Lk, int64_t koff,
+                             void* stream);
 
 typedef struct pz_softmax_args {
   const float* S; int64_t lds;
@@ -160,6 +163,15 @@
                     int64_t krows, const void* vtc, const float* vs, int64_t ldvt, void* stream);
 int pz_flash_fwd_probs(const pz_flash_args* a, void* P, void* tcap, int64_t ldp, void* stream);
 int pz_flash_bwd_ds(const pz_flash_args* a, const void* P, const void* tcap, void* dS, int64_t ldp, void* stream);
+typedef struct pz_flash_dqkv {
+  void* dqkv[3];
+  const int64_t* pos[3];
+  const float* cs[3];
+  int64_t T[3];
+  int64_t ld;
+} pz_flash_dqkv;
+int pz_flash_bwd_ds_pack(const pz_flash_args* a, const void* P, const void* tcap, void* dS, int64_t ldp,
+                         const pz_flash_dqkv* d, void* stream);
 int pz_flash_bwd_prep(const pz_flash_args* a, void* stream);
 int pz_flash_bwd(const pz_flash_args* a, void* stream);
 
diff --git a/open-pi-zero_amd/csrc/pz_attn.hip b/open-pi-zero_amd/csrc/pz_attn.hip
--- a/open-pi-zero_amd/csrc/pz_attn.hip
+++ b/open-pi-zero_amd/csrc/pz_attn.hip
@@ -53,6 +53,7 @@
   for (int e = threadIdx.x; e < nkv * hd; e += blockDim.x) dv[e] = sv[e];
 }
 
+template <bool QCOLS>
 __global__ void qkv_rope_split_bwd_kernel(const bf16_t* __restrict__ dq, const bf16_t* __restrict__ dk,
                                           const bf16_t* __restrict__ dv, const int64_t* __restrict__ pos,
                                           const float* __restrict__ cs, bf16_t* dqkv, int64_t T, int nh,
@@ -64,18 +65,20 @@
   const int width = (nh + 2 * nkv) * hd;
   bf16_t* dst = dqkv + tok * width;
   const float* c = cs + pos[tok] * hd;
-  const bf16_t* sq = dq ? dq + (b * Lq + qoff + t) * (int64_t)(nh * hd) : nullptr;
-  for (int e = threadIdx.x; e < nh * half; e += blockDim.x) {
-    const int h = e / half, i = e % half;
-    float o1 = 0.f, o2 = 0.f;
-    if (sq) {
-      const float y1 = bf2f(sq[h * hd + i]), y2 = bf2f(sq[h * hd + i + half]);
-      const float co = c[2 * i], si = c[2 * i + 1];
-      o1 = y1 * co + y2 * si;
-      o2 = y2 * co - y1 * si;
-    }
-    dst[h * hd + i] = f2bf(o1);
-    dst[h * hd + i + half] = f2bf(o2);
+  if constexpr (QCOLS) {
+    const bf16_t* sq = dq ? dq + (b * Lq + qoff + t) * (int64_t)(nh * hd) : nullptr;
+    for (int e = threadIdx.x; e < nh * half; e += blockDim.x) {
+      const int h = e / half, i = e % half;
+      float o1 = 0.f, o2 = 0.f;
+      if (sq) {
+        const float y1 = bf2f(sq[h * hd + i]), y2 = bf2f(sq[h * hd + i + half]);
+        const float co = c[2 * i], si = c[2 * i + 1];
+        o1 = y1 * co + y2 * si;
+        o2 = y2 * co - y1 * si;
+      }
+      dst[h * hd + i] = f2bf(o1);
+      dst[h * hd + i + half] = f2bf(o2);
+    }
   }
   const bf16_t* sk = dk + (b * Lk + koff + t) * (int64_t)(nkv * hd);
   const bf16_t* sv = dv + (b * Lk + koff + t) * (int64_t)(nkv * hd);
@@ -367,9 +370,22 @@
                                      const float* cs, void* dqkv, int64_t B, int64_t T, int64_t nh, int64_t nkv,
                                      int64_t hd, int64_t Lq, int64_t qoff, int64_t Lk, int64_t koff, void* stream) {
   PZ_CHECK_ARG(dk && dv && pos && cs && dqkv && B > 0 && T > 0, "qkv_rope_split_bwd: bad args");
-  hipLaunchKernelGGL(qkv_rope_split_bwd_kernel, dim3((unsigned)T, (unsigned)B), dim3(256), 0,
+  hipLaunchKernelGGL(qkv_rope_split_bwd_kernel<true>, dim3((unsigned)T, (unsigned)B), dim3(256), 0,
                      (hipStream_t)stream, (const bf16_t*)dq, (const bf16_t*)dk, (const bf16_t*)dv, pos, cs,
                      (bf16_t*)dqkv, T, (int)nh, (int)nkv, (int)hd, Lq, qoff, Lk, koff);
+  PZ_CHECK_LAUNCH();
+  return PZ_OK;
+}
+
+extern "C" int pz_qkv_rope_split_bwd_kv(const void* dk, const void* dv, const int64_t* pos, const float* cs,
+                                        void* dqkv, int64_t B, int64_t T, int64_t nh, int64_t nkv, int64_t hd,
+                                        int64_t Lk, int64_t koff, void* stream) {
+  PZ_CHECK_ARG(dk && dv && pos && cs && dqkv && B > 0 && T > 0 && nh >= 0 && nkv > 0 && hd > 0,
+               "qkv_rope_split_bwd_kv: bad args");
+  PZ_CHECK_ARG(koff >= 0 && koff + T <= Lk, "qkv_rope_split_bwd_kv: token range");
+  hipLaunchKernelGGL(qkv_rope_split_bwd_kernel<false>, dim3((unsigned)T, (unsigned)B), dim3(256), 0,
+                     (hipStream_t)stream, (const bf16_t*)nullptr, (const bf16_t*)dk, (const bf16_t*)dv, pos, cs,
+                     (bf16_t*)dqkv, T, (int)nh, (int)nkv, (int)hd, (int64_t)0, (int64_t)0, Lk, koff);
   PZ_CHECK_LAUNCH();
   return PZ_OK;
 }
diff --git a/open-pi-zero_amd/csrc/pz_flash.hip b/open-pi-zero_amd/csrc/pz_flash.hip
--- a/open-pi-zero_amd/csrc/pz_flash.hip
+++ b/open-pi-zero_amd/csrc/pz_flash.hip
@@ -2176,6 +2176,8 @@
 }
 
 constexpr int JD_SLOT = 64 * 512, JD_SMEM = 4 * JD_SLOT;
+constexpr int JD_HALF_LDP = (JP_MAXKB - 1) * FA_KB + 32;
+#define JD_SKIP(kb, i) (HALF && (kb) == JP_MAXKB - 1 && (i) >= 2)
 
 struct JdDma {
   int wave, lane;
@@ -2208,7 +2210,7 @@
   for (int u = 0; u < 4; ++u) o[DG * 4 + u] = mfma(fs_cat(tv[u][0], tv[u][1]), pk, o[DG * 4 + u]);
 }
 
-template <bool CAP>
+template <bool CAP, bool HALF>
 __global__ void __launch_bounds__(JP_NW * 64, 1) flash_fwd_probs_dma_kernel(pz_flash_args a, bf16_t* P, bf16_t* TC,
                                                                          int64_t ldp) {
   extern __shared__ __attribute__((aligned(16))) char fa_smem[];
@@ -2253,6 +2255,7 @@
     auto logits = [&](auto FAST) {
 #pragma unroll
       for (int i = 0; i < 4; ++i) {
+        if (JD_SKIP(kb, i)) continue;
         float tv[4];
 #pragma unroll
         for (int e = 0; e < 4; ++e) {
@@ -2295,7 +2298,8 @@
     for (int ks = 0; ks < 8; ++ks) {
       const char* kp = slot + 16 * ((4 * ks + g) ^ l15);
 #pragma unroll
-      for (int i = 0; i < 4; ++i) sc[kb][i] = mfma(*reinterpret_cast<const bf16x8*>(kp + i * 8192), qf[ks], sc[kb][i]);
+      for (int i = 0; i < 4; ++i)
+        if (!JD_SKIP(kb, i)) sc[kb][i] = mfma(*reinterpret_cast<const bf16x8*>(kp + i * 8192), qf[ks], sc[kb][i]);
     }
     if (kb >= 1) logits_blk(kb - 1);
   }
@@ -2308,6 +2312,7 @@
     for (int kb = 0; kb < JP_MAXKB; ++kb)
 #pragma unroll
       for (int i = 0; i < 4; ++i) {
+        if (JD_SKIP(kb, i)) continue;
         const int j0 = kb * FA_KB + i * 16 + 4 * g;
         if (clean && (kb + 1) * 64 <= full_keys) *reinterpret_cast<u32x2*>(trow + j0) = tcv[kb][i];
         else if (live && j0 < ldp) *reinterpret_cast<u32x2*>(trow + j0) = tcv[kb][i];
@@ -2321,6 +2326,7 @@
     for (int i = 0; i < 4; ++i)
 #pragma unroll
       for (int e = 0; e < 4; ++e) {
+        if (JD_SKIP(kb, i)) continue;
         const float pv = __builtin_amdgcn_exp2f(sc[kb][i][e] - mx);
         sc[kb][i][e] = pv;
         sum += pv;
@@ -2330,10 +2336,11 @@
   bf16x8 pf[JP_MAXKB][2];
 #pragma unroll
   for (int kb = 0; kb < JP_MAXKB; ++kb) {
-    unsigned pk[4][2];
+    unsigned pk[4][2] = {};
     auto probs = [&](auto FAST) {
 #pragma unroll
       for (int i = 0; i < 4; ++i) {
+        if (JD_SKIP(kb, i)) continue;
         if constexpr (decltype(FAST)::value) {
           pk[i][0] = pack2bf(sc[kb][i][0] * inv, sc[kb][i][1] * inv);
           pk[i][1] = pack2bf(sc[kb][i][2] * inv, sc[kb][i][3] * inv);
@@ -2379,6 +2386,7 @@
     jd_pv_group<0, 1>(o, vs, pf[kb][0]);
     jd_pv_group<0, 2>(o, vs, pf[kb][0]);
     jd_pv_group<0, 3>(o, vs, pf[kb][0]);
+    if (JD_SKIP(kb, 2)) continue;
     jd_pv_group<1, 0>(o, vs, pf[kb][1]);
     jd_pv_group<1, 1>(o, vs, pf[kb][1]);
     jd_pv_group<1, 2>(o, vs, pf[kb][1]);
@@ -2395,8 +2403,18 @@
   }
 }
 
+
+__device__ __forceinline__ void jd_unrope(float y1, float y2, float co, float si, float& o1, float& o2) {
+#pragma clang fp contract(off)
+  const float a1 = y1 * co, a2 = y1 * si;
+  o1 = __builtin_fmaf(y2, si, a1);
+  o2 = __builtin_fmaf(y2, co, -a2);
+}
+
+template <bool HALF>
 __global__ void __launch_bounds__(JP_NW * 64, 1) flash_bwd_ds_dma_kernel(pz_flash_args a, const bf16_t* P,
-                                                                      const bf16_t* TC, bf16_t* dS, int64_t ldp) {
+                                                                      const bf16_t* TC, bf16_t* dS, int64_t ldp,
+                                                                      pz_flash_dqkv pkd, bool pack) {
   extern __shared__ __attribute__((aligned(16))) char fa_smem[];
   constexpr int RPW = JP_NW * 16;
   const int lane = threadIdx.x & 63, wave = threadIdx.x >> 6, g = lane >> 4, l15 = lane & 15;
@@ -2406,7 +2424,7 @@
   const int64_t b = zh / a.H, h = zh % a.H;
   const int64_t r = (int64_t)qblk * RPW + wave * 16 + l15;
   const bool live = r < a.nq;
-  const bool want_dq = a.dq != nullptr;
+  const bool want_dq = a.dq != nullptr || pack;
   const bf16_t* V = (const bf16_t*)a.v + b * a.v_bstride + h * a.v_hstride;
   const bf16_t* K = want_dq ? (const bf16_t*)a.k + b * a.k_bstride + h * a.k_hstride : V;
   const int64_t ldk = want_dq ? a.ldk : a.ldv;
@@ -2428,10 +2446,29 @@
     JD_DLD(0); JD_DLD(1); JD_DLD(2); JD_DLD(3); JD_DLD(4); JD_DLD(5); JD_DLD(6); JD_DLD(7);
 #undef JD_DLD
   }
+  const bf16_t* prow = P + (b * a.nq + (live ? r : 0)) * ldp;
+  bf16_t* pdst = nullptr;
+  const float* ptab = nullptr;
+  u32x2 ppos;
+  {
+    const int64_t* pp = reinterpret_cast<const int64_t*>(prow);
+    if (pack) {
+      const FaRow fr{&a};
+      const int gi = live ? fr.grp(r) : 0;
+      ptab = pkd.dqkv[0] ? pkd.cs[0] : (pkd.dqkv[1] ? pkd.cs[1] : pkd.cs[2]);
+      if (live && pkd.dqkv[gi]) {
+        const int rpt = (int)a.rows_per_token, rl = (int)(r - a.g_row0[gi]), t = rl / rpt, hh = rl - t * rpt;
+        const int64_t tok = b * pkd.T[gi] + t;
+        pdst = (bf16_t*)pkd.dqkv[gi] + tok * pkd.ld + hh * 256 + 4 * g;
+        ptab = pkd.cs[gi];
+        pp = pkd.pos[gi] + tok;
+      }
+    }
+    asm volatile("global_load_dwordx2 %0, %1, off" : "=v"(ppos) : "v"(pp) : "memory");
+  }
   issue(0);
   issue(1);
   issue(2);
-  const bf16_t* prow = P + (b * a.nq + (live ? r : 0)) * ldp;
   const bf16_t* trow = TC ? TC + (b * a.nq + (live ? r : 0)) * ldp : prow;
   const bool clean = __ballot(!live) == 0ull;
   f32x4 dp[JP_MAXKB][4];
@@ -2456,7 +2493,8 @@
     for (int ks = 0; ks < 8; ++ks) {
       const char* vp = slot + 16 * ((4 * ks + g) ^ l15);
 #pragma unroll
-      for (int i = 0; i < 4; ++i) dp[kb][i] = mfma(*reinterpret_cast<const bf16x8*>(vp + i * 8192), df[ks], dp[kb][i]);
+      for (int i = 0; i < 4; ++i)
+        if (!JD_SKIP(kb, i)) dp[kb][i] = mfma(*reinterpret_cast<const bf16x8*>(vp + i * 8192), df[ks], dp[kb][i]);
     }
   }
   int gl = g;
@@ -2465,6 +2503,7 @@
   for (int k2 = 0; k2 < JP_MAXKB; ++k2)
 #pragma unroll
     for (int i = 0; i < 4; ++i) {
+      if (JD_SKIP(k2, i)) continue;
       const int j0 = k2 * FA_KB + i * 16 + 4 * gl;
       const int jc = j0 < ldp ? j0 : 0;
       asm volatile("global_load_dwordx2 %0, %1, off" : "=v"(pw[k2][i]) : "v"(prow + jc) : "memory");
@@ -2473,11 +2512,13 @@
   for (int k2 = 0; k2 < JP_MAXKB; ++k2)
 #pragma unroll
     for (int i = 0; i < 4; ++i) {
+      if (JD_SKIP(k2, i)) continue;
       const int j0 = k2 * FA_KB + i * 16 + 4 * gl;
       const int jc = j0 < ldp ? j0 : 0;
       asm volatile("global_load_dwordx2 %0, %1, off" : "=v"(tw[k2][i]) : "v"(trow + jc) : "memory");
     }
-  FS_WAIT_VM(20);
+  if constexpr (HALF) FS_WAIT_VM(18);
+  else FS_WAIT_VM(20);
   bf16_t* orow = dS + (b * a.nq + (live ? r : 0)) * ldp;
   const bool cap = a.cap > 0.f;
   float dot = 0.f;
@@ -2485,6 +2526,7 @@
   for (int kb = 0; kb < JP_MAXKB; ++kb)
 #pragma unroll
     for (int i = 0; i < 4; ++i) {
+      if (JD_SKIP(kb, i)) continue;
       asm volatile("" : "+v"(pw[kb][i]));
       const int j0 = kb * FA_KB + i * 16 + 4 * g;
       if (!(live && j0 < nk)) pw[kb][i] = u32x2{0u, 0u};
@@ -2498,13 +2540,15 @@
 #pragma unroll
   for (int kb = 0; kb < JP_MAXKB; ++kb)
 #pragma unroll
-    for (int i = 0; i < 4; ++i) asm volatile("" : "+v"(tw[kb][i]));
+    for (int i = 0; i < 4; ++i)
+      if (!JD_SKIP(kb, i)) asm volatile("" : "+v"(tw[kb][i]));
   bf16x8 dsf[JP_MAXKB][2];
 #pragma unroll
   for (int kb = 0; kb < JP_MAXKB; ++kb) {
-    unsigned pk[4][2];
+    unsigned pk[4][2] = {};
 #pragma unroll
     for (int i = 0; i < 4; ++i) {
+      if (JD_SKIP(kb, i)) continue;
       const int j0 = kb * FA_KB + i * 16 + 4 * g;
       const u32x2 tv2 = (cap && live && j0 < nk) ? tw[kb][i] : u32x2{0u, 0u};
       const float pv[4] = {__uint_as_float(pw[kb][i][0] << 16), __uint_as_float(pw[kb][i][0] & 0xffff0000u),
@@ -2531,6 +2575,7 @@
   unsigned ka[8];
 #pragma unroll
   for (int d7 = 0; d7 < 8; ++d7) ka[d7] = fs_lds_addr(fa_smem + (4 * g + q4) * 512 + 32 * (d7 ^ w) + 8 * p4);
+  f32x4 ct[16];
 #pragma unroll
   for (int kb = 0; kb < JP_MAXKB; ++kb) {
     const int s = 5 + kb;
@@ -2538,6 +2583,15 @@
     if (s == 9) FS_WAIT_VM(0);
     FS_BARRIER();
     if (s + 3 <= 9) issue(s + 3);
+    if (s == 9 && pack) {
+      asm volatile("" : "+v"(ppos));
+      const int64_t pos = pdst ? (int64_t)(((uint64_t)ppos[1] << 32) | ppos[0]) : 0;
+      const float* c = ptab + pos * 256 + 8 * g;
+#define JD_CLD(i) asm volatile("global_load_dwordx4 %0, %1, off offset:%2" : "=v"(ct[i]) : "v"(c), "i"(((i) >> 1) * 128 + ((i) & 1) * 16) : "memory")
+      JD_CLD(0); JD_CLD(1); JD_CLD(2); JD_CLD(3); JD_CLD(4); JD_CLD(5); JD_CLD(6); JD_CLD(7);
+      JD_CLD(8); JD_CLD(9); JD_CLD(10); JD_CLD(11); JD_CLD(12); JD_CLD(13); JD_CLD(14); JD_CLD(15);
+#undef JD_CLD
+    }
     if (want_dq) {
       const unsigned sb = (unsigned)((s % 4) * JD_SLOT);
       unsigned ks_[8];
@@ -2547,6 +2601,7 @@
       jd_pv_group<0, 1>(dq, ks_, dsf[kb][0]);
       jd_pv_group<0, 2>(dq, ks_, dsf[kb][0]);
       jd_pv_group<0, 3>(dq, ks_, dsf[kb][0]);
+      if (JD_SKIP(kb, 2)) continue;
       jd_pv_group<1, 0>(dq, ks_, dsf[kb][1]);
       jd_pv_group<1, 1>(dq, ks_, dsf[kb][1]);
       jd_pv_group<1, 2>(dq, ks_, dsf[kb][1]);
@@ -2554,6 +2609,29 @@
     }
   }
   if (!live || !want_dq) return;
+  if (pack) {
+    if (!pdst) return;
+    bf16_t* dst = pdst;
+    FS_WAIT_VM(0);
+    asm volatile(""
+                 : "+v"(ct[0]), "+v"(ct[1]), "+v"(ct[2]), "+v"(ct[3]), "+v"(ct[4]), "+v"(ct[5]), "+v"(ct[6]), "+v"(ct[7]),
+                   "+v"(ct[8]), "+v"(ct[9]), "+v"(ct[10]), "+v"(ct[11]), "+v"(ct[12]), "+v"(ct[13]), "+v"(ct[14]),
+                   "+v"(ct[15]));
+#pragma unroll
+    for (int db = 0; db < 8; ++db) {
+      const f32x4 c01 = ct[2 * db], c23 = ct[2 * db + 1];
+      const unsigned l01 = pack2bf(dq[db][0], dq[db][1]), l23 = pack2bf(dq[db][2], dq[db][3]);
+      const unsigned h01 = pack2bf(dq[db + 8][0], dq[db + 8][1]), h23 = pack2bf(dq[db + 8][2], dq[db + 8][3]);
+      float o1[4], o2[4];
+      jd_unrope(__uint_as_float(l01 << 16), __uint_as_float(h01 << 16), c01[0], c01[1], o1[0], o2[0]);
+      jd_unrope(__uint_as_float(l01 & 0xffff0000u), __uint_as_float(h01 & 0xffff0000u), c01[2], c01[3], o1[1], o2[1]);
+      jd_unrope(__uint_as_float(l23 << 16), __uint_as_float(h23 << 16), c23[0], c23[1], o1[2], o2[2]);
+      jd_unrope(__uint_as_float(l23 & 0xffff0000u), __uint_as_float(h23 & 0xffff0000u), c23[2], c23[3], o1[3], o2[3]);
+      *reinterpret_cast<u32x2*>(dst + db * 16) = u32x2{pack2bf(o1[0], o1[1]), pack2bf(o1[2], o1[3])};
+      *reinterpret_cast<u32x2*>(dst + 128 + db * 16) = u32x2{pack2bf(o2[0], o2[1]), pack2bf(o2[2], o2[3])};
+    }
+    return;
+  }
   bf16_t* dQ = (bf16_t*)a.dq + b * a.q_bstride + h * a.q_hstride + r * a.ldq;
 #pragma unroll
   for (int db = 0; db < 16; ++db) {
@@ -2872,6 +2950,11 @@
 }
 
 
+static bool fa_joint_lean() {
+  const char* e = getenv("PZ_JOINT_LEAN");
+  return !(e && e[0] == '0');
+}
+
 extern "C" int pz_flash_fwd_probs(const pz_flash_args* a, void* P, void* tcap, int64_t ldp, void* stream) {
   PZ_CHECK_ARG(a && a->q && a->k && a->v && P && a->Z > 0 && a->H > 0 && a->nq > 0 && a->nk > 0,
                "flash_fwd_probs: bad args");
@@ -2889,23 +2972,27 @@
   PZ_CHECK_ARG(a->nq + a->mask_row0 < (1 << 22) && a->Z * a->H < 65536, "flash_fwd_probs: nq / units too large");
   const int64_t units = a->Z * a->H, nqb = (a->nq + JP_NW * 16 - 1) / (JP_NW * 16);
   {
-    static bool attr0 = false, attr1 = false;
+    static bool attr[2][2] = {};
+    const bool half = fa_joint_lean() && ldp <= JD_HALF_LDP;
+    auto launch = [&](auto kern, bool& done) {
+      fa_smem_attr(kern, JD_SMEM, done);
+      hipLaunchKernelGGL(kern, dim3((unsigned)(nqb * units)), dim3(JP_NW * 64), JD_SMEM, (hipStream_t)stream, *a,
+                         (bf16_t*)P, (bf16_t*)tcap, ldp);
+    };
     if (a->cap > 0.f) {
-      fa_smem_attr(flash_fwd_probs_dma_kernel<true>, JD_SMEM, attr1);
-      hipLaunchKernelGGL(flash_fwd_probs_dma_kernel<true>, dim3((unsigned)(nqb * units)), dim3(JP_NW * 64), JD_SMEM,
-                         (hipStream_t)stream, *a, (bf16_t*)P, (bf16_t*)tcap, ldp);
+      if (half) launch(flash_fwd_probs_dma_kernel<true, true>, attr[1][1]);
+      else launch(flash_fwd_probs_dma_kernel<true, false>, attr[1][0]);
     } else {
-      fa_smem_attr(flash_fwd_probs_dma_kernel<false>, JD_SMEM, attr0);
-      hipLaunchKernelGGL(flash_fwd_probs_dma_kernel<false>, dim3((unsigned)(nqb * units)), dim3(JP_NW * 64), JD_SMEM,
-                         (hipStream_t)stream, *a, (bf16_t*)P, (bf16_t*)tcap, ldp);
+      if (half) launch(flash_fwd_probs_dma_kernel<false, true>, attr[0][1]);
+      else launch(flash_fwd_probs_dma_kernel<false, false>, attr[0][0]);
     }
     PZ_CHECK_LAUNCH();
     return PZ_OK;
   }
 }
 
-extern "C" int pz_flash_bwd_ds(const pz_flash_args* a, const void* P, const void* tcap, void* dS, int64_t ldp,
-                               void* stream) {
+static int fa_bwd_ds(const pz_flash_args* a, const void* P, const void* tcap, void* dS, int64_t ldp,
+                     const pz_flash_dqkv* d, void* stream) {
   PZ_CHECK_ARG(a && a->v && P && dS && a->Z > 0 && a->H > 0 && a->nq > 0 && a->nk > 0, "flash_bwd_ds: bad args");
   PZ_CHECK_ARG(a->head_dim == 256, "flash_bwd_ds: head_dim %lld (256 only)", (long long)a->head_dim);
   PZ_CHECK_ARG(a->nk <= JP_MAXKB * FA_KB && ldp >= a->nk && ldp % 4 == 0, "flash_bwd_ds: nk %lld / ldp %lld",
@@ -2916,18 +3003,53 @@
   PZ_CHECK_ARG(PZ_ALIGNED(a->v, 16) && a->ldv % 8 == 0 && a->v_bstride % 8 == 0 && PZ_ALIGNED(P, 8) &&
                    PZ_ALIGNED(dS, 8) && (!tcap || PZ_ALIGNED(tcap, 8)),
                "flash_bwd_ds: alignment");
-  if (a->dq)
+  if (a->dq && !d)
     PZ_CHECK_ARG(a->k && PZ_ALIGNED(a->k, 16) && a->ldk % 8 == 0 && a->k_bstride % 8 == 0 && PZ_ALIGNED(a->dq, 8) &&
                      a->ldq % 4 == 0 && a->q_bstride % 4 == 0,
                  "flash_bwd_ds: dQ needs K (16-byte rows) and an 8-byte aligned dQ");
+  if (d) {
+    PZ_CHECK_ARG(a->k && PZ_ALIGNED(a->k, 16) && a->ldk % 8 == 0 && a->k_bstride % 8 == 0,
+                 "flash_bwd_ds_pack: dQ needs K (16-byte rows)");
+    PZ_CHECK_ARG(a->H == 1 && a->rows_per_token > 0 && a->rows_per_token * 256 <= d->ld && d->ld % 4 == 0 &&
+                     a->nq % a->rows_per_token == 0,
+                 "flash_bwd_ds_pack: H %lld, rows per token %lld, pitch %lld", (long long)a->H,
+                 (long long)a->rows_per_token, (long long)d->ld);
+    bool any = false;
+    for (int i = 0; i < a->n_groups; ++i) any = any || d->dqkv[i];
+    PZ_CHECK_ARG(any, "flash_bwd_ds_pack: no group has a destination");
+    for (int i = 0; i < a->n_groups; ++i) {
+      const int64_t end = i + 1 < a->n_groups ? a->g_row0[i + 1] : a->nq;
+      PZ_CHECK_ARG(a->g_row0[i] % a->rows_per_token == 0 && end >= a->g_row0[i], "flash_bwd_ds_pack: group %d rows", i);
+      if (!d->dqkv[i]) continue;
+      PZ_CHECK_ARG(d->pos[i] && d->cs[i] && PZ_ALIGNED(d->cs[i], 16) && PZ_ALIGNED(d->dqkv[i], 8) &&
+                       (end - a->g_row0[i]) / a->rows_per_token <= d->T[i],
+                   "flash_bwd_ds_pack: group %d destination", i);
+    }
+  }
   PZ_CHECK_ARG(a->Z * a->H < 65536, "flash_bwd_ds: too many units");
   const int64_t units = a->Z * a->H, nqb = (a->nq + JP_NW * 16 - 1) / (JP_NW * 16);
-  static bool attr = false;
-  fa_smem_attr(flash_bwd_ds_dma_kernel, JD_SMEM, attr);
-  hipLaunchKernelGGL(flash_bwd_ds_dma_kernel, dim3((unsigned)(nqb * units)), dim3(JP_NW * 64), JD_SMEM,
-                     (hipStream_t)stream, *a, (const bf16_t*)P, (const bf16_t*)tcap, (bf16_t*)dS, ldp);
+  static bool attr[2] = {};
+  const bool half = fa_joint_lean() && ldp <= JD_HALF_LDP;
+  auto launch = [&](auto kern, bool& done) {
+    fa_smem_attr(kern, JD_SMEM, done);
+    hipLaunchKernelGGL(kern, dim3((unsigned)(nqb * units)), dim3(JP_NW * 64), JD_SMEM, (hipStream_t)stream, *a,
+                       (const bf16_t*)P, (const bf16_t*)tcap, (bf16_t*)dS, ldp, d ? *d : pz_flash_dqkv{}, d != nullptr);
+  };
+  if (half) launch(flash_bwd_ds_dma_kernel<true>, attr[1]);
+  else launch(flash_bwd_ds_dma_kernel<false>, attr[0]);
   PZ_CHECK_LAUNCH();
   return PZ_OK;
+}
+
+extern "C" int pz_flash_bwd_ds(const pz_flash_args* a, const void* P, const void* tcap, void* dS, int64_t ldp,
+                               void* stream) {
+  return fa_bwd_ds(a, P, tcap, dS, ldp, nullptr, stream);
+}
+
+extern "C" int pz_flash_bwd_ds_pack(const pz_flash_args* a, const void* P, const void* tcap, void* dS, int64_t ldp,
+                                    const pz_flash_dqkv* d, void* stream) {
+  PZ_CHECK_ARG(d, "flash_bwd_ds_pack: no destination");
+  return fa_bwd_ds(a, P, tcap, dS, ldp, d, stream);
 }
 
 extern "C" int pz_flash_bwd_prep(const pz_flash_args* a, void* stream) {
diff --git a/open-pi-zero_amd/pizero_native/_lib.py b/open-pi-zero_amd/pizero_native/_lib.py
--- a/open-pi-zero_amd/pizero_native/_lib.py
+++ b/open-pi-zero_amd/pizero_native/_lib.py
@@ -82,6 +82,10 @@
         ("ws", vp), ("ws_bytes", i64),
         ("mask_row0", i64),
     ]
+
+
+class FlashDqkv(C.Structure):
+    _fields_ = [("dqkv", vp * 3), ("pos", vp * 3), ("cs", vp * 3), ("T", i64 * 3), ("ld", i64)]
 
 
 class AdamW8Args(C.Structure):
@@ -142,6 +146,7 @@
     "pz_rope_table": [vp, i64, i64, f32, vp],
     "pz_qkv_rope_split": [vp, vp, vp, vp, vp, vp, i64, i64, i64, i64, i64, i64, i64, i64, i64, vp],
     "pz_qkv_rope_split_bwd": [vp, vp, vp, vp, vp, vp, i64, i64, i64, i64, i64, i64, i64, i64, i64, vp],
+    "pz_qkv_rope_split_bwd_kv": [vp, vp, vp, vp, vp, i64, i64, i64, i64, i64, i64, i64, vp],
     "pz_gemv_qkv_rope": [C.POINTER(QkvRopeArgs), vp],
     "pz_gemm_qkv_rope": [C.POINTER(QkvRopeArgs), vp],
     "pz_decode_attn": [C.POINTER(DecodeAttnArgs), vp],
@@ -151,6 +156,7 @@
     "pz_flash_fwd": [C.POINTER(FlashArgs), vp],
     "pz_flash_fwd_probs": [C.POINTER(FlashArgs), vp, vp, i64, vp],
     "pz_flash_bwd_ds": [C.POINTER(FlashArgs), vp, vp, vp, i64, vp],
+    "pz_flash_bwd_ds_pack": [C.POINTER(FlashArgs), vp, vp, vp, i64, C.POINTER(FlashDqkv), vp],
     "pz_flash_bwd_prep": [C.POINTER(FlashArgs), vp],
     "pz_flash_bwd": [C.POINTER(FlashArgs), vp],
     "pz_patchify": [vp, vp, i64, i64, i64, i64, i64, vp],
diff --git a/open-pi-zero_amd/pizero_native/engine.py b/open-pi-zero_amd/pizero_native/engine.py
--- a/open-pi-zero_amd/pizero_native/engine.py
+++ b/open-pi-zero_amd/pizero_native/engine.py
@@ -1081,13 +1081,17 @@
         dO[g.name] = o
         dXm[g.name] = dxm
 
-    def _qkv_backward(self, g, gs, p, dQ, dK, dV, dX, dXm, pos, B, L, Lp, beta, rpp, nh, hd, dev, A=None, l=None):
+    def _qkv_backward(self, g, gs, p, dQ, dK, dV, dX, dXm, pos, B, L, Lp, beta, rpp, nh, hd, dev, A=None, l=None,
+                      dqkv=None):
         x = gs["x"]
         M = x.shape[0]
         W = (nh + 2) * hd
-        dqkv = torch.empty(M, W, device=dev, dtype=BF16)
-        ops.qkv_rope_split_bwd(None if gs.get("skip") else dQ, dK, dV, pos[g.pos_key], self.rope(g.theta), dqkv,
-                               B, g.T, nh, 1, hd, L, g.off, Lp, g.off)
+        if dqkv is not None:
+            ops.qkv_rope_split_bwd_kv(dK, dV, pos[g.pos_key], self.rope(g.theta), dqkv, B, g.T, nh, 1, hd, Lp, g.off)
+        else:
+            dqkv = torch.empty(M, W, device=dev, dtype=BF16)
+            ops.qkv_rope_split_bwd(None if gs.get("skip") else dQ, dK, dV, pos[g.pos_key], self.rope(g.theta), dqkv,
+                                   B, g.T, nh, 1, hd, L, g.off, Lp, g.off)
         names = [p + f"self_attn.{k}_proj.weight" for k in "qkv"]
         rgs = [self.rg(n) for n in names]
         site = self.lora(*names)
@@ -1149,9 +1153,12 @@
                 A.mod.record_stream(side)
                 A.dmod.record_stream(side)
         ada = sv.get("ada") or {}
+        lean = (os.environ.get("PZ_JOINT_LEAN", "1") != "0" and "lse" not in sv["joint"][0]
+                and not isinstance(cnt, GeneralMask) and L <= 320 and hd == 256)
         for l in reversed(range(d.nL)):
             st = sv["joint"][l]
-            dQ = torch.empty(B, L, nh * hd, device=dev, dtype=BF16)
+            dQ = None if lean else torch.empty(B, L, nh * hd, device=dev, dtype=BF16)
+            dqkv = {}
             dK = torch.empty(B, Lp, hd, device=dev, dtype=BF16)
             dV = torch.empty(B, Lp, hd, device=dev, dtype=BF16)
             dO = {}
@@ -1183,8 +1190,17 @@
                 if not isinstance(cnt, GeneralMask) and L <= 320 and hd == 256:
                     if dS is None:
                         dS = torch.empty(B, L * nh, Lp, device=dev, dtype=BF16)
-                    ops.flash_bwd_ds(self._joint_flash(groups, Qj, Kj, Vj, st["O"], None, cnt, B, L, dO=dO,
-                                                       dq=dQ), Pm, tc, dS, Lp)
+                    fa = self._joint_flash(groups, Qj, Kj, Vj, st["O"], None, cnt, B, L, dO=dO, dq=dQ)
+                    W = (nh + 2) * hd
+                    if lean:
+                        dqkv = {g.name: torch.empty(B * g.T, W, device=dev, dtype=BF16) for g in groups
+                                if not st["g"][g.name].get("skip")}
+                    if dqkv:
+                        ops.flash_bwd_ds_pack(fa, Pm, tc, dS, Lp, [
+                            (dqkv[g.name], pos[g.pos_key], self.rope(g.theta), g.T) if g.name in dqkv else None
+                            for g in sorted(groups, key=lambda g: g.off)], W)
+                    else:
+                        ops.flash_bwd_ds(fa, Pm, tc, dS, Lp)
                     dq_done = True
                 else:
                     if dP is None:
@@ -1215,13 +1231,14 @@
                     dV.zero_()
             if side is not None:
                 side.wait_stream(main)
-                for t in (dQ, dK, dV):
-                    t.record_stream(side)
+                for t in (dQ, dK, dV, *(t for n, t in dqkv.items() if n != "vlm")):
+                    if t is not None:
+                        t.record_stream(side)
             for g in groups:
                 with self._on(side, g):
                     self._qkv_backward(g, st["g"][g.name], f"{g.prefix}{l}.", dQ, dK, dV, dX, dXm, pos, B, L, Lp, beta,
-                                       rpp, nh, hd, dev, ada.get(g.name), l)
-            self._chk(f"joint bwd layer {l}", dO=dO, dS=dS, dQ=dQ, dK=dK, dV=dV, dX=dX)
+                                       rpp, nh, hd, dev, ada.get(g.name), l, dqkv=dqkv.get(g.name))
+            self._chk(f"joint bwd layer {l}", dO=dO, dS=dS, dQ=dQ, dqkv=dqkv, dK=dK, dV=dV, dX=dX)
             self._notify("joint", l, (side,) if side is not None else ())
         if side is not None:
             main.wait_stream(side)
diff --git a/open-pi-zero_amd/pizero_native/ops.py b/open-pi-zero_amd/pizero_native/ops.py
--- a/open-pi-zero_amd/pizero_native/ops.py
+++ b/open-pi-zero_amd/pizero_native/ops.py
@@ -22,6 +22,7 @@
     QkvRopeArgs,
     DecodeAttnArgs,
     FlashArgs,
+    FlashDqkv,
     GemmArgs,
     SmallGemmArgs,
     NativeError,
@@ -395,6 +396,10 @@
 def qkv_rope_split(qkv, pos, cs, q_out, k_out, v_out, B, T, nh, nkv, hd, Lq, qoff, Lk, koff):
     call("pz_qkv_rope_split", _p(qkv), _p(pos), _p(cs), _p(q_out), _p(k_out), _p(v_out), B, T, nh, nkv, hd,
          Lq, qoff, Lk, koff, _st())
+
+
+def qkv_rope_split_bwd_kv(dk, dv, pos, cs, dqkv, B, T, nh, nkv, hd, Lk, koff):
+    call("pz_qkv_rope_split_bwd_kv", _p(dk), _p(dv), _p(pos), _p(cs), _p(dqkv), B, T, nh, nkv, hd, Lk, koff, _st())
 
 
 def qkv_rope_split_bwd(dq, dk, dv, pos, cs, dqkv, B, T, nh, nkv, hd, Lq, qoff, Lk, koff):
@@ -531,6 +536,15 @@
 
 def flash_bwd_ds(a, P, tcap, dS, ldp):
     call("pz_flash_bwd_ds", C.byref(a), _p(P), _p(tcap), _p(dS), int(ldp), _st())
+
+
+def flash_bwd_ds_pack(a, P, tcap, dS, ldp, dests, ld):
+    d = FlashDqkv()
+    d.ld = int(ld)
+    for i, dst in enumerate(dests):
+        if dst is not None:
+            d.dqkv[i], d.pos[i], d.cs[i], d.T[i] = _p(dst[0]), _p(dst[1]), _p(dst[2]), int(dst[3])
+    call("pz_flash_bwd_ds_pack", C.byref(a), _p(P), _p(tcap), _p(dS), int(ldp), C.byref(d), _st())
 
 
 def flash_fwd_probs(a, P, tcap, ldp):
```

Measured after the change: 275.7 samples/s, median of 6. No clear change (+0.3%).
